# kolinko/effort

Measured on AMD Instinct MI355X. Metric: effective GB/s + tokens/s vs effort %, Mistral-7B FFN 4096x11008 fp16, higher is better.
Workload: dtype f16

## Files before the change

### effort_amd/_lib.py

```python
from __future__ import annotations

import ctypes as C
import os
import subprocess

_HERE = os.path.dirname(os.path.abspath(__file__))
LAB_LIB_PATH = os.path.join(_HERE, "libeffort_hip_lab.so")
LIB_PATH = (LAB_LIB_PATH if os.environ.get("EFFORT_HIP_LIB") == "lab" else os.environ.get("EFFORT_HIP_LIB")) or os.path.join(_HERE, "libeffort_hip.so")

ERRORS = {
    -1: "EFFORT_ERR_ARG", -2: "EFFORT_ERR_SHAPE", -3: "EFFORT_ERR_EFFORT", -4: "EFFORT_ERR_HIP",
    -5: "EFFORT_ERR_KIND", -6: "EFFORT_ERR_CONVERT", -7: "EFFORT_ERR_BLAS", -8: "EFFORT_ERR_COMM",
}


class EffortError(RuntimeError):
    def __init__(self, code: int, where: str, detail: str = ""):
        self.code = code
        super().__init__(f"{where}: {ERRORS.get(code, code)} {detail}".strip())


def build(verbose: bool = False) -> str:
    cmd = ["make", "-C", os.path.join(_HERE, "csrc"), "-j8", "all"]
    res = subprocess.run(cmd, capture_output=not verbose, text=True)
    if res.returncode != 0:
        raise RuntimeError("building libeffort_hip.so failed:\n" + (res.stdout or "") + (res.stderr or ""))
    return LIB_PATH


_P = C.c_void_p
_SIGS = {
    "effort_create": (_P, [C.c_int, _P]),
    "effort_destroy": (None, [_P]),
    "effort_set_stream": (C.c_int, [_P, _P]),
    "effort_sync": (C.c_int, [_P]),
    "effort_set_overlap": (C.c_int, [_P, C.c_int]),
    "effort_set_row_reuse": (C.c_int, [_P, C.c_int]),
    "effort_join": (C.c_int, [_P]),
    "effort_last_error": (C.c_char_p, [_P]),
    "effort_version": (C.c_char_p, []),
    "effort_weights_fp16": (_P, [_P, _P, _P, _P, C.c_int, C.c_int, C.c_int, C.c_int]),
    "effort_weights_fp16_pitched": (_P, [_P, _P, C.c_int, _P, _P, C.c_int, C.c_int, C.c_int, C.c_int]),
    "effort_aligned_row_pitch": (C.c_int, [C.c_int]),
    "effort_weights_q4": (_P, [_P, _P, _P, _P, _P, C.c_int64, C.c_int, C.c_int, C.c_int]),
    "effort_weights_free": (None, [_P]),
    "effort_weights_refresh": (C.c_int, [_P]),
    "effort_weights_align_rows": (C.c_int, [_P]),
    "effort_weights_row_pitch": (C.c_int, [_P]),
    "effort_weights_get_bound": (C.c_int, [_P, C.POINTER(C.c_float)]),
    "effort_weights_set_bound": (C.c_int, [_P, C.POINTER(C.c_float)]),
    "effort_weights_column_shard": (_P, [_P, C.c_int, C.c_int]),
    "effort_comm_unique_id": (C.c_int, [_P]),
    "effort_comm_create": (C.c_int, [_P, C.c_int, C.c_int, _P]),
    "effort_comm_destroy": (C.c_int, [_P]),
    "effort_comm_rank": (C.c_int, [_P]),
    "effort_comm_world": (C.c_int, [_P]),
    "effort_allgather_outputs": (C.c_int, [_P, _P, _P, C.c_int]),
    "effort_bucketmul": (C.c_int, [_P, _P, _P, _P, _P, C.c_double]),
    "effort_bucketmul_q4": (C.c_int, [_P, _P, _P, _P, _P, C.c_double]),
    "effort_bucketmul_group": (C.c_int, [_P, C.c_int, _P, _P, _P, _P, _P]),
    "effort_bucketmul_q4_group": (C.c_int, [_P, C.c_int, _P, _P, _P, _P, _P]),
    "effort_bucketmul_group_fused": (C.c_int, [_P, C.c_int, _P, _P, _P, _P, _P, _P, _P, _P]),
    "effort_bucketmul_q4_group_fused": (C.c_int, [_P, C.c_int, _P, _P, _P, _P, _P, _P, _P, _P]),
    "effort_group_dispatch_count": (C.c_int, [_P, C.c_int, C.POINTER(C.c_uint32)]),
    "effort_group_cutoff": (C.c_int, [_P, C.c_int, C.POINTER(C.c_float)]),
    "effort_debug_occupancy": (C.c_int, [_P, C.c_int, C.c_int, C.c_int, C.c_int]),
    "effort_set_persistent": (C.c_int, [_P, C.c_int]),
    "effort_debug_hook_lane": (C.c_int, [_P, C.c_int]),
    "effort_add_rmsnorm_mul": (C.c_int, [_P, _P, _P, _P, _P, C.c_int]),
    "effort_rope_kv": (C.c_int, [_P, _P, _P, _P, _P, _P, _P, _P, C.c_int, C.c_int, C.c_int, C.c_int, C.c_float]),
    "effort_attention": (C.c_int, [_P, _P, _P, _P, _P, _P, C.c_int, C.c_int, C.c_int]),
    "effort_rope_attention": (C.c_int, [_P, _P, _P, _P, _P, _P, _P, _P, C.c_int, C.c_int, C.c_int, C.c_int, C.c_float]),
    "effort_silu_mul": (C.c_int, [_P, _P, _P, _P, C.c_int]),
    "effort_fetch_row": (C.c_int, [_P, _P, _P, _P, C.c_int]),
    "effort_argmax": (C.c_int, [_P, _P, C.c_int, _P, _P, _P, C.c_int]),
    "effort_decode_status": (C.c_int, [_P, C.POINTER(C.c_int)]),
    "effort_sample": (C.c_int, [_P, _P, C.c_int, _P, _P, _P, _P, C.c_int, _P, _P]),
    "effort_topk": (C.c_int, [_P, _P, C.c_int, C.c_int, _P, _P]),
    "effort_sample_bits": (C.c_uint32, [C.c_uint32, C.c_uint32, C.c_uint32, C.c_uint32]),
    "effort_convert_status": (C.c_int, [_P, C.POINTER(C.c_int)]),
    "effort_q4_outlier_count": (C.c_int64, [C.c_int, C.c_int, C.c_double]),
    "effort_convert_q4": (C.c_int, [_P, _P, C.c_int, C.c_int, C.c_double, _P, _P, _P, _P]),
    "effort_top2_softmax": (C.c_int, [_P, _P, C.c_int, _P, _P]),
    "effort_mix2": (C.c_int, [_P, _P, _P, _P, _P, C.c_int]),
    "effort_moe_route": (C.c_int, [_P, _P, _P, _P, C.c_int, C.c_int, _P, _P, _P]),
    "effort_mix2_add": (C.c_int, [_P, _P, _P, _P, _P, C.c_int]),
    "effort_dense_gemv": (C.c_int, [_P, _P, _P, _P, C.c_int, C.c_int]),
    "effort_dense_gemv_expert": (C.c_int, [_P, _P, _P, _P, _P, C.c_int, C.c_int, C.c_int]),
    "effort_set_dense_backend": (C.c_int, [_P, C.c_int]),
    "effort_last_dispatch_count": (C.c_int, [_P, C.POINTER(C.c_uint32)]),
    "effort_last_cutoff": (C.c_int, [_P, C.POINTER(C.c_float)]),
    "effort_calc_dispatch": (C.c_int, [_P, _P, _P, _P, C.c_double, _P, _P]),
    "effort_convert_fp16": (C.c_int, [_P, _P, C.c_int, C.c_int, _P, _P, _P]),
    "effort_convert_fp16_pitched": (C.c_int, [_P, _P, C.c_int, C.c_int, _P, C.c_int, _P, _P]),
    "effort_cosine": (C.c_int, [_P, _P, _P, C.c_int, C.POINTER(C.c_float)]),
    "effort_set_split_cutoff": (C.c_int, [_P, C.c_int]),
    "effort_set_tuning": (C.c_int, [_P, C.c_int, C.c_int, C.c_int]),
    "effort_is_lab_build": (C.c_int, []),
    "effort_enable_kernel_timing": (C.c_int, [_P, C.c_int]),
    "effort_debug_stamps": (C.c_int, [_P, C.POINTER(C.c_ulonglong)]),
    "effort_debug_slice_counts": (C.c_int, [_P, C.c_int, C.POINTER(C.c_uint32), C.c_int]),
    "effort_debug_plan": (C.c_int, [C.c_int, C.c_int, C.c_int, C.c_int, _P, _P, _P, _P, _P, _P, C.c_int, C.c_int, C.c_int, C.c_int, _P, _P, _P, _P, _P, _P, _P, _P, _P]),
    "effort_debug_trace": (C.c_int, [_P, C.POINTER(C.c_ulonglong), C.c_int]),
    "effort_kernel_clock": (C.c_int, [_P, C.POINTER(C.c_double), C.POINTER(C.c_int)]),
    "effort_kernel_timing": (C.c_int, [_P, C.POINTER(C.c_double), C.POINTER(C.c_double), C.POINTER(C.c_double), C.POINTER(C.c_int)]),
}

_lib = None


def lib() -> C.CDLL:
    global _lib
    if _lib is None:
        if not os.path.exists(LIB_PATH):
            raise RuntimeError(
                f"{LIB_PATH} is missing: the HIP extension has not been built "
                "(run `python -c 'import __graft_entry__ as g; g.build()'` or `make -C effort_amd/csrc`). "
                "effort_amd has no CPU fallback.")
        import torch
        l = C.CDLL(LIB_PATH)
        for name, (res, args) in _SIGS.items():
            if (name.startswith("effort_debug_") or name == "effort_is_lab_build") and os.environ.get("EFFORT_HIP_LIB") and not hasattr(l, name):
                continue
            fn = getattr(l, name)
            fn.restype = res
            fn.argtypes = args
        _lib = l
    return _lib


def exported_symbols() -> list[str]:
    return sorted(_SIGS)
```

### effort_amd/csrc/api.hip

```cpp
#include <dlfcn.h>
#include <rccl/rccl.h>
#include <rocblas/rocblas.h>

#include <cstdio>
#include <cstring>
#include <map>
#include <mutex>
#include <new>
#include <vector>

#include "../../include/effort_hip.h"
#include "../../include/effort_hip_debug.h"
#include "effort_internal.h"
#include "plan.h"
#include "sample_device.h"

using namespace effort;

static constexpr size_t kStampBytes = (size_t)(kTraceOff + kTraceItems * 12) * 8;

struct Lane {
    hipStream_t own = nullptr;
    hipEvent_t done = nullptr;
    bool dirty = false;
    unsigned long long capId = 0;
    float* d_cutoff = nullptr;
    uint32_t* d_count = nullptr;
    float* d_slabs = nullptr;
    uint32_t* d_counters = nullptr;
    uint32_t* d_sliceCounts = nullptr;
    uint32_t* d_queue = nullptr;
    uint32_t lastCalls = 1, lastSliceOff[effort::kMaxGroup] = {0}, lastSlices[effort::kMaxGroup] = {0};
    struct Range { uintptr_t lo, hi; };
    std::vector<Range> reads, writes;
    bool pending = false;
};

struct effort_ctx {
    static constexpr int kMaxLanes = 4;
    int device = 0;
    hipStream_t stream = nullptr;
    int numCU = 256;
    Lane lane[kMaxLanes];
    int nLanes = 1, lastLane = 0, nextLane = 0;
    int busyStreak = 0;
    bool migrated = false;
    hipEvent_t forkEv = nullptr;
    size_t slabBytes = 0;
    uint32_t* d_blockScratch = nullptr;
    uint16_t* d_vhalf = nullptr;
    size_t vhalfElems = 0;
    float* d_cos = nullptr;
    uint16_t* d_convVals = nullptr;
    size_t convElems = 0;
    int* d_status = nullptr;
    int persistent = -1;
    static constexpr uint32_t kMaxTiles = 1024, kMaxSlices = 4096;
    static constexpr size_t kSlabBytes = (size_t)64 << 20;
    static constexpr size_t kMaxRanges = 1024;
    unsigned long long* d_tstamp = nullptr;
    double wallClockKHz = 100000.0;
    rocblas_handle blas = nullptr;
    ncclComm_t comm = nullptr;
    int commRank = 0, commWorld = 1;
    bool denseRocblas = false;
    int tuneW = 0, tuneE = 0, tuneS = 0;
    bool splitCutoff = false;
    bool rowReuse = false;
    bool timing = false;
    bool clock = false;
    bool trace = false;
    static constexpr int kMaxSamples = 4096;
    hipEvent_t* ev = nullptr;
    int nSamples = 0;
    char err[256] = {0};
};

struct effort_w {
    effort_ctx* ctx = nullptr;
    Format fmt = kFp16;
    const uint16_t* buckets = nullptr;
    const uint16_t* bucketsSrc = nullptr;
    uint16_t* aligned = nullptr;
    uint32_t rowPitch = 0;
    uint32_t srcPitch = 0;
    const void* stats = nullptr;
    const uint16_t* probes = nullptr;
    uint32_t inDim = 0, outDim = 0, rowsPerIn = 0, numExperts = 1, cols = 0;
    bool view = false;
    effort_w* parent = nullptr;
    uint32_t viewTrim = 0;
    int views = 0;
    bool dead = false;
    float* rankBound = nullptr;
    uint16_t* means16 = nullptr;
    uint64_t nOutliers = 0;
    uint32_t* olBlockPtr = nullptr;
    uint32_t* olEntry = nullptr;
    uint32_t* olMeta = nullptr;
};

static int fail(effort_ctx* c, int code, const char* what, hipError_t e = hipSuccess) {
    if (c) {
        if (e != hipSuccess) snprintf(c->err, sizeof(c->err), "%s: %s", what, hipGetErrorString(e));
        else snprintf(c->err, sizeof(c->err), "%s", what);
    }
    return code;
}
#define HIP_TRY(ctx, call)                                                   \
    do {                                                                     \
        hipError_t e_ = (call);                                              \
        if (e_ != hipSuccess) return fail((ctx), EFFORT_ERR_HIP, #call, e_); \
    } while (0)

struct RcclApi {
    void* lib = nullptr;
    ncclResult_t (*GetUniqueId)(ncclUniqueId*) = nullptr;
    ncclResult_t (*CommInitRank)(ncclComm_t*, int, ncclUniqueId, int) = nullptr;
    ncclResult_t (*CommDestroy)(ncclComm_t) = nullptr;
    ncclResult_t (*AllGather)(const void*, void*, size_t, ncclDataType_t, ncclComm_t, hipStream_t) = nullptr;
    const char* (*GetErrorString)(ncclResult_t) = nullptr;
    bool ok = false;
};
static const RcclApi& rccl() {
    static RcclApi api = [] {
        RcclApi a;
        for (const char* name : {"librccl.so.1", "librccl.so", "/opt/rocm/lib/librccl.so.1", "/opt/rocm/lib/librccl.so"}) {
            a.lib = dlopen(name, RTLD_NOW | RTLD_GLOBAL);
            if (a.lib) break;
        }
        if (!a.lib) return a;
        a.GetUniqueId = reinterpret_cast<decltype(a.GetUniqueId)>(dlsym(a.lib, "ncclGetUniqueId"));
        a.CommInitRank = reinterpret_cast<decltype(a.CommInitRank)>(dlsym(a.lib, "ncclCommInitRank"));
        a.CommDestroy = reinterpret_cast<decltype(a.CommDestroy)>(dlsym(a.lib, "ncclCommDestroy"));
        a.AllGather = reinterpret_cast<decltype(a.AllGather)>(dlsym(a.lib, "ncclAllGather"));
        a.GetErrorString = reinterpret_cast<decltype(a.GetErrorString)>(dlsym(a.lib, "ncclGetErrorString"));
        a.ok = a.GetUniqueId && a.CommInitRank && a.CommDestroy && a.AllGather && a.GetErrorString;
        return a;
    }();
    return api;
}

extern "C" const char* effort_version(void) { return "effort-hip 0.1 (gfx950)"; }
static char g_createErr[256] = "null context";
extern "C" const char* effort_last_error(effort_ctx* c) { return c ? c->err : g_createErr; }

static bool lane_alloc(effort_ctx* c, Lane& L) {
    bool ok = hipMalloc(&L.d_cutoff, 512) == hipSuccess && hipMalloc(&L.d_count, 16) == hipSuccess &&
              hipMalloc(&L.d_slabs, c->slabBytes) == hipSuccess && hipMalloc(&L.d_counters, effort_ctx::kMaxTiles * 4) == hipSuccess &&
              hipMalloc(&L.d_sliceCounts, effort_ctx::kMaxSlices * 4) == hipSuccess && hipMalloc(&L.d_queue, kQueueWords * 4) == hipSuccess;
    if (!ok) return false;
    hipMemset(L.d_counters, 0, effort_ctx::kMaxTiles * 4);
    hipMemset(L.d_sliceCounts, 0, effort_ctx::kMaxSlices * 4);
    hipMemset(L.d_queue, 0, kQueueWords * 4);
    hipMemset(L.d_cutoff, 0, 512);
    hipMemset(L.d_count, 0, 16);
    return true;
}
static std::mutex g_poolMutex;
static std::map<int, std::vector<hipStream_t>> g_streamPool;
static std::map<int, std::vector<hipEvent_t>> g_eventPool;
static hipStream_t pool_stream(int device) {
    std::lock_guard<std::mutex> lk(g_poolMutex);
    auto& pool = g_streamPool[device];
    if (!pool.empty()) { hipStream_t s = pool.back(); pool.pop_back(); return s; }
    hipStream_t s = nullptr;
    return hipStreamCreateWithFlags(&s, hipStreamNonBlocking) == hipSuccess ? s : nullptr;
}
static hipEvent_t pool_event(int device) {
    std::lock_guard<std::mutex> lk(g_poolMutex);
    auto& pool = g_eventPool[device];
    if (!pool.empty()) { hipEvent_t e = pool.back(); pool.pop_back(); return e; }
    hipEvent_t e = nullptr;
    return hipEventCreateWithFlags(&e, hipEventDisableTiming) == hipSuccess ? e : nullptr;
}
static void pool_put(int device, hipStream_t s) { if (s) { std::lock_guard<std::mutex> lk(g_poolMutex); g_streamPool[device].push_back(s); } }
static void pool_put(int device, hipEvent_t e) { if (e) { std::lock_guard<std::mutex> lk(g_poolMutex); g_eventPool[device].push_back(e); } }

static void lane_free(int device, Lane& L) {
    pool_put(device, L.own);
    pool_put(device, L.done);
    hipFree(L.d_cutoff); hipFree(L.d_count); hipFree(L.d_slabs); hipFree(L.d_counters); hipFree(L.d_sliceCounts); hipFree(L.d_queue);
    L = Lane();
}

extern "C" effort_ctx* effort_create(int device, void* stream) {
    if (hipSetDevice(device) != hipSuccess) return nullptr;
    effort_ctx* c = new (std::nothrow) effort_ctx();
    if (!c) return nullptr;
    c->device = device;
    c->stream = reinterpret_cast<hipStream_t>(stream);
    hipDeviceProp_t prop;
    if (hipGetDeviceProperties(&prop, device) == hipSuccess) c->numCU = prop.multiProcessorCount;
    c->slabBytes = effort_ctx::kSlabBytes;
    {
        static std::mutex m; static std::map<int, bool> prepared;
        std::lock_guard<std::mutex> lk(m);
        if (!prepared[device]) {
            const hipError_t pe = bucket_mul_prepare_device();
            if (pe != hipSuccess) { snprintf(g_createErr, sizeof(g_createErr), "effort_create: kernel attributes: %s", hipGetErrorString(pe)); delete c; return nullptr; }
            prepared[device] = true;
        }
    }
    bool ok = lane_alloc(c, c->lane[0]) && hipMalloc(&c->d_blockScratch, 4096 * 4) == hipSuccess &&
              hipMalloc(&c->d_cos, 16) == hipSuccess && hipMalloc(&c->d_status, 16) == hipSuccess &&
              hipMalloc(&c->d_tstamp, kStampBytes) == hipSuccess;
    if (!ok) { snprintf(g_createErr, sizeof(g_createErr), "effort_create: out of device memory for the context scratch"); effort_destroy(c); return nullptr; }
    int khz = 0;
    if (hipDeviceGetAttribute(&khz, hipDeviceAttributeWallClockRate, device) == hipSuccess && khz > 0) c->wallClockKHz = khz;
    hipMemset(c->d_tstamp, 0, kStampBytes);
    { unsigned long long init[2] = {~0ull, 0ull}; hipMemcpy(c->d_tstamp, init, 16, hipMemcpyHostToDevice); }
    hipMemset(c->d_status, 0, 16);
    return c;
}

static hipStream_t lane_stream(effort_ctx* c, int i) { return c->nLanes > 1 ? c->lane[i].own : c->stream; }
static hipError_t lane_mark(Lane& L) {
    if (!L.dirty) return hipSuccess;
    const hipError_t e = hipEventRecord(L.done, L.own);
    if (e == hipSuccess) L.dirty = false;
    return e;
}
static unsigned long long capture_of(hipStream_t st) {
    hipStreamCaptureStatus cap = hipStreamCaptureStatusNone;
    unsigned long long id = 0;
    if (hipStreamGetCaptureInfo(st, &cap, &id) != hipSuccess) { (void)hipGetLastError(); return 0; }
    return cap == hipStreamCaptureStatusActive ? (id ? id : ~0ull) : 0ull;
}
static bool lanes_match_capture(effort_ctx* c, unsigned long long now) {
    for (int i = 0; i < c->nLanes; i++) {
        Lane& L = c->lane[i];
        if (!L.pending || L.capId == now) continue;
        if (L.capId == 0) {
            snprintf(c->err, sizeof(c->err), "lanes hold launches enqueued BEFORE this hipGraph capture began: call effort_join (or effort_sync) before beginning the capture");
            return false;
        }
        L.pending = false; L.dirty = false; L.capId = 0; L.reads.clear(); L.writes.clear();
    }
    return true;
}
static int join_lanes(effort_ctx* c) {
    if (c->nLanes <= 1) return EFFORT_OK;
    bool any = false;
    for (int i = 0; i < c->nLanes; i++) any = any || c->lane[i].pending;
    if (any && !lanes_match_capture(c, capture_of(c->stream))) return EFFORT_ERR_ARG;
    for (int i = 0; i < c->nLanes; i++) {
        Lane& L = c->lane[i];
        if (!L.pending) continue;
        hipError_t e = lane_mark(L);
        if (e == hipSuccess) e = hipStreamWaitEvent(c->stream, L.done, 0);
        if (e != hipSuccess) { snprintf(c->err, sizeof(c->err), "join: %s", hipGetErrorString(e)); return EFFORT_ERR_HIP; }
        L.pending = false; L.capId = 0; L.reads.clear(); L.writes.clear();
    }
    c->busyStreak = 0; c->migrated = false;
    return EFFORT_OK;
}
static bool overlaps(const std::vector<Lane::Range>& a, const std::vector<Lane::Range>& b) {
    for (const auto& x : a) for (const auto& y : b) if (x.lo < y.hi && y.lo < x.hi) return true;
    return false;
}
struct LaneChoice {
    bool laned = false;
    int li = 0;
    std::vector<Lane::Range> rd, wr;
    int hazard[effort_ctx::kMaxLanes], nh = 0;
    unsigned long long capNow = 0;
};
struct LaneGuard {
    Lane& L; bool forked = false;
    ~LaneGuard() { if (forked) { L.dirty = true; L.pending = true; } }
};
static int choose_lane(effort_ctx* c, LaneChoice& lc, int n, const effort_w* const* ws, const float* const* vs, const uint32_t* const* expNos,
                       float* const* outs, const void* const* vAux, const float* const* resids) {
    if (lc.laned) {
        lc.capNow = capture_of(c->stream);
        if (!lanes_match_capture(c, lc.capNow)) return EFFORT_ERR_ARG;
        bool full = false;
        for (int i = 0; i < c->nLanes; i++) full = full || c->lane[i].reads.size() + c->lane[i].writes.size() > effort_ctx::kMaxRanges;
        if (full) { const int jrc = join_lanes(c); if (jrc != EFFORT_OK) return jrc; }
        auto add = [](std::vector<Lane::Range>& v, const void* p, size_t bytes) { if (p && bytes) v.push_back({(uintptr_t)p, (uintptr_t)p + bytes}); };
        for (int i = 0; i < n; i++) {
            add(lc.rd, vs[i], (size_t)ws[i]->inDim * 4);
            if (expNos && expNos[i]) add(lc.rd, expNos[i], 4);
            if (vAux && vAux[i]) add(lc.rd, vAux[i], (size_t)ws[i]->inDim * 4);
            if (resids && resids[i]) add(lc.rd, resids[i], (size_t)ws[i]->outDim * 4);
            add(lc.wr, outs[i], (size_t)ws[i]->outDim * 4);
        }
        for (int i = 0; i < c->nLanes; i++) {
            const Lane& L = c->lane[i];
            if (L.pending && (overlaps(lc.rd, L.writes) || overlaps(lc.wr, L.writes) || overlaps(lc.wr, L.reads))) lc.hazard[lc.nh++] = i;
        }
        lc.li = lc.nh ? lc.hazard[0] : c->nextLane;
        if (lc.nh == 1 && c->busyStreak >= 4 && !c->migrated) {
            for (int k = 1; k < c->nLanes; k++) {
                const int cand = (lc.hazard[0] + k) % c->nLanes;
                if (!c->lane[cand].pending) { lc.li = cand; c->migrated = true; c->busyStreak = 0; break; }
            }
        }
    } else if (c->nLanes > 1) {
        { const int jrc = join_lanes(c); if (jrc != EFFORT_OK) return jrc; }
    }
    return EFFORT_OK;
}
static int fork_lane(effort_ctx* c, const LaneChoice& lc, LaneGuard& guard) {
    if (!lc.laned || guard.forked) return EFFORT_OK;
    Lane& L = guard.L;
    const int li = lc.li, nh = lc.nh;
    const int* hazard = lc.hazard;
    bool wait = true;
    if (lc.capNow == 0) {
        const hipError_t q = hipStreamQuery(c->stream);
        if (q == hipSuccess) wait = false;
        else {
            (void)hipGetLastError();
            if (q != hipErrorNotReady) return fail(c, EFFORT_ERR_HIP, "hipStreamQuery", q);
        }
    }
    if (wait) {
        HIP_TRY(c, hipEventRecord(c->forkEv, c->stream));
        HIP_TRY(c, hipStreamWaitEvent(L.own, c->forkEv, 0));
    }
    c->busyStreak = (wait && nh == 1 && hazard[0] == li) ? c->busyStreak + 1 : 0;
    guard.forked = true;
    L.capId = lc.capNow;
    auto add_new = [](std::vector<Lane::Range>& have, const std::vector<Lane::Range>& more) {
        for (const auto& x : more) {
            bool seen = false;
            for (const auto& y : have) if (y.lo == x.lo && y.hi == x.hi) { seen = true; break; }
            if (!seen) have.push_back(x);
        }
    };
    for (int k = 0; k < nh; k++) if (hazard[k] != li) {
        Lane& H = c->lane[hazard[k]];
        HIP_TRY(c, lane_mark(H));
        HIP_TRY(c, hipStreamWaitEvent(L.own, H.done, 0));
        add_new(L.reads, H.reads); add_new(L.writes, H.writes);
        H.reads.clear(); H.writes.clear(); H.pending = false;
    }
    if (!nh) c->nextLane = (c->nextLane + 1) % c->nLanes;
    add_new(L.reads, lc.rd);
    add_new(L.writes, lc.wr);
    return EFFORT_OK;
}

extern "C" int effort_set_overlap(effort_ctx* c, int lanes) {
    if (!c || lanes < 1 || lanes > effort_ctx::kMaxLanes) return EFFORT_ERR_ARG;
    hipSetDevice(c->device);
    int rc = join_lanes(c);
    if (rc != EFFORT_OK) return rc;
    if (lanes > 1) {
        if (!c->forkEv && !(c->forkEv = pool_event(c->device))) return fail(c, EFFORT_ERR_HIP, "set_overlap: event");
        for (int i = 0; i < lanes; i++) {
            Lane& L = c->lane[i];
            if (!L.d_slabs && !lane_alloc(c, L)) return fail(c, EFFORT_ERR_HIP, "set_overlap: out of device memory for a lane's scratch");
            if (!L.own && !(L.own = pool_stream(c->device))) return fail(c, EFFORT_ERR_HIP, "set_overlap: stream");
            if (!L.done && !(L.done = pool_event(c->device))) return fail(c, EFFORT_ERR_HIP, "set_overlap: event");
        }
    }
    c->nLanes = lanes; c->lastLane = 0; c->nextLane = 0;
    return EFFORT_OK;
}
extern "C" int effort_join(effort_ctx* c) {
    if (!c) return EFFORT_ERR_ARG;
    return join_lanes(c);
}

extern "C" void effort_destroy(effort_ctx* c) {
    if (!c) return;
    hipSetDevice(c->device);
    for (int i = 0; i < effort_ctx::kMaxLanes; i++) if (c->lane[i].own) hipStreamSynchronize(c->lane[i].own);
    hipStreamSynchronize(c->stream);
    if (c->comm) rccl().CommDestroy(c->comm);
    if (c->blas) rocblas_destroy_handle(c->blas);
    if (c->ev) { for (int i = 0; i < effort_ctx::kMaxSamples * 4; i++) if (c->ev[i]) hipEventDestroy(c->ev[i]); delete[] c->ev; }
    for (int i = 0; i < effort_ctx::kMaxLanes; i++) lane_free(c->device, c->lane[i]);
    pool_put(c->device, c->forkEv);
    hipFree(c->d_blockScratch); hipFree(c->d_vhalf); hipFree(c->d_cos); hipFree(c->d_convVals); hipFree(c->d_status); hipFree(c->d_tstamp);
    delete c;
}

extern "C" int effort_set_stream(effort_ctx* c, void* stream) {
    if (!c) return EFFORT_ERR_ARG;
    if (reinterpret_cast<hipStream_t>(stream) != c->stream && join_lanes(c) != EFFORT_OK) return EFFORT_ERR_HIP;
    c->stream = reinterpret_cast<hipStream_t>(stream);
    if (c->blas) rocblas_set_stream(c->blas, c->stream);
    return EFFORT_OK;
}

extern "C" int effort_sync(effort_ctx* c) {
    if (!c) return EFFORT_ERR_ARG;
    { const int jrc = join_lanes(c); if (jrc != EFFORT_OK) return jrc; }
    HIP_TRY(c, hipStreamSynchronize(c->stream));
    return EFFORT_OK;
}

static int check_shape(uint32_t inDim, uint32_t outDim) {
    if (inDim < (uint32_t)kProbes || outDim == 0 || outDim % 32 || outDim > 16384) return EFFORT_ERR_SHAPE;
    return EFFORT_OK;
}

static int register_bound(effort_ctx* c, effort_w* w) {
    hipSetDevice(c->device);
    const size_t rows = (size_t)w->numExperts * w->rowsPerIn * w->inDim;
    float* scratch = nullptr;
    bool ok = (w->rankBound || hipMalloc(&w->rankBound, (size_t)w->numExperts * 4) == hipSuccess) && hipMalloc(&scratch, rows * 4) == hipSuccess;
    if (ok) ok = launch_rank_bound(w->fmt, w->bucketsSrc, w->srcPitch / 2u, w->stats, w->numExperts, w->rowsPerIn, w->inDim, w->cols, scratch, w->rankBound, c->stream) == hipSuccess;
    if (ok && w->fmt == kFp16) {
        ok = w->means16 || hipMalloc(&w->means16, rows * 2) == hipSuccess;
        if (ok) ok = launch_compact_means(w->stats, w->means16, (uint32_t)rows, c->stream) == hipSuccess;
    }
    if (ok) ok = hipStreamSynchronize(c->stream) == hipSuccess;
    hipFree(scratch);
    return ok ? EFFORT_OK : fail(c, EFFORT_ERR_HIP, "weight registration: rank bound");
}

extern "C" int effort_aligned_row_pitch(int outDim) {
    if (outDim <= 0 || outDim % 32 || outDim > 16384) return EFFORT_ERR_SHAPE;
    return (outDim / 16 * 2 + 127) / 128 * 128;
}

extern "C" effort_w* effort_weights_fp16_pitched(effort_ctx* c, const void* buckets, int rowPitchBytes, const void* stats, const void* probes,
                                                 int inDim, int outDim, int percentLoad, int numExperts) {
    if (!c || !buckets || !stats || !probes) { fail(c, EFFORT_ERR_ARG, "effort_weights_fp16: null argument"); return nullptr; }
    const int pitch = rowPitchBytes ? rowPitchBytes : (outDim > 0 ? outDim / 16 * 2 : 0);
    if (inDim <= 0 || outDim <= 0 || percentLoad < 1 || percentLoad > 16 || numExperts < 1 || check_shape(inDim, outDim) != EFFORT_OK ||
        inDim > 65535 || pitch < outDim / 16 * 2 || pitch % 4 || (size_t)numExperts * percentLoad * inDim * pitch > 0xFFFFFFFFull) {
        fail(c, EFFORT_ERR_SHAPE, "effort_weights_fp16: unsupported shape or row pitch (a multiple of 4 bytes >= 2*cols; buckets < 4 GiB)"); return nullptr; }
    effort_w* w = new (std::nothrow) effort_w();
    if (!w) return nullptr;
    w->ctx = c; w->fmt = kFp16;
    w->buckets = static_cast<const uint16_t*>(buckets); w->stats = stats; w->probes = static_cast<const uint16_t*>(probes);
    w->inDim = inDim; w->outDim = outDim; w->rowsPerIn = percentLoad; w->numExperts = numExperts; w->cols = outDim / 16;
    w->bucketsSrc = w->buckets; w->rowPitch = w->srcPitch = (uint32_t)pitch;
    if (register_bound(c, w) != EFFORT_OK) { effort_weights_free(w); return nullptr; }
    return w;
}
extern "C" effort_w* effort_weights_fp16(effort_ctx* c, const void* buckets, const void* stats, const void* probes,
                                         int inDim, int outDim, int percentLoad, int numExperts) {
    return effort_weights_fp16_pitched(c, buckets, 0, stats, probes, inDim, outDim, percentLoad, numExperts);
}

extern "C" effort_w* effort_weights_q4(effort_ctx* c, const void* buckets, const void* stats, const void* probes,
                                       const void* outliers, int64_t nOutliers, int inDim, int outDim, int numExperts) {
    if (!c || !buckets || !stats || !probes) { fail(c, EFFORT_ERR_ARG, "effort_weights_q4: null argument"); return nullptr; }
    if (inDim <= 0 || outDim <= 0 || numExperts < 1 || check_shape(inDim, outDim) != EFFORT_OK || outDim % 32 || inDim > 65535 ||
        nOutliers < 0 || (size_t)numExperts * 8 * inDim * (outDim / 32) * 2 > 0xFFFFFFFFull) {
        fail(c, EFFORT_ERR_SHAPE, "effort_weights_q4: unsupported shape (or buckets >= 4 GiB)"); return nullptr; }
    effort_w* w = new (std::nothrow) effort_w();
    if (!w) return nullptr;
    w->ctx = c; w->fmt = kQ4;
    w->buckets = static_cast<const uint16_t*>(buckets); w->stats = stats; w->probes = static_cast<const uint16_t*>(probes);
    w->inDim = inDim; w->outDim = outDim; w->rowsPerIn = 8; w->numExperts = numExperts; w->cols = outDim / 32;
    w->bucketsSrc = w->buckets; w->rowPitch = w->srcPitch = w->cols * 2u;
    if (register_bound(c, w) != EFFORT_OK) { effort_weights_free(w); return nullptr; }
    if (outliers && nOutliers > 0) {
        if (outDim > 65536) { fail(c, EFFORT_ERR_SHAPE, "effort_weights_q4: outliers need outDim <= 65536"); effort_weights_free(w); return nullptr; }
        hipSetDevice(c->device);
        {
            int bad[2] = {0, 0};
            bool okv = hipMemsetAsync(c->d_status + 2, 0, 8, c->stream) == hipSuccess &&
                       launch_validate_outliers(static_cast<const float*>(outliers), (uint64_t)nOutliers, (uint32_t)inDim, (uint32_t)outDim, c->d_status + 2, c->stream) == hipSuccess &&
                       hipMemcpyAsync(bad, c->d_status + 2, 8, hipMemcpyDeviceToHost, c->stream) == hipSuccess && hipStreamSynchronize(c->stream) == hipSuccess;
            if (!okv || bad[0] || bad[1]) {
                fail(c, okv ? EFFORT_ERR_ARG : EFFORT_ERR_HIP, !okv ? "effort_weights_q4: outlier validation" :
                     bad[0] ? "effort_weights_q4: outlier entries outside the matrix (inIdx >= inDim or outIdx >= outDim)"
                            : "effort_weights_q4: outlier values that are not f16 numbers (the table comes from an f16 matrix, q4_draft.py:58-67)");
                effort_weights_free(w); return nullptr;
            }
        }
        uint32_t *tmp = nullptr, *rowPtr = nullptr;
        w->nOutliers = (uint64_t)nOutliers;
        const uint32_t olBlocks = ((uint32_t)outDim + 63u) / 64u;
        bool ok = hipMalloc(&rowPtr, ((size_t)outDim + 2) * 4) == hipSuccess && hipMalloc(&w->olBlockPtr, ((size_t)olBlocks + 1) * 4) == hipSuccess &&
                  hipMalloc(&w->olMeta, (size_t)olBlocks * 64 * 4) == hipSuccess &&
                  hipMalloc(&w->olEntry, ((size_t)nOutliers + 64) * 4) == hipSuccess && hipMalloc(&tmp, 4 * (size_t)nOutliers * 4) == hipSuccess;
        if (ok) ok = hipMemsetAsync(w->olEntry + (size_t)nOutliers, 0, 64 * 4, c->stream) == hipSuccess;
        if (ok) ok = launch_build_outlier_index(static_cast<const float*>(outliers), w->nOutliers, (uint32_t)inDim, (uint32_t)outDim, rowPtr, w->olBlockPtr,
                                                w->olEntry, w->olMeta, tmp, c->stream) == hipSuccess;
        if (ok) ok = hipStreamSynchronize(c->stream) == hipSuccess;
        hipFree(tmp);
        uint32_t longest = 0;
        if (ok) ok = hipMemcpy(&longest, rowPtr + (size_t)outDim + 1, 4, hipMemcpyDeviceToHost) == hipSuccess;
        hipFree(rowPtr);
        if (!ok) { fail(c, EFFORT_ERR_HIP, "effort_weights_q4: outlier index"); effort_weights_free(w); return nullptr; }
        if (longest >= (1u << 24)) { fail(c, EFFORT_ERR_SHAPE, "effort_weights_q4: more than 2^24 outliers on one output"); effort_weights_free(w); return nullptr; }
    }
    return w;
}

static int copy_aligned(effort_w* w) {
    const size_t rows = (size_t)w->numExperts * w->rowsPerIn * w->inDim;
    HIP_TRY(w->ctx, hipMemcpy2DAsync(w->aligned, w->rowPitch, w->bucketsSrc, w->srcPitch, (size_t)w->cols * 2, rows, hipMemcpyDeviceToDevice, w->ctx->stream));
    HIP_TRY(w->ctx, hipStreamSynchronize(w->ctx->stream));
    return EFFORT_OK;
}
extern "C" int effort_weights_refresh(effort_w* w) {
    if (!w || !w->ctx || w->dead) return EFFORT_ERR_ARG;
    if (w->view) return fail(w->ctx, EFFORT_ERR_ARG, "effort_weights_refresh: a column shard takes its bound from the full handle -- refresh that one and shard again");
    hipSetDevice(w->ctx->device);
    int rc = join_lanes(w->ctx);
    if (rc == EFFORT_OK) rc = register_bound(w->ctx, w);
    if (rc == EFFORT_OK && w->aligned) rc = copy_aligned(w);
    return rc;
}
extern "C" int effort_weights_align_rows(effort_w* w) {
    if (!w || !w->ctx || w->dead) return EFFORT_ERR_ARG;
    if (w->aligned || w->rowPitch % 128u == 0u) return EFFORT_OK;
    hipSetDevice(w->ctx->device);
    const uint32_t pitch = (w->cols * 2u + 127u) / 128u * 128u;
    const size_t rows = (size_t)w->numExperts * w->rowsPerIn * w->inDim;
    if (rows * pitch > 0xFFFFFFFFull) return fail(w->ctx, EFFORT_ERR_SHAPE, "effort_weights_align_rows: the padded buckets would reach 4 GiB");
    if (hipMalloc(&w->aligned, rows * pitch) != hipSuccess) return fail(w->ctx, EFFORT_ERR_HIP, "effort_weights_align_rows: out of device memory");
    HIP_TRY(w->ctx, hipMemsetAsync(w->aligned, 0, rows * pitch, w->ctx->stream));
    w->rowPitch = pitch;
    const int rc = copy_aligned(w);
    if (rc != EFFORT_OK) { hipFree(w->aligned); w->aligned = nullptr; w->rowPitch = w->srcPitch; return rc; }
    w->buckets = w->aligned;
    return EFFORT_OK;
}
extern "C" int effort_weights_row_pitch(const effort_w* w) { return w ? (int)w->rowPitch : EFFORT_ERR_ARG; }
extern "C" int effort_weights_get_bound(effort_w* w, float* host_out) {
    if (!w || !w->ctx || !host_out || !w->rankBound) return EFFORT_ERR_ARG;
    HIP_TRY(w->ctx, hipMemcpy(host_out, w->rankBound, (size_t)w->numExperts * 4, hipMemcpyDeviceToHost));
    return EFFORT_OK;
}
extern "C" int effort_weights_set_bound(effort_w* w, const float* host_in) {
    if (!w || !w->ctx || !host_in || !w->rankBound || w->dead) return EFFORT_ERR_ARG;
    for (uint32_t e = 0; e < w->numExperts; e++) if (!(host_in[e] >= 0.0f)) return EFFORT_ERR_ARG;
    { const int jrc = join_lanes(w->ctx); if (jrc != EFFORT_OK) return jrc; }
    HIP_TRY(w->ctx, hipStreamSynchronize(w->ctx->stream));
    HIP_TRY(w->ctx, hipMemcpy(w->rankBound, host_in, (size_t)w->numExperts * 4, hipMemcpyHostToDevice));
    return EFFORT_OK;
}

static std::mutex g_viewMutex;
extern "C" void effort_weights_free(effort_w* w) {
    if (!w) return;
    if (w->view) {
        effort_w* const par = w->parent;
        hipFree(w->rankBound);
        delete w;
        bool last = false;
        if (par) { std::lock_guard<std::mutex> lk(g_viewMutex); last = --par->views == 0 && par->dead; if (last) par->dead = false; }
        if (last) effort_weights_free(par);
        return;
    }
    {
        std::lock_guard<std::mutex> lk(g_viewMutex);
        if (w->views > 0) { w->dead = true; return; }
    }
    hipFree(w->olBlockPtr); hipFree(w->olEntry); hipFree(w->olMeta);
    hipFree(w->aligned); hipFree(w->rankBound); hipFree(w->means16);
    delete w;
}

extern "C" effort_w* effort_weights_column_shard(const effort_w* full, int rank, int world) {
    if (!full || !full->ctx) return nullptr;
    effort_ctx* c = full->ctx;
    const uint32_t unit = full->fmt == kFp16 ? 16u : 32u;
    if (world < 1 || rank < 0 || rank >= world || full->cols % (uint32_t)world || (full->cols / (uint32_t)world) % 2u) {
        fail(c, EFFORT_ERR_SHAPE, "effort_weights_column_shard: the bucket columns must split evenly into an even number per rank"); return nullptr; }
    const uint32_t per = full->cols / (uint32_t)world, outDim = per * unit;
    if (check_shape(full->inDim, outDim) != EFFORT_OK) { fail(c, EFFORT_ERR_SHAPE, "effort_weights_column_shard: shard shape"); return nullptr; }
    if (full->nOutliers && outDim % 64u) {
        fail(c, EFFORT_ERR_SHAPE, "effort_weights_column_shard: the shard must hold whole blocks of the outlier index"); return nullptr; }
    effort_w* w = new (std::nothrow) effort_w();
    if (!w) return nullptr;
    {
        std::lock_guard<std::mutex> lk(g_viewMutex);
        if (full->view || full->dead) { fail(c, EFFORT_ERR_ARG, "effort_weights_column_shard: shard a full, live handle"); delete w; return nullptr; }
        const_cast<effort_w*>(full)->views++;
    }
    *w = *full;
    w->view = true; w->parent = const_cast<effort_w*>(full); w->views = 0; w->dead = false;
    w->aligned = nullptr; w->rankBound = nullptr;
    w->buckets = full->buckets + (size_t)rank * per;
    w->viewTrim = (uint32_t)((size_t)rank * per * 2u);
    w->bucketsSrc = w->buckets; w->srcPitch = full->rowPitch;
    w->cols = per; w->outDim = outDim;
    hipSetDevice(c->device);
    if (hipMalloc(&w->rankBound, (size_t)w->numExperts * 4) != hipSuccess ||
        hipMemcpy(w->rankBound, full->rankBound, (size_t)w->numExperts * 4, hipMemcpyDeviceToDevice) != hipSuccess) {
        fail(c, EFFORT_ERR_HIP, "effort_weights_column_shard: bound"); hipFree(w->rankBound);
        effort_w* const par = w->parent;
        delete w;
        bool last;
        { std::lock_guard<std::mutex> lk(g_viewMutex); last = --par->views == 0 && par->dead; if (last) par->dead = false; }
        if (last) effort_weights_free(par);
        return nullptr; }
    if (full->nOutliers) {
        w->olBlockPtr = full->olBlockPtr + (size_t)rank * outDim / 64u;
        w->olMeta = full->olMeta + (size_t)rank * outDim;
    }
    return w;
}
extern "C" int effort_comm_unique_id(void* id_out) {
    if (!id_out) return EFFORT_ERR_ARG;
    static_assert(sizeof(ncclUniqueId) == EFFORT_COMM_ID_BYTES, "effort_hip.h: EFFORT_COMM_ID_BYTES");
    if (!rccl().ok) return EFFORT_ERR_COMM;
    return rccl().GetUniqueId(static_cast<ncclUniqueId*>(id_out)) == ncclSuccess ? EFFORT_OK : EFFORT_ERR_COMM;
}
extern "C" int effort_comm_create(effort_ctx* c, int rank, int world, const void* id) {
    if (!c || !id || world < 1 || rank < 0 || rank >= world) return fail(c, EFFORT_ERR_ARG, "comm_create: bad argument");
    if (c->comm) return fail(c, EFFORT_ERR_ARG, "comm_create: the context has a communicator already");
    hipSetDevice(c->device);
    ncclUniqueId uid;
    memcpy(&uid, id, sizeof(uid));
    if (!rccl().ok) return fail(c, EFFORT_ERR_COMM, "comm_create: librccl.so could not be opened (dlopen) -- multi-GPU needs RCCL");
    const ncclResult_t r = rccl().CommInitRank(&c->comm, world, uid, rank);
    if (r != ncclSuccess) { c->comm = nullptr; snprintf(c->err, sizeof(c->err), "ncclCommInitRank: %s", rccl().GetErrorString(r)); return EFFORT_ERR_COMM; }
    c->commRank = rank; c->commWorld = world;
    return EFFORT_OK;
}
extern "C" int effort_comm_destroy(effort_ctx* c) {
    if (!c) return EFFORT_ERR_ARG;
    if (c->comm) { hipSetDevice(c->device); effort_sync(c); rccl().CommDestroy(c->comm); c->comm = nullptr; c->commRank = 0; c->commWorld = 1; }
    return EFFORT_OK;
}
extern "C" int effort_comm_rank(effort_ctx* c) { return c ? c->commRank : EFFORT_ERR_ARG; }
extern "C" int effort_comm_world(effort_ctx* c) { return c ? c->commWorld : EFFORT_ERR_ARG; }
extern "C" int effort_allgather_outputs(effort_ctx* c, const float* send, float* recv, int count) {
    if (!c || !send || !recv || count < 1) return fail(c, EFFORT_ERR_ARG, "allgather_outputs: bad argument");
    if (!c->comm) return fail(c, EFFORT_ERR_ARG, "allgather_outputs: no communicator (effort_comm_create)");
    { const int jrc = join_lanes(c); if (jrc != EFFORT_OK) return jrc; }
    const ncclResult_t r = rccl().AllGather(send, recv, (size_t)count, ncclFloat, c->comm, c->stream);
    if (r != ncclSuccess) { snprintf(c->err, sizeof(c->err), "ncclAllGather: %s", rccl().GetErrorString(r)); return EFFORT_ERR_COMM; }
    return EFFORT_OK;
}

static int ensure_timing(effort_ctx* c) {
    if (c->ev) return EFFORT_OK;
    c->ev = new (std::nothrow) hipEvent_t[effort_ctx::kMaxSamples * 4]();
    if (!c->ev) return EFFORT_ERR_HIP;
    for (int i = 0; i < effort_ctx::kMaxSamples * 4; i++) HIP_TRY(c, hipEventCreate(&c->ev[i]));
    return EFFORT_OK;
}

static PlanEnv plan_env(const effort_ctx* c, bool laned, bool thinEffort) {
    PlanEnv env;
    env.numCU = c->numCU; env.nLanes = c->nLanes; env.laned = laned;
    env.persistent = c->persistent; env.tuneW = c->tuneW; env.tuneE = c->tuneE; env.tuneS = c->tuneS;
    env.splitCutoff = c->splitCutoff; env.clock = c->clock;
    env.slabBytes = c->slabBytes; env.maxTiles = effort_ctx::kMaxTiles; env.maxSlices = effort_ctx::kMaxSlices;
    env.thinEffort = thinEffort;
#ifdef EFFORT_LAB
    static const uint32_t ablate = getenv("EFFORT_ABLATE") ? (uint32_t)atoi(getenv("EFFORT_ABLATE")) : 0u;
    static const bool noJobs = getenv("EFFORT_NO_CUTJOBS") != nullptr, noCompact = getenv("EFFORT_NO_COMPACT_MEANS") != nullptr;
    env.ablate = ablate; env.noJobs = noJobs; env.noCompact = noCompact;
    if (getenv("EFFORT_TAIL_CALLS")) {
        env.tailCalls = atoi(getenv("EFFORT_TAIL_CALLS"));
        env.tailMult = getenv("EFFORT_TAIL_MULT") ? atoi(getenv("EFFORT_TAIL_MULT")) : 2;
    }
#endif
    return env;
}
static PlanCall plan_call(const effort_w* w, int pre, bool resid) {
    return PlanCall{w->inDim, w->outDim, w->cols, w->rowsPerIn, w->rowPitch, w->numExperts, w->means16 != nullptr, (uint16_t)pre, resid};
}
static bool thin_effort(int n, const double* efforts) {
    double sum = 0.0;
    for (int i = 0; i < n; i++) sum += efforts[i];
    return sum < 0.08 * n;
}

static int do_group(effort_ctx* c, Format fmt, int n, const effort_w* const* ws, const float* const* vs,
                    const uint32_t* const* expNos, float* const* outs, const double* efforts,
                    const int* prologues = nullptr, const void* const* vAux = nullptr, const float* const* resids = nullptr) {
    if (!c || !ws || !vs || !outs || !efforts) return fail(c, EFFORT_ERR_ARG, "bucketmul: null argument");
    if (n < 1 || n > kMaxGroup) return fail(c, EFFORT_ERR_ARG, "bucketmul: group size outside 1..32");
    PlanCall pc[kMaxGroup];
    for (int i = 0; i < n; i++) {
        if (!ws[i] || !vs[i] || !outs[i]) return fail(c, EFFORT_ERR_ARG, "bucketmul: null argument");
        if (ws[i]->dead) return fail(c, EFFORT_ERR_ARG, "bucketmul: the handle was freed (its buffers live on only for its column shards)");
        if (ws[i]->fmt != fmt) return fail(c, EFFORT_ERR_KIND, "bucketmul: weight handle of the wrong kind");
        if (!(efforts[i] >= 0.0 && efforts[i] <= 1.0)) return fail(c, EFFORT_ERR_EFFORT, "bucketmul: effort outside [0,1]");
        const int pre = prologues ? prologues[i] : 0;
        if (pre < 0 || pre > 2 || (pre && (!vAux || !vAux[i]))) return fail(c, EFFORT_ERR_ARG, "bucketmul: bad input prologue");
        if (pre && c->splitCutoff) return fail(c, EFFORT_ERR_KIND, "bucketmul: input prologues need the fused cutoff");
        if (pre && fmt == kQ4 && ws[i]->olBlockPtr && (uint32_t)ws[i]->inDim > bucket_mul_ol_lds_floats())
            return fail(c, EFFORT_ERR_SHAPE, "bucketmul: an input prologue on a Q4 handle with outliers needs inDim <= 16384 (materialise the input, or register without outliers)");
        pc[i] = plan_call(ws[i], pre, resids && resids[i]);
    }
    LaneChoice lc;
    lc.laned = c->nLanes > 1 && !c->timing && !c->clock;
    const PlanEnv env = plan_env(c, lc.laned, thin_effort(n, efforts));
    GroupPlan plan;
    if (plan_group(fmt, env, n, pc, &plan) != EFFORT_OK) return fail(c, plan.err, plan.msg);
    const bool tm = c->timing && c->nSamples < effort_ctx::kMaxSamples;
    hipEvent_t* ev = tm ? c->ev + 4 * c->nSamples : nullptr;
    { const int lrc = choose_lane(c, lc, n, ws, vs, expNos, outs, vAux, resids); if (lrc != EFFORT_OK) return lrc; }
    Lane& L = c->lane[lc.li];
    const hipStream_t st = lc.laned ? L.own : c->stream;
    LaneGuard guard{L};
    c->lastLane = lc.li;
    if (tm) HIP_TRY(c, hipEventRecord(ev[0], st));
    for (uint32_t l = 0; l < plan.nLaunches; l++) {
        const LaunchPlan& lp = plan.launch[l];
        GroupKArgs ga;
        memset(&ga, 0, sizeof(ga));
        ga.groupDone = L.d_counters + effort_ctx::kMaxTiles - 1;
        ga.slabs = L.d_slabs; ga.counters = L.d_counters; ga.sliceCounts = L.d_sliceCounts; ga.cutoff = L.d_cutoff + lp.first;
        ga.tstamp = c->clock ? c->d_tstamp : nullptr;
        ga.ablate = env.ablate; ga.trace = (c->clock && c->trace) ? 1u : 0u;
        ga.split = (c->splitCutoff ? 1u : 0u) | (lp.compact ? 4u : 0u) | (c->rowReuse ? 8u : 0u);
        ga.numCU = (uint32_t)c->numCU; ga.queue = L.d_queue;
        ga.count = lp.count; ga.totalTiles = lp.totalTiles; ga.totalItems = lp.totalItems;
        ga.persistent = lp.persistent; ga.cutJobs = lp.cutJobs; ga.staggerSleeps = lp.staggerSleeps;
        for (uint32_t k = 0; k < lp.count; k++) {
            const int i = (int)(lp.first + k);
            const effort_w* w = ws[i];
            const CallPlan& p = plan.call[i];
            CallDesc& a = ga.call[k];
            a.buckets = w->buckets; a.stats = lp.compact ? (const void*)w->means16 : w->stats; a.rankBound = w->rankBound; a.probes = w->probes; a.v = vs[i];
            a.expNo = expNos ? expNos[i] : nullptr; a.out = outs[i];
            a.ol = OutlierIndex{fmt == kQ4 ? w->olBlockPtr : nullptr, w->olEntry, w->olMeta};
            a.q = (uint16_t)(int)((double)(kProbes - 1) * (1.0 - efforts[i]));
            a.bucketsTrim = (uint16_t)w->viewTrim;
            a.pre = pc[i].pre; a.vAux = a.pre ? vAux[i] : nullptr; a.resid = resids ? resids[i] : nullptr;
            a.slabOff = p.slabOff; a.tileOff = (uint16_t)p.tileOff; a.sliceOff = (uint16_t)p.sliceOff; a.geom = (uint16_t)p.geom;
            ga.geom[p.geom] = p.g;
            ga.wgEnd8[k] = (uint16_t)p.itemEnd8;
            L.lastSliceOff[i] = p.sliceOff; L.lastSlices[i] = p.g.slices;
        }
        { const int frc = fork_lane(c, lc, guard); if (frc != EFFORT_OK) return frc; }
        if (c->splitCutoff && !(env.ablate & 1u)) HIP_TRY(c, launch_find_cutoff_group(ga, st));
        HIP_TRY(c, launch_bucket_mul(fmt, plan.W, plan.E, ga, st));
    }
    L.lastCalls = (uint32_t)n;
    if (tm) { HIP_TRY(c, hipEventRecord(ev[1], st)); c->nSamples++; }
    return EFFORT_OK;
}

extern "C" int effort_bucketmul(effort_ctx* c, const effort_w* w, const float* v, const uint32_t* expNo, float* out, double effort) {
    return do_group(c, kFp16, 1, &w, &v, &expNo, &out, &effort);
}
extern "C" int effort_bucketmul_q4(effort_ctx* c, const effort_w* w, const float* v, const uint32_t* expNo, float* out, double effort) {
    return do_group(c, kQ4, 1, &w, &v, &expNo, &out, &effort);
}
extern "C" int effort_bucketmul_group(effort_ctx* c, int n, const effort_w* const* ws, const float* const* vs,
                                      const uint32_t* const* expNos, float* const* outs, const double* efforts) {
    return do_group(c, kFp16, n, ws, vs, expNos, outs, efforts);
}
extern "C" int effort_bucketmul_group_fused(effort_ctx* c, int n, const effort_w* const* ws, const float* const* vs,
                                            const uint32_t* const* expNos, float* const* outs, const double* efforts,
                                            const int* prologues, const void* const* vAux, const float* const* resids) {
    return do_group(c, kFp16, n, ws, vs, expNos, outs, efforts, prologues, vAux, resids);
}
extern "C" int effort_bucketmul_q4_group_fused(effort_ctx* c, int n, const effort_w* const* ws, const float* const* vs,
                                               const uint32_t* const* expNos, float* const* outs, const double* efforts,
                                               const int* prologues, const void* const* vAux, const float* const* resids) {
    return do_group(c, kQ4, n, ws, vs, expNos, outs, efforts, prologues, vAux, resids);
}
extern "C" int effort_bucketmul_q4_group(effort_ctx* c, int n, const effort_w* const* ws, const float* const* vs,
                                         const uint32_t* const* expNos, float* const* outs, const double* efforts) {
    return do_group(c, kQ4, n, ws, vs, expNos, outs, efforts);
}

extern "C" int effort_calc_dispatch(effort_ctx* c, const effort_w* w, const float* v, const uint32_t* expNo, double effort,
                                    float* dispatch, uint32_t* count) {
    if (!c || !w || !v || !dispatch || w->dead) return fail(c, EFFORT_ERR_ARG, "calc_dispatch: null argument (or a freed handle)");
    if (!(effort >= 0.0 && effort <= 1.0)) return fail(c, EFFORT_ERR_EFFORT, "calc_dispatch: effort outside [0,1]");
    { const int jrc = join_lanes(c); if (jrc != EFFORT_OK) return jrc; }
    Lane& L = c->lane[0];
    c->lastLane = 0;
    const PlanCall pc = plan_call(w, 0, false);
    GroupPlan plan;
    if (plan_group(w->fmt, plan_env(c, false, false), 1, &pc, &plan) != EFFORT_OK) return fail(c, plan.err, "calc_dispatch: geometry");
    const MulGeom& g = plan.call[0].g;
    const uint32_t q = (uint32_t)(int)((double)(kProbes - 1) * (1.0 - effort));
    HIP_TRY(c, launch_find_cutoff(v, w->probes, expNo, q, L.d_cutoff, L.d_count, nullptr, c->stream));
    HIP_TRY(c, launch_calc_dispatch(w->fmt, w->stats, v, expNo, L.d_cutoff, g, dispatch, count, L.d_count, c->d_blockScratch, c->stream));
    L.lastCalls = 1; L.lastSlices[0] = 0;
    return EFFORT_OK;
}

extern "C" int effort_group_dispatch_count(effort_ctx* c, int idx, uint32_t* host_out) {
    if (!c || !host_out || idx < 0 || (uint32_t)idx >= c->lane[c->lastLane].lastCalls) return EFFORT_ERR_ARG;
    { const int jrc = join_lanes(c); if (jrc != EFFORT_OK) return jrc; }
    Lane& L = c->lane[c->lastLane];
    if (L.lastSlices[idx] == 0) {
        HIP_TRY(c, hipMemcpyAsync(host_out, L.d_count, 4, hipMemcpyDeviceToHost, c->stream));
        HIP_TRY(c, hipStreamSynchronize(c->stream));
        return EFFORT_OK;
    }
    static thread_local uint32_t h[effort_ctx::kMaxSlices];
    HIP_TRY(c, hipMemcpyAsync(h, L.d_sliceCounts + L.lastSliceOff[idx], (size_t)L.lastSlices[idx] * 4, hipMemcpyDeviceToHost, c->stream));
    HIP_TRY(c, hipStreamSynchronize(c->stream));
    uint32_t n = 0;
    for (uint32_t i = 0; i < L.lastSlices[idx]; i++) n += h[i];
    *host_out = n;
    return EFFORT_OK;
}
extern "C" int effort_debug_slice_counts(effort_ctx* c, int idx, uint32_t* host, int maxSlices) {
    if (!c || !host || idx < 0 || (uint32_t)idx >= c->lane[c->lastLane].lastCalls || maxSlices < 1) return EFFORT_ERR_ARG;
    { const int jrc = join_lanes(c); if (jrc != EFFORT_OK) return jrc; }
    Lane& L = c->lane[c->lastLane];
    const uint32_t n = L.lastSlices[idx] < (uint32_t)maxSlices ? L.lastSlices[idx] : (uint32_t)maxSlices;
    if (n) HIP_TRY(c, hipMemcpyAsync(host, L.d_sliceCounts + L.lastSliceOff[idx], (size_t)n * 4, hipMemcpyDeviceToHost, c->stream));
    HIP_TRY(c, hipStreamSynchronize(c->stream));
    return (int)n;
}
extern "C" int effort_debug_plan(int q4, int numCU, int lanes, int n, const int* inDim, const int* outDim, const int* percentLoad,
                                 const int* prologue, const int* hasResid, const double* effort, int persistent, int tuneW, int tuneE, int tuneS,
                                 int* we, int* slices, int* tiles, int* sliceRows, int* launchOf,
                                 int* launchPersistent, int* launchCutJobs, int* launchCompact, int* launchStagger) {
    if (numCU < 1 || lanes < 1 || lanes > effort_ctx::kMaxLanes || n < 1 || n > kMaxGroup || !inDim || !outDim || !effort || !we || !slices || !tiles ||
        !sliceRows || !launchOf || !launchPersistent || !launchCutJobs || !launchCompact || !launchStagger) return EFFORT_ERR_ARG;
    const Format fmt = q4 ? kQ4 : kFp16;
    effort_ctx c0;
    c0.numCU = numCU; c0.nLanes = lanes; c0.persistent = persistent; c0.tuneW = tuneW; c0.tuneE = tuneE; c0.tuneS = tuneS;
    c0.slabBytes = effort_ctx::kSlabBytes;
    PlanCall pc[kMaxGroup];
    for (int i = 0; i < n; i++) {
        const int load = q4 ? 8 : (percentLoad ? percentLoad[i] : 16);
        if (inDim[i] <= 0 || outDim[i] <= 0 || check_shape((uint32_t)inDim[i], (uint32_t)outDim[i]) != EFFORT_OK || load < 1 || load > 16) return EFFORT_ERR_SHAPE;
        if (!(effort[i] >= 0.0 && effort[i] <= 1.0)) return EFFORT_ERR_EFFORT;
        const uint32_t cols = (uint32_t)outDim[i] / (q4 ? 32u : 16u);
        pc[i] = PlanCall{(uint32_t)inDim[i], (uint32_t)outDim[i], cols, (uint32_t)load, cols * 2u, 1u, !q4, (uint16_t)(prologue ? prologue[i] : 0), hasResid && hasResid[i]};
    }
    GroupPlan plan;
    const int rc = plan_group(fmt, plan_env(&c0, lanes > 1, thin_effort(n, effort)), n, pc, &plan);
    if (rc != EFFORT_OK) return rc;
    we[0] = plan.W; we[1] = plan.E;
    for (int i = 0; i < n; i++) {
        const CallPlan& p = plan.call[i];
        slices[i] = (int)p.g.slices; tiles[i] = (int)p.g.tiles; sliceRows[i] = (int)p.g.sliceRows; launchOf[i] = (int)p.launch;
    }
    for (uint32_t l = 0; l < plan.nLaunches; l++) {
        const LaunchPlan& lp = plan.launch[l];
        launchPersistent[l] = (int)lp.persistent; launchCutJobs[l] = (int)lp.cutJobs; launchCompact[l] = lp.compact ? 1 : 0; launchStagger[l] = (int)lp.staggerSleeps;
    }
    return (int)plan.nLaunches;
}
extern "C" int effort_group_cutoff(effort_ctx* c, int idx, float* host_out) {
    if (!c || !host_out || idx < 0 || (uint32_t)idx >= c->lane[c->lastLane].lastCalls) return EFFORT_ERR_ARG;
    { const int jrc = join_lanes(c); if (jrc != EFFORT_OK) return jrc; }
    Lane& L = c->lane[c->lastLane];
    HIP_TRY(c, hipMemcpyAsync(host_out, L.d_cutoff + idx, 4, hipMemcpyDeviceToHost, c->stream));
    HIP_TRY(c, hipStreamSynchronize(c->stream));
    return EFFORT_OK;
}
extern "C" int effort_last_dispatch_count(effort_ctx* c, uint32_t* host_out) { return effort_group_dispatch_count(c, 0, host_out); }
extern "C" int effort_last_cutoff(effort_ctx* c, float* host_out) { return effort_group_cutoff(c, 0, host_out); }

extern "C" int effort_set_dense_backend(effort_ctx* c, int rocblas) {
    if (!c) return EFFORT_ERR_ARG;
    c->denseRocblas = rocblas != 0;
    return EFFORT_OK;
}
extern "C" int effort_dense_gemv(effort_ctx* c, const void* W, const float* v, float* out, int inDim, int outDim) {
    if (!c || !W || !v || !out || inDim <= 0 || outDim <= 0) return fail(c, EFFORT_ERR_ARG, "dense_gemv: bad argument");
    { const int jrc = join_lanes(c); if (jrc != EFFORT_OK) return jrc; }
    if (inDim % 16) return fail(c, EFFORT_ERR_SHAPE, "dense_gemv: inDim % 16 != 0 (helpers/mps.swift:18)");
    if (!c->denseRocblas && dense_gemv_supported((uint32_t)inDim, (uint32_t)outDim)) {
        HIP_TRY(c, launch_dense_gemv(static_cast<const uint16_t*>(W), v, out, (uint32_t)inDim, (uint32_t)outDim, c->stream));
        return EFFORT_OK;
    }
    if (!c->blas) {
        if (rocblas_create_handle(&c->blas) != rocblas_status_success) return fail(c, EFFORT_ERR_BLAS, "rocblas_create_handle");
        rocblas_set_stream(c->blas, c->stream);
        rocblas_set_pointer_mode(c->blas, rocblas_pointer_mode_host);
    }
    if ((size_t)inDim > c->vhalfElems) {
        HIP_TRY(c, hipStreamSynchronize(c->stream));
        hipFree(c->d_vhalf); c->d_vhalf = nullptr; c->vhalfElems = 0;
        HIP_TRY(c, hipMalloc(&c->d_vhalf, (size_t)inDim * 2));
        c->vhalfElems = inDim;
    }
    HIP_TRY(c, launch_f32_to_f16(v, c->d_vhalf, inDim, c->stream));
    const float alpha = 1.0f, beta = 0.0f;
    rocblas_status s = rocblas_hssgemv_strided_batched(c->blas, rocblas_operation_transpose, inDim, outDim, &alpha,
                                                       static_cast<const rocblas_half*>(W), inDim, 0,
                                                       reinterpret_cast<const rocblas_half*>(c->d_vhalf), 1, 0, &beta, out, 1, 0, 1);
    if (s != rocblas_status_success) return fail(c, EFFORT_ERR_BLAS, "rocblas_hssgemv_strided_batched");
    return EFFORT_OK;
}
extern "C" int effort_dense_gemv_expert(effort_ctx* c, const void* W, const uint32_t* expNo, const float* v, float* out, int inDim, int outDim,
                                        int numExperts) {
    if (!c || !W || !expNo || !v || !out || inDim <= 0 || outDim <= 0 || numExperts <= 0) return fail(c, EFFORT_ERR_ARG, "dense_gemv_expert: bad argument");
    { const int jrc = join_lanes(c); if (jrc != EFFORT_OK) return jrc; }
    if (!dense_gemv_supported((uint32_t)inDim, (uint32_t)outDim) || (size_t)numExperts * outDim * inDim * 2 > 0xFFFFFFFFull)
        return fail(c, EFFORT_ERR_SHAPE, "dense_gemv_expert: inDim % 16 != 0, inDim > 65536, or a stack of 4 GiB or more");
    HIP_TRY(c, launch_dense_gemv_expert(static_cast<const uint16_t*>(W), expNo, v, out, (uint32_t)inDim, (uint32_t)outDim, (uint32_t)numExperts, c->stream));
    return EFFORT_OK;
}

extern "C" int effort_convert_fp16_pitched(effort_ctx* c, const void* W, int outDim, int inDim, void* buckets, int rowPitchBytes, void* stats, void* probes) {
    if (!c || !W || !buckets || !stats || !probes) return fail(c, EFFORT_ERR_ARG, "convert_fp16: null argument");
    { const int jrc = join_lanes(c); if (jrc != EFFORT_OK) return jrc; }
    if (outDim <= 0 || inDim < kProbes || !(outDim >= kProbes || kProbes % outDim == 0) || outDim > 16384 || inDim > 32000 ||
        outDim % 16 || (outDim / 16) % 4)
        return fail(c, EFFORT_ERR_CONVERT, "convert_fp16: bucketize preconditions violated");
    const int pitch = rowPitchBytes ? rowPitchBytes : outDim / 16 * 2;
    if (pitch < outDim / 16 * 2 || pitch % 8) return fail(c, EFFORT_ERR_CONVERT, "convert_fp16: row pitch must be a multiple of 8 bytes >= 2*cols");
    const size_t elems = (size_t)outDim * inDim;
    if (elems > c->convElems) {
        HIP_TRY(c, hipStreamSynchronize(c->stream));
        hipFree(c->d_convVals); c->d_convVals = nullptr; c->convElems = 0;
        HIP_TRY(c, hipMalloc(&c->d_convVals, elems * 2));
        c->convElems = elems;
    }
    HIP_TRY(c, launch_convert_fp16(static_cast<const uint16_t*>(W), outDim, inDim, static_cast<uint16_t*>(buckets), (uint32_t)pitch / 2u,
                                   static_cast<uint16_t*>(stats), static_cast<uint16_t*>(probes), c->d_convVals, c->d_status, c->stream));
    return EFFORT_OK;
}
extern "C" int effort_convert_fp16(effort_ctx* c, const void* W, int outDim, int inDim, void* buckets, void* stats, void* probes) {
    return effort_convert_fp16_pitched(c, W, outDim, inDim, buckets, 0, stats, probes);
}

extern "C" int64_t effort_q4_outlier_count(int inDim, int outDim, double perc) {
    if (inDim <= 0 || outDim <= 0 || !(perc >= 0.0 && perc <= 1.0)) return EFFORT_ERR_ARG;
    return (int64_t)((double)((int64_t)inDim * outDim) * perc);
}
extern "C" int effort_convert_q4(effort_ctx* c, const void* core2, int inDim, int outDim, double perc, void* buckets, void* stats, void* probes,
                                 void* outliers) {
    if (!c || !core2 || !buckets || !stats || !probes) return fail(c, EFFORT_ERR_ARG, "convert_q4: null argument");
    { const int jrc = join_lanes(c); if (jrc != EFFORT_OK) return jrc; }
    if (inDim <= 0 || outDim <= 0 || outDim % 32 || (int64_t)inDim * outDim >= (1ll << 32) || !(perc >= 0.0 && perc <= 1.0))
        return fail(c, EFFORT_ERR_CONVERT, "convert_q4: outDim % 32 != 0 (q4_draft.py:299), or a matrix of 2^32 elements or more");
    const int64_t cnt = effort_q4_outlier_count(inDim, outDim, perc);
    if (cnt >= (1ll << 31)) return fail(c, EFFORT_ERR_CONVERT, "convert_q4: 2^31 outliers or more (the candidate sort counts in int)");
    if (cnt > 0 && !outliers) return fail(c, EFFORT_ERR_ARG, "convert_q4: outliers buffer missing");
    hipSetDevice(c->device);
    HIP_TRY(c, launch_convert_q4(static_cast<const uint16_t*>(core2), (uint32_t)inDim, (uint32_t)outDim, (uint32_t)cnt, static_cast<uint16_t*>(buckets),
                                 static_cast<float*>(stats), static_cast<uint16_t*>(probes), static_cast<float*>(outliers), c->numCU, c->stream));
    return EFFORT_OK;
}

extern "C" int effort_cosine(effort_ctx* c, const float* a, const float* b, int n, float* host_out) {
    if (!c || !a || !b || !host_out || n <= 0) return EFFORT_ERR_ARG;
    { const int jrc = join_lanes(c); if (jrc != EFFORT_OK) return jrc; }
    HIP_TRY(c, launch_cosine(a, b, n, c->d_cos, c->stream));
    HIP_TRY(c, hipMemcpyAsync(host_out, c->d_cos, 4, hipMemcpyDeviceToHost, c->stream));
    HIP_TRY(c, hipStreamSynchronize(c->stream));
    return EFFORT_OK;
}

extern "C" int effort_add_rmsnorm_mul(effort_ctx* c, float* h, const float* delta, const void* w, float* out, int n) {
    if (!c || !h || !w || !out || n <= 0) return fail(c, EFFORT_ERR_ARG, "add_rmsnorm_mul: bad argument");
    { const int jrc = join_lanes(c); if (jrc != EFFORT_OK) return jrc; }
    HIP_TRY(c, launch_add_rmsnorm_mul(h, delta, static_cast<const uint16_t*>(w), out, (uint32_t)n, c->stream));
    return EFFORT_OK;
}
extern "C" int effort_rope_kv(effort_ctx* c, const float* xq, const float* xk, const float* xv, float* qOut, float* kCache,
                              float* vCache, const uint32_t* pos, int numHeads, int numHeadsKV, int headDim, int maxTokens, float ropeBase) {
    if (!c || !xq || !xk || !xv || !qOut || !kCache || !vCache || !pos) return fail(c, EFFORT_ERR_ARG, "rope_kv: null argument");
    { const int jrc = join_lanes(c); if (jrc != EFFORT_OK) return jrc; }
    if (numHeads <= 0 || numHeadsKV <= 0 || numHeads % numHeadsKV || headDim < 2 || headDim > 1024 || headDim % 2 || !(ropeBase > 1.0f) || maxTokens <= 0)
        return fail(c, EFFORT_ERR_SHAPE, "rope_kv: bad head geometry");
    HIP_TRY(c, launch_rope_kv(xq, xk, xv, qOut, kCache, vCache, pos, numHeads, numHeadsKV, headDim, ropeBase, (uint32_t)maxTokens, c->d_status + 1, c->stream));
    return EFFORT_OK;
}
extern "C" int effort_attention(effort_ctx* c, const float* q, const float* kCache, const float* vCache, const uint32_t* pos,
                                float* out, int numHeads, int headDim, int maxTokens) {
    if (!c || !q || !kCache || !vCache || !pos || !out) return fail(c, EFFORT_ERR_ARG, "attention: null argument");
    { const int jrc = join_lanes(c); if (jrc != EFFORT_OK) return jrc; }
    if (numHeads <= 0 || maxTokens <= 0 || maxTokens > 8192 || (headDim != 64 && headDim != 128 && headDim != 256))
        return fail(c, EFFORT_ERR_SHAPE, "attention: headDim 64/128/256, maxTokens <= 8192");
    HIP_TRY(c, launch_attention(q, kCache, vCache, pos, out, numHeads, headDim, maxTokens, c->stream));
    return EFFORT_OK;
}
extern "C" int effort_rope_attention(effort_ctx* c, const float* xq, const float* xk, const float* xv, float* kCache, float* vCache,
                                     const uint32_t* pos, float* out, int numHeads, int numHeadsKV, int headDim, int maxTokens, float ropeBase) {
    if (!c || !xq || !xk || !xv || !kCache || !vCache || !pos || !out) return fail(c, EFFORT_ERR_ARG, "rope_attention: null argument");
    { const int jrc = join_lanes(c); if (jrc != EFFORT_OK) return jrc; }
    if (numHeads <= 0 || numHeadsKV <= 0 || numHeads % numHeadsKV || maxTokens <= 0 || maxTokens > 8192 || !(ropeBase > 1.0f) ||
        (headDim != 64 && headDim != 128 && headDim != 256))
        return fail(c, EFFORT_ERR_SHAPE, "rope_attention: headDim 64/128/256, maxTokens <= 8192");
    HIP_TRY(c, launch_rope_attention(xq, xk, xv, kCache, vCache, pos, out, numHeads, numHeadsKV, headDim, maxTokens, ropeBase, c->d_status + 1, c->stream));
    return EFFORT_OK;
}
extern "C" int effort_silu_mul(effort_ctx* c, const float* x1, const float* x3, float* out, int n) {
    if (!c || !x1 || !x3 || !out || n <= 0) return fail(c, EFFORT_ERR_ARG, "silu_mul: bad argument");
    { const int jrc = join_lanes(c); if (jrc != EFFORT_OK) return jrc; }
    HIP_TRY(c, launch_silu_mul(x1, x3, out, (uint32_t)n, c->stream));
    return EFFORT_OK;
}
extern "C" int effort_fetch_row(effort_ctx* c, const void* emb, const uint32_t* id, float* out, int n) {
    if (!c || !emb || !id || !out || n <= 0) return fail(c, EFFORT_ERR_ARG, "fetch_row: bad argument");
    { const int jrc = join_lanes(c); if (jrc != EFFORT_OK) return jrc; }
    HIP_TRY(c, launch_fetch_row(static_cast<const uint16_t*>(emb), id, out, (uint32_t)n, c->stream));
    return EFFORT_OK;
}
extern "C" int effort_top2_softmax(effort_ctx* c, const float* gate, int n, uint32_t* idx2, float* val2) {
    if (!c || !gate || !idx2 || !val2 || n < 1) return fail(c, EFFORT_ERR_ARG, "top2_softmax: bad argument");
    { const int jrc = join_lanes(c); if (jrc != EFFORT_OK) return jrc; }
    HIP_TRY(c, launch_top2_softmax(gate, (uint32_t)n, idx2, val2, c->stream));
    return EFFORT_OK;
}
extern "C" int effort_mix2(effort_ctx* c, const float* f0, const float* f1, const float* val2, float* out, int n) {
    if (!c || !f0 || !f1 || !val2 || !out || n <= 0) return fail(c, EFFORT_ERR_ARG, "mix2: bad argument");
    { const int jrc = join_lanes(c); if (jrc != EFFORT_OK) return jrc; }
    HIP_TRY(c, launch_mix2(f0, f1, val2, out, (uint32_t)n, c->stream));
    return EFFORT_OK;
}
extern "C" int effort_moe_route(effort_ctx* c, const float* h, const void* normW, const void* gateW, int n, int numExperts, float* gateOut,
                                uint32_t* idx2, float* val2) {
    if (!c || !h || !normW || !gateW || !idx2 || !val2) return fail(c, EFFORT_ERR_ARG, "moe_route: null argument");
    { const int jrc = join_lanes(c); if (jrc != EFFORT_OK) return jrc; }
    if (n <= 0 || numExperts <= 0 || !moe_route_supported((uint32_t)n, (uint32_t)numExperts))
        return fail(c, EFFORT_ERR_SHAPE, "moe_route: n % 16 == 0, 16 <= n <= 16384, 1 <= numExperts <= 64");
    HIP_TRY(c, launch_moe_route(h, static_cast<const uint16_t*>(normW), static_cast<const uint16_t*>(gateW), (uint32_t)n, (uint32_t)numExperts, gateOut,
                                idx2, val2, c->stream));
    return EFFORT_OK;
}
extern "C" int effort_mix2_add(effort_ctx* c, float* h, const float* f0, const float* f1, const float* val2, int n) {
    if (!c || !h || !f0 || !f1 || !val2 || n <= 0) return fail(c, EFFORT_ERR_ARG, "mix2_add: bad argument");
    { const int jrc = join_lanes(c); if (jrc != EFFORT_OK) return jrc; }
    HIP_TRY(c, launch_mix2_add(h, f0, f1, val2, (uint32_t)n, c->stream));
    return EFFORT_OK;
}
extern "C" int effort_argmax(effort_ctx* c, const float* logits, int n, uint32_t* idOut, uint32_t* pos, uint32_t* history, int historyLen) {
    if (!c || !logits || !idOut || !pos || n <= 0 || (history && historyLen <= 0)) return fail(c, EFFORT_ERR_ARG, "argmax: bad argument");
    { const int jrc = join_lanes(c); if (jrc != EFFORT_OK) return jrc; }
    HIP_TRY(c, launch_argmax(logits, (uint32_t)n, idOut, pos, history, (uint32_t)(history ? historyLen : 0), c->d_status + 1, c->stream));
    return EFFORT_OK;
}
extern "C" int effort_sample(effort_ctx* c, const float* logits, int n, const effort_sample_params* params, uint32_t* idOut, uint32_t* pos,
                             uint32_t* history, int historyLen, uint32_t* topkIdx, float* topkVal) {
    if (!c || !logits || !params || !idOut || !pos || n <= 0 || (history && historyLen <= 0)) return fail(c, EFFORT_ERR_ARG, "sample: bad argument");
    { const int jrc = join_lanes(c); if (jrc != EFFORT_OK) return jrc; }
    HIP_TRY(c, launch_sample(logits, (uint32_t)n, params, idOut, pos, history, (uint32_t)(history ? historyLen : 0), c->d_status + 1, topkIdx, topkVal,
                             c->stream));
    return EFFORT_OK;
}
extern "C" int effort_topk(effort_ctx* c, const float* logits, int n, int k, uint32_t* idx, float* val) {
    if (!c || !logits || !idx || !val || n <= 0 || k < 1 || k > EFFORT_SAMPLE_MAX_K) return fail(c, EFFORT_ERR_ARG, "topk: bad argument (1 <= k <= 64)");
    { const int jrc = join_lanes(c); if (jrc != EFFORT_OK) return jrc; }
    HIP_TRY(c, launch_topk(logits, (uint32_t)n, (uint32_t)k, idx, val, c->stream));
    return EFFORT_OK;
}
extern "C" uint32_t effort_sample_bits(uint32_t seedLo, uint32_t seedHi, uint32_t stream, uint32_t pos) { return philox_x0(seedLo, seedHi, stream, pos); }
extern "C" int effort_decode_status(effort_ctx* c, int* host_out) {
    if (!c || !host_out) return EFFORT_ERR_ARG;
    { const int jrc = join_lanes(c); if (jrc != EFFORT_OK) return jrc; }
    HIP_TRY(c, hipMemcpyAsync(host_out, c->d_status + 1, 4, hipMemcpyDeviceToHost, c->stream));
    HIP_TRY(c, hipMemsetAsync(c->d_status + 1, 0, 4, c->stream));
    HIP_TRY(c, hipStreamSynchronize(c->stream));
    return EFFORT_OK;
}
extern "C" int effort_convert_status(effort_ctx* c, int* host_out) {
    if (!c || !host_out) return EFFORT_ERR_ARG;
    { const int jrc = join_lanes(c); if (jrc != EFFORT_OK) return jrc; }
    HIP_TRY(c, hipMemcpyAsync(host_out, c->d_status, 4, hipMemcpyDeviceToHost, c->stream));
    HIP_TRY(c, hipMemsetAsync(c->d_status, 0, 4, c->stream));
    HIP_TRY(c, hipStreamSynchronize(c->stream));
    return EFFORT_OK;
}

extern "C" int effort_set_tuning(effort_ctx* c, int W, int E, int S) {
    if (!c) return EFFORT_ERR_ARG;
    if ((W || E) && !supported(W ? W : 16, E ? E : 1)) return fail(c, EFFORT_ERR_ARG, "set_tuning: unsupported (waves, elems)");
    if (S < 0) return EFFORT_ERR_ARG;
    c->tuneW = W; c->tuneE = E; c->tuneS = S;
    return EFFORT_OK;
}

extern "C" int effort_debug_occupancy(effort_ctx* c, int q4, int W, int E, int ldsBytes) {
    if (!c || !supported(W, E)) return EFFORT_ERR_ARG;
    return bucket_mul_occupancy(q4 ? kQ4 : kFp16, W, E, (size_t)ldsBytes);
}

extern "C" int effort_set_persistent(effort_ctx* c, int wgPerCU) {
    if (!c || wgPerCU < -1 || wgPerCU > 8) return EFFORT_ERR_ARG;
    c->persistent = wgPerCU;
    return EFFORT_OK;
}

extern "C" int effort_debug_hook_lane(effort_ctx* c, int lane) {
    if (!c || lane < 0 || lane >= c->nLanes) return EFFORT_ERR_ARG;
    c->lastLane = lane;
    return EFFORT_OK;
}

extern "C" int effort_set_row_reuse(effort_ctx* c, int reuse) {
    if (!c) return EFFORT_ERR_ARG;
    c->rowReuse = reuse != 0;
    return EFFORT_OK;
}

extern "C" int effort_set_split_cutoff(effort_ctx* c, int split) {
    if (!c) return EFFORT_ERR_ARG;
    c->splitCutoff = split != 0;
    return EFFORT_OK;
}

#ifdef EFFORT_LAB
static constexpr bool kLabBuild = true;
#else
static constexpr bool kLabBuild = false;
#endif
static int lab_only(effort_ctx* c) { return fail(c, EFFORT_ERR_KIND, "device-clock stamps / traces are compiled into libeffort_hip_lab.so only (EFFORT_HIP_LIB=lab)"); }
extern "C" int effort_is_lab_build(void) { return kLabBuild ? 1 : 0; }

extern "C" int effort_enable_kernel_timing(effort_ctx* c, int enable) {
    if (!c) return EFFORT_ERR_ARG;
    if (!kLabBuild && enable >= 2) return lab_only(c);
    if (enable == 1) { int rc = ensure_timing(c); if (rc != EFFORT_OK) return rc; }
    c->timing = enable == 1;
    c->clock = kLabBuild && enable != 0;
    c->trace = kLabBuild && enable == 3;
    if (c->trace) HIP_TRY(c, hipMemsetAsync(c->d_tstamp + kTraceOff, 0, (size_t)kTraceItems * 96, c->stream));
    c->nSamples = 0;
    HIP_TRY(c, hipMemsetAsync(c->d_tstamp, 0, 4096, c->stream));
    HIP_TRY(c, hipMemsetAsync(c->d_tstamp, 0xFF, 8, c->stream));
    return EFFORT_OK;
}

extern "C" int effort_debug_stamps(effort_ctx* c, unsigned long long* host32) {
    if (!c || !host32) return EFFORT_ERR_ARG;
    if (!kLabBuild) return lab_only(c);
    HIP_TRY(c, hipMemcpyAsync(host32, c->d_tstamp + 8, 192, hipMemcpyDeviceToHost, c->stream));
    unsigned long long lines[32 * 8];
    HIP_TRY(c, hipMemcpyAsync(lines, c->d_tstamp + 64, sizeof(lines), hipMemcpyDeviceToHost, c->stream));
    HIP_TRY(c, hipStreamSynchronize(c->stream));
    for (int i = 0; i < 8; i++) { host32[24 + i] = 0; for (int l = 0; l < 32; l++) host32[24 + i] += lines[l * 8 + i]; }
    return EFFORT_OK;
}

extern "C" int effort_debug_trace(effort_ctx* c, unsigned long long* host, int maxRecords) {
    if (!c || !host || maxRecords < 1 || maxRecords > kTraceItems) return EFFORT_ERR_ARG;
    if (!kLabBuild) return lab_only(c);
    HIP_TRY(c, hipMemcpyAsync(host, c->d_tstamp + kTraceOff, (size_t)maxRecords * 64, hipMemcpyDeviceToHost, c->stream));
    HIP_TRY(c, hipMemcpyAsync(host + (size_t)maxRecords * 8, c->d_tstamp + kTraceOff + (size_t)kTraceItems * 8, (size_t)maxRecords * 32, hipMemcpyDeviceToHost, c->stream));
    HIP_TRY(c, hipStreamSynchronize(c->stream));
    return EFFORT_OK;
}

extern "C" int effort_kernel_clock(effort_ctx* c, double* mul_us_avg, int* n_launches) {
    if (!c) return EFFORT_ERR_ARG;
    if (!kLabBuild) return lab_only(c);
    unsigned long long h[4] = {0, 0, 0, 0};
    HIP_TRY(c, hipMemcpyAsync(h, c->d_tstamp, 32, hipMemcpyDeviceToHost, c->stream));
    HIP_TRY(c, hipStreamSynchronize(c->stream));
    if (mul_us_avg) *mul_us_avg = h[3] ? (double)h[2] / (double)h[3] * 1000.0 / c->wallClockKHz : 0.0;
    if (n_launches) *n_launches = (int)h[3];
    HIP_TRY(c, hipMemsetAsync(c->d_tstamp + 2, 0, 16, c->stream));
    return EFFORT_OK;
}

extern "C" int effort_kernel_timing(effort_ctx* c, double* mul_us, double* cutoff_us, double* integrate_us, int* n) {
    if (!c) return EFFORT_ERR_ARG;
    HIP_TRY(c, hipStreamSynchronize(c->stream));
    double a = 0, b = 0, d = 0;
    for (int i = 0; i < c->nSamples; i++) {
        float ms;
        HIP_TRY(c, hipEventElapsedTime(&ms, c->ev[4 * i + 0], c->ev[4 * i + 1])); b += ms;
    }
    const int ns = c->nSamples ? c->nSamples : 1;
    if (cutoff_us) *cutoff_us = a * 1000.0 / ns;
    if (mul_us) *mul_us = b * 1000.0 / ns;
    if (integrate_us) *integrate_us = d * 1000.0 / ns;
    if (n) *n = c->nSamples;
    c->nSamples = 0;
    return EFFORT_OK;
}
```

### effort_amd/csrc/bucket_mul.hip

```cpp
#include <cstring>
#include <type_traits>

#include "cutoff_device.h"

namespace effort {

#ifndef EFFORT_KBATCH
#define EFFORT_KBATCH 16
#endif
constexpr int kBatch = EFFORT_KBATCH;
#ifndef EFFORT_KBATCH4
#define EFFORT_KBATCH4 8
#endif
template <int E> __host__ __device__ constexpr int batch_rows() { return E >= 4 ? EFFORT_KBATCH4 : kBatch; }
constexpr int kRounds = 16;

#ifndef EFFORT_ABLATE_NOSCATTER
#define EFFORT_ABLATE_NOSCATTER 0
#endif
#ifndef EFFORT_ABLATE_NOLOAD
#define EFFORT_ABLATE_NOLOAD 0
#endif

#ifndef EFFORT_MIN_WAVES_PER_EU
#define EFFORT_MIN_WAVES_PER_EU 4
#endif

#ifndef EFFORT_ROW_AUX
#define EFFORT_ROW_AUX 2
#endif
constexpr int kRowAux = EFFORT_ROW_AUX;
#ifndef EFFORT_OL_NT
#define EFFORT_OL_NT 0
#endif
#if EFFORT_OL_NT
#define EFFORT_OL_LOAD(p) __builtin_nontemporal_load(p)
#else
#define EFFORT_OL_LOAD(p) (*(p))
#endif
#define GA_PERSISTENT(ga) (PERSIST ? (ga).persistent : 0u)
#define GA_CUTJOBS(ga) (PERSIST ? (ga).cutJobs : 0u)
#ifndef EFFORT_LAB
#define EFFORT_PRODUCT_ONLY 1
#if defined(EFFORT_PAD_TEST) || defined(EFFORT_CUT_FINE) || defined(EFFORT_NO_TOUCH) || defined(EFFORT_NO_STAMPS) || EFFORT_ABLATE_NOSCATTER || EFFORT_ABLATE_NOLOAD
#error "lab switches need -DEFFORT_LAB (they belong in libeffort_hip_lab.so / build/variants, never in the shipped library)"
#endif
#endif
#ifdef EFFORT_PRODUCT_ONLY
constexpr bool kProductOnly = true;
#else
constexpr bool kProductOnly = false;
#endif
#ifdef EFFORT_PRODUCT_ONLY
#define GA_TSTAMP(ga) ((unsigned long long*)nullptr)
#define GA_ABLATE(ga) 0u
#define GA_TRACE(ga) 0u
#elif defined(EFFORT_LEAN_STAMPS)
#define GA_TSTAMP(ga) ((ga).tstamp)
#define GA_ABLATE(ga) (PERSIST ? (ga).ablate : 0u)
#define GA_TRACE(ga) 0u
#else
#define GA_TSTAMP(ga) (PERSIST ? (ga).tstamp : nullptr)
#define GA_ABLATE(ga) (PERSIST ? (ga).ablate : 0u)
#define GA_TRACE(ga) (PERSIST ? (ga).trace : 0u)
#endif
constexpr uint32_t kMaxLdsBytes = 160u * 1024u - 1024u;
constexpr int kSc1 = 16;

template <int FMT> struct Fmt;
template <> struct Fmt<kFp16> { static constexpr int kAcc = 16, kSlots = 16; };
template <> struct Fmt<kQ4> { static constexpr int kAcc = 32, kSlots = 64; };

template <int FMT> struct MeanT;
template <> struct MeanT<kFp16> { typedef uint16_t type; };
template <> struct MeanT<kQ4> { typedef float type; };

template <int E> struct Piece;
template <> struct Piece<1> {
    uint32_t w;
    template <int AUX> __device__ __forceinline__ void load(__amdgpu_buffer_rsrc_t r, uint32_t voff, uint32_t soff) { w = __builtin_amdgcn_raw_buffer_load_b16(r, voff, soff, AUX); }
    __device__ __forceinline__ uint32_t word(int) const { return w & 0xFFFFu; }
    __device__ __forceinline__ uint32_t dword(int) const { return w; }
};
template <> struct Piece<2> {
    uint32_t w;
    template <int AUX> __device__ __forceinline__ void load(__amdgpu_buffer_rsrc_t r, uint32_t voff, uint32_t soff) { w = __builtin_amdgcn_raw_buffer_load_b32(r, voff, soff, AUX); }
    __device__ __forceinline__ uint32_t word(int j) const { return (w >> (16 * j)) & 0xFFFFu; }
    __device__ __forceinline__ uint32_t dword(int) const { return w; }
};
template <> struct Piece<4> {
    uint32_t w[2];
    template <int AUX> __device__ __forceinline__ void load(__amdgpu_buffer_rsrc_t r, uint32_t voff, uint32_t soff) {
        auto t = __builtin_amdgcn_raw_buffer_load_b64(r, voff, soff, AUX); w[0] = t[0]; w[1] = t[1];
    }
    __device__ __forceinline__ uint32_t word(int j) const { return (w[j >> 1] >> (16 * (j & 1))) & 0xFFFFu; }
    __device__ __forceinline__ uint32_t dword(int j) const { return w[j >> 1]; }
};
__host__ __device__ inline uint32_t align_up(uint32_t x, uint32_t a) { return (x + a - 1) / a * a; }

constexpr int kOlBatch = 16;
constexpr uint32_t kOlLdsFloats = 16384;
template <int E> __host__ __device__ inline uint32_t ol_outputs_per_item(const MulGeom& g) { return align_up((32u * E * 64u + g.slices - 1u) / g.slices, 64u); }
constexpr uint32_t kOlEarlyFloats = 4096;
constexpr int kOlMerged = 8;
constexpr uint32_t kOlSumFloats = 1024;
template <int E> __host__ __device__ inline uint32_t ol_scratch_bytes(const MulGeom& g) {
    const uint32_t per = ol_outputs_per_item<E>(g);
    return (per > kOlSumFloats ? per : kOlSumFloats) * 4u + (g.inDim <= kOlLdsFloats ? g.inDim * 4u : 0u);
}

template <int FMT, int E, int W>
__host__ __device__ inline LdsPlan plan_lds(const MulGeom* geoms, int nGeoms, bool merge) {
    uint32_t slots = 0, vrows = 0, ol = 0, vEarly = 0;
    for (int i = 0; i < nGeoms; i++) {
        const MulGeom& g = geoms[i];
        if (!g.slices) continue;
        slots = slots > g.slots ? slots : g.slots;
        const uint32_t vr = align_up(g.sliceRows, 64);
        vrows = vrows > vr ? vrows : vr;
        if (FMT != kFp16) {
            const uint32_t x = ol_scratch_bytes<E>(g); ol = ol > x ? ol : x;
            if (merge && W == 8 && g.inDim <= kOlEarlyFloats) vEarly = vEarly > g.inDim * 4u ? vEarly : g.inDim * 4u;
        }
    }
    LdsPlan p;
    uint32_t o = 0;
    p.offM = o; o += align_up(slots, 64) * 4;
    p.offV[0] = o; o += vrows * 4;
    p.offV[1] = FMT == kFp16 ? o : p.offV[0];
    if (FMT == kFp16) o += vrows * 4;
    if (FMT != kFp16 && o < ol) o = align_up(ol, 16);
    p.offA = o; o += (uint32_t)Fmt<FMT>::kSlots * E * 64 * 4;
    p.offL = o; o += align_up(slots * 2, 16);
    const uint32_t tbl = cutoff_table_bytes(64 * W);
    if (o < p.offA + tbl) o = p.offA + tbl;
    p.offC = o; o += 2048;
    p.offO = vEarly ? o : 0u; o += vEarly;
    static_assert(kCutoffLdsBytes <= 1280, "the cutoff scratch must end below the flags of the misc region");
    p.total = o;
    return p;
}
struct ItemRef { uint32_t ci, t, s; };

__device__ __forceinline__ bool locate_item(const GroupKArgs& ga, const uint32_t item, ItemRef& r) {
    uint32_t ci = 0;
    for (uint32_t i = 0; i + 1 < ga.count; i++) if ((item >> 3) >= (uint32_t)ga.wgEnd8[i]) ci = i + 1;
    ci = __builtin_amdgcn_readfirstlane(ci);
    const MulGeom& g = ga.geom[ga.call[ci].geom];
    const uint32_t b = item - (ci ? (uint32_t)ga.wgEnd8[ci - 1] * 8u : 0u), xcd = b & 7u, k = b >> 3;
    r.ci = ci;
    if ((g.slices & 7u) == 0u) {
        r.s = (k / g.tiles) * 8u + ((xcd + ci) & 7u); r.t = k % g.tiles;
        return true;
    }
    const uint32_t per = (uint32_t)ga.wgEnd8[ci] - (ci ? (uint32_t)ga.wgEnd8[ci - 1] : 0u);
    const uint32_t idx = ((xcd + ci) & 7u) * per + k;
    r.s = idx / g.tiles; r.t = idx - r.s * g.tiles;
    return r.s < g.slices;
}

typedef uint32_t u32x4 __attribute__((ext_vector_type(4)));
__device__ __forceinline__ void lds_dma_dword(const u32x4 rsrc, const uint32_t voff, const uint32_t ldsAddr) {
    uint32_t keep;
    asm volatile("s_mov_b32 %0, m0\n\ts_mov_b32 m0, %2\n\ts_nop 0\n\tbuffer_load_dword %1, %3, 0 offen lds\n\ts_mov_b32 m0, %0"
                 : "=&s"(keep) : "v"(voff), "s"(ldsAddr), "s"(rsrc) : "memory");
}
__device__ __forceinline__ u32x4 make_rsrc(const void* base, uint32_t bytes) {
    const uint64_t p = (uint64_t)(size_t)base;
    u32x4 r;
    r[0] = __builtin_amdgcn_readfirstlane((uint32_t)p); r[1] = __builtin_amdgcn_readfirstlane((uint32_t)(p >> 32) & 0xFFFFu);
    r[2] = __builtin_amdgcn_readfirstlane(bytes); r[3] = 0x00020000u;
    return r;
}

template <int FMT, int W, bool COMPACT>
__device__ __forceinline__ void stage_issue(const GroupKArgs& ga, const ItemRef& r, const int tid, char* smem, const LdsPlan& lp, const uint32_t par) {
    constexpr int NT = 64 * W;
    using lds_v = __attribute__((address_space(3))) void;
    const CallDesc& a = ga.call[__builtin_amdgcn_readfirstlane(r.ci)];
    const MulGeom& g = ga.geom[a.geom];
    const uint32_t wave = __builtin_amdgcn_readfirstlane(tid >> 6);
    const uint32_t B = g.sliceRows, j0 = __builtin_amdgcn_readfirstlane(r.s) * B, nb = min(B, g.inDim - j0), lg = g.sliceLog2;
    const uint32_t e = a.expNo ? a.expNo[0] : 0u;
    const uint32_t rowBase = e * g.expertRows;
    const uint32_t rowsPerIn = g.rowsPerIn, inDim = g.inDim, mask = (1u << lg) - 1u;
    const uint32_t nSlots = FMT == kFp16 ? (rowsPerIn << lg) : (nb << 3);
    constexpr bool compact = COMPACT && FMT == kFp16;
    const u32x4 rs = make_rsrc(a.stats, (uint32_t)((size_t)g.numExperts * g.expertRows * (compact ? 2u : 8u)));
    const u32x4 rv = make_rsrc(a.v, inDim * 4u);
    const uint32_t ldsM = __builtin_amdgcn_readfirstlane((uint32_t)(size_t)(lds_v*)(smem + lp.offM));
    const uint32_t ldsV = __builtin_amdgcn_readfirstlane((uint32_t)(size_t)(lds_v*)(smem + ((par & 1u) ? lp.offV[1] : lp.offV[0])));
    if constexpr (compact) {
#pragma unroll
        for (int rr = 0; rr < kRounds / 2; rr++) {
            if (((uint32_t)(rr * NT) + wave * 64u) * 2u >= nSlots) continue;
            const uint32_t c = ((uint32_t)(rr * NT) + (uint32_t)tid) * 2u, rank = c >> lg, jl = c & mask;
            const bool ok = rank < rowsPerIn && jl < nb;
            lds_dma_dword(rs, (rowBase + (ok ? rank * inDim + j0 + jl : j0)) * 2u, ldsM + ((uint32_t)(rr * NT) + wave * 64u) * 4u);
        }
    } else
#pragma unroll
    for (int rr = 0; rr < kRounds; rr++) {
        if ((uint32_t)(rr * NT) + wave * 64u >= nSlots) continue;
        const uint32_t c = rr * NT + tid;
        uint32_t voff;
        if (FMT == kFp16) {
            const uint32_t rank = c >> lg, jl = c & mask;
            const bool ok = rank < rowsPerIn && jl < nb;
            voff = (rowBase + (ok ? rank * inDim + j0 + jl : j0)) * 8u + 4u;
        } else {
            voff = ((rowBase + j0 * 8u + (c < nSlots ? c : 0u)) * 2u + 1u) * 4u;
        }
        lds_dma_dword(rs, voff, ldsM + ((uint32_t)(rr * NT) + wave * 64u) * 4u);
    }
#pragma unroll
    for (int u = 0; u < (FMT == kFp16 ? 1 : 2); u++) {
        if ((uint32_t)(u * NT) + wave * 64u >= nb) continue;
        lds_dma_dword(rv, (j0 + (uint32_t)(u * NT + tid)) * 4u, ldsV + ((uint32_t)(u * NT) + wave * 64u) * 4u);
    }
}

template <int FMT, int E, int W, bool FUSED, bool COMPACT, bool PERSIST, typename Prefetch>
__device__ __forceinline__ void mul_item(const GroupKArgs& ga, const uint32_t item, const ItemRef& ref, char* smem, const LdsPlan& lp, uint32_t& cachedCall,
                                         float& cachedCutoff, const uint32_t par, const bool staged, const bool firstItem, Prefetch prefetch) {
    constexpr int NACC = Fmt<FMT>::kAcc;
    constexpr int TILE_F = NACC * E * 64;
    constexpr int TILE_L = Fmt<FMT>::kSlots * E * 64;
    constexpr int NT = 64 * W;
    constexpr int VPT = 4096 / NT;
    constexpr int KB = batch_rows<E>();

    const uint32_t ci = __builtin_amdgcn_readfirstlane(ref.ci), s = __builtin_amdgcn_readfirstlane(ref.s), t = __builtin_amdgcn_readfirstlane(ref.t);
    const CallDesc& a = ga.call[ci];
    const MulGeom& g = ga.geom[a.geom];
    float* const a_slabs = ga.slabs + (size_t)a.slabOff * 64u;
    uint32_t* const a_counters = ga.counters + a.tileOff;
    uint32_t* const a_sliceCounts = ga.sliceCounts + a.sliceOff;
    float* const a_cutoff = ga.cutoff + ci;
    (void)item;

    int tid0 = threadIdx.x;
    asm volatile("" : "+v"(tid0));
    const int tid = tid0, lane = tid & 63;
#if defined(EFFORT_NO_STAMPS) || defined(EFFORT_CUT_FINE)
    const bool wstamp = false;
#else
    const bool wstamp = GA_TSTAMP(ga) && tid == 0;
#endif
    unsigned long long ph[6] = {0, 0, 0, 0, 0, 0};
    if (wstamp) ph[0] = wall_clock64();
#ifdef EFFORT_CUT_FINE
    const bool stampCut = GA_TSTAMP(ga) && item == 0 && tid == 0, stamp = false;
#define EFFORT_PSTAMP(i) if (stampCut) GA_TSTAMP(ga)[26 + (i)] = clock64();
#else
#define EFFORT_PSTAMP(i)
    const bool stamp = GA_TSTAMP(ga) && item == 0 && tid == 0;
    const bool stampCut = stamp;
#endif
    if (stamp) GA_TSTAMP(ga)[16] = wall_clock64();
    const int wave = __builtin_amdgcn_readfirstlane(tid >> 6);
    const uint32_t B = g.sliceRows;
    const uint32_t offC = __builtin_amdgcn_readfirstlane(lp.offC), offL = __builtin_amdgcn_readfirstlane(lp.offL), offM = __builtin_amdgcn_readfirstlane(lp.offM);
    const uint32_t offA = __builtin_amdgcn_readfirstlane(lp.offA);
    int* acc = reinterpret_cast<int*>(smem + offA);
    float* vblk = reinterpret_cast<float*>(smem + __builtin_amdgcn_readfirstlane((par & 1u) ? lp.offV[1] : lp.offV[0]));
    uint32_t* flags = reinterpret_cast<uint32_t*>(smem + offC + 1280);
    float* wbound = reinterpret_cast<float*>(smem + offC + 1344);
    uint16_t* list = reinterpret_cast<uint16_t*>(smem + offL);
    const uint32_t* m32 = reinterpret_cast<const uint32_t*>(smem + offM);
    const float* means = reinterpret_cast<const float*>(smem + offM);

    const uint32_t j0 = s * B;
    uint32_t vSlabOff = (s * g.tiles + t) * (uint32_t)(TILE_F * 4), vSlabBytes = (uint32_t)min((size_t)0xFFFFFFFFu, (size_t)g.slices * g.tiles * TILE_F * 4);
    uint32_t vSlices = g.slices, vSliceStride = g.tiles * (uint32_t)(TILE_F * 4);
    if constexpr (!PERSIST) asm volatile("" : "+v"(vSlabOff), "+v"(vSlabBytes), "+v"(vSlices), "+v"(vSliceStride));
    const uint32_t nb = min(B, g.inDim - j0);
    const uint32_t e = a.expNo ? a.expNo[0] : 0u;

    EFFORT_PSTAMP(1)
    if (!staged) stage_issue<FMT, W, COMPACT>(ga, ref, tid, smem, lp, par);
    EFFORT_PSTAMP(2)
    constexpr bool kPreZero = !PERSIST;
    if constexpr (kPreZero) cutoff_table_zero<NT>(reinterpret_cast<uint32_t*>(smem + offA), tid);
    constexpr bool kOlMerge = FMT != kFp16 && W == 8 && (!PERSIST || kProductOnly);
    const uint32_t olPer = ol_outputs_per_item<E>(g);
    bool olAny = false, olEarly = false;
    uint32_t olParts = 1u, olStride = 0u;
    uint32_t olBFirst = 0u, olNB = 0u;
    float olVx[kOlMerge ? 8 : 1]; uint32_t olMeta0 = 0u, olBeg0 = 0u, olEnd0 = 0u;
    auto ol_share = [&]() {
        const uint32_t oBeg = min(t * (uint32_t)TILE_F + s * olPer, g.outDim);
        const uint32_t oEnd = max(oBeg, min(min(t * (uint32_t)TILE_F + (s + 1u) * olPer, (t + 1u) * (uint32_t)TILE_F), g.outDim));
        olBFirst = oBeg >> 6; olNB = ((oEnd + 63u) >> 6) - olBFirst;
        olParts = (olNB && olNB < (uint32_t)W) ? (uint32_t)W / olNB : 1u;
        olStride = olNB * 64u;
    };
    if constexpr (FMT != kFp16) {
        olAny = a.ol.blockPtr != nullptr;
        if (olAny) {
            if constexpr (kOlMerge) {
                ol_share();
                olEarly = g.inDim <= kOlEarlyFloats && lp.offO != 0u;
                if (olEarly) {
                    if constexpr (FUSED) {
                        if (a.pre == (uint16_t)kPreNone) {
#pragma unroll
                            for (int u = 0; u < 8; u++) olVx[u] = a.v[min((uint32_t)(u * NT + tid), g.inDim - 1u)];
                        }
                    } else {
#pragma unroll
                    for (int u = 0; u < 8; u++) olVx[u] = a.v[min((uint32_t)(u * NT + tid), g.inDim - 1u)];
                    }
                    if ((uint32_t)wave < olNB * olParts) {
                        const uint32_t bq = (uint32_t)wave / olParts;
                        olMeta0 = a.ol.meta[(size_t)(olBFirst + bq) * 64u + (uint32_t)lane];
                        olBeg0 = a.ol.blockPtr[olBFirst + bq]; olEnd0 = a.ol.blockPtr[olBFirst + bq + 1u];
                    }
                }
            }
        }
    }
    const float rankBound = a.rankBound[e];
    float vj[VPT]; uint16_t prj[VPT];
    const uint16_t* pr = a.probes + (size_t)e * kProbes;
    const bool fused = (ga.split & 1u) == 0u;
#pragma unroll
    for (int i = 0; i < VPT; i++) { vj[i] = 0.0f; prj[i] = 0; }
    const bool needCut = fused && cachedCall != ci;
    const bool viaJob = needCut && GA_CUTJOBS(ga) != 0u && !firstItem;
    const uint32_t pre = FUSED ? (uint32_t)a.pre : (uint32_t)kPreNone;
    float rawn[VPT]; uint32_t auxc[VPT]; uint32_t auxS = 0u;
    uint32_t auxS1 = 0u;
    const bool preAny = FUSED && pre != (uint32_t)kPreNone;
    const bool needCutEarly = fused && cachedCall != ci;
#pragma unroll
    for (int i = 0; i < VPT; i++) { rawn[i] = 0.0f; auxc[i] = 0u; }
    if (preAny) {
        const bool gate = pre == (uint32_t)kPreSiluGate;
        if (needCutEarly || !gate) {
#pragma unroll
            for (int i = 0; i < VPT; i++) rawn[i] = *(a.v + tid + NT * i);
        }
        if (needCutEarly) {
#pragma unroll
            for (int i = 0; i < VPT; i++) {
                auxc[i] = gate ? __float_as_uint(*(reinterpret_cast<const float*>(a.vAux) + tid + NT * i)) : (uint32_t)reinterpret_cast<const uint16_t*>(a.vAux)[tid + NT * i];
                prj[i] = pr[tid + NT * i];
            }
        }
        const uint32_t js = j0 + min((uint32_t)tid, nb - 1u);
        auxS = gate ? __float_as_uint(*(reinterpret_cast<const float*>(a.vAux) + js)) : (uint32_t)reinterpret_cast<const uint16_t*>(a.vAux)[js];
        if constexpr (FUSED && FMT != kFp16) {
            const uint32_t js1 = j0 + min((uint32_t)(tid + NT), nb - 1u);
            auxS1 = gate ? __float_as_uint(*(reinterpret_cast<const float*>(a.vAux) + js1)) : (uint32_t)reinterpret_cast<const uint16_t*>(a.vAux)[js1];
            if (olEarly && !needCutEarly) {
                if (gate) {
#pragma unroll
                    for (int i = 0; i < VPT; i++) rawn[i] = *(a.v + tid + NT * i);
                }
#pragma unroll
                for (int i = 0; i < VPT; i++)
                    auxc[i] = gate ? __float_as_uint(*(reinterpret_cast<const float*>(a.vAux) + tid + NT * i)) : (uint32_t)reinterpret_cast<const uint16_t*>(a.vAux)[tid + NT * i];
            }
        }
    }
    const uint32_t lg = g.sliceLog2;
    const uint32_t nSlots = FMT == kFp16 ? (g.rowsPerIn << lg) : (nb << 3);
    float normInv = 1.0f;
    if (FUSED && pre == kPreRmsNorm) {
        constexpr int R = 1024 / NT;
        static_assert(R >= 1 && R * NT == 1024 && R * W == 16, "fused rmsNorm: the workgroup must divide add_rmsnorm_mul_kernel's 1024 threads");
        float part[R];
#pragma unroll
        for (int r = 0; r < R; r++) part[r] = 0.0f;
#pragma unroll
        for (int i = 0; i < VPT; i++) part[i % R] += rawn[i] * rawn[i];
        for (uint32_t base = 4096u + (uint32_t)tid; base < g.inDim; base += 1024u) {
#pragma unroll
            for (int r = 0; r < R; r++) {
                const uint32_t j = base + (uint32_t)(r * NT);
                if (j < g.inDim) { const float x = *(a.v + j); part[r] += x * x; }
            }
        }
#pragma unroll
        for (int r = 0; r < R; r++) {
            part[r] = wave_sum_f32(part[r]);
            if (lane == 0) wbound[r * W + wave] = part[r];
        }
        __syncthreads();
        float tot = 0.0f;
#pragma unroll
        for (int w2 = 0; w2 < 16; w2++) tot += wbound[w2];
        normInv = 1.0f / sqrtf(tot / (float)g.inDim + 1e-5f);
        __syncthreads();
    }
    auto xform = [&](float x, uint32_t aux) -> float {
        if (!FUSED) return x;
        if (pre == kPreSiluGate) return __uint_as_float(aux) * x / (1.0f + expf(-x));
        if (pre == kPreRmsNorm) return (x * normInv) * half_bits_to_float((uint16_t)aux);
        return x;
    };
    auto load_cut_inputs = [&]() {
        if (preAny) {
#pragma unroll
            for (int i = 0; i < VPT; i++) vj[i] = xform(rawn[i], auxc[i]);
        } else {
#pragma unroll
            for (int i = 0; i < VPT; i++) { vj[i] = *(a.v + tid + NT * i); prj[i] = pr[tid + NT * i]; }
        }
    };
    if constexpr (kPreZero) {
        asm volatile("s_waitcnt lgkmcnt(0)" ::: "memory");
        __builtin_amdgcn_s_barrier();
    }
    if (needCut && !viaJob) load_cut_inputs();
    EFFORT_PSTAMP(3)
    uint32_t* const cutWords = ga.queue + 9 * 16;
    uint32_t cutWord = 0;
    if (viaJob && tid == 0 && !(GA_ABLATE(ga) & 32u)) cutWord = __hip_atomic_load(&cutWords[ci], __ATOMIC_RELAXED, __HIP_MEMORY_SCOPE_AGENT);
    asm volatile("s_waitcnt vmcnt(0)" ::: "memory");
    EFFORT_PSTAMP(4)
    uint32_t vColOK = 0, voff = 0, vRecords = 0, vBuckLo = 0, vBuckHi = 0, vRowPitch = 0, vInDim = 0, vRow0 = 0;
    auto stream_geom = [&]() {
        const uint32_t col = t * (64u * E) + (uint32_t)lane * E;
        vColOK = col < g.cols ? 1u : 0u;
        voff = (vColOK ? col : (g.cols - 1u) / (uint32_t)E * (uint32_t)E) * 2u;
        vRecords = (uint32_t)min((size_t)0xFFFFFFFFu, (size_t)g.numExperts * g.expertRows * g.rowPitch - (size_t)a.bucketsTrim);
        vBuckLo = (uint32_t)(size_t)a.buckets; vBuckHi = (uint32_t)((size_t)a.buckets >> 32);
        vRowPitch = g.rowPitch; vInDim = g.inDim; vRow0 = e * g.expertRows + (FMT == kFp16 ? j0 : j0 * 8u);
    };
    if constexpr (!PERSIST) {
        stream_geom();
        asm volatile("" : "+v"(vColOK), "+v"(voff), "+v"(vRecords), "+v"(vBuckLo), "+v"(vBuckHi), "+v"(vRowPitch), "+v"(vInDim), "+v"(vRow0));
    }
    if constexpr (kOlMerge) {
        if (olEarly) {
            float* const vf = reinterpret_cast<float*>(smem + __builtin_amdgcn_readfirstlane(lp.offO));
#pragma unroll
            for (int u = 0; u < 8; u++) {
                if constexpr (FUSED) { if ((uint32_t)(u * NT + tid) < g.inDim) vf[u * NT + tid] = preAny ? xform(rawn[u % VPT], auxc[u % VPT]) : olVx[u]; }
                else if ((uint32_t)(u * NT + tid) < g.inDim) vf[u * NT + tid] = olVx[u];
            }
        }
    }
    float bound = 0.0f;
#pragma unroll
    for (int u = 0; u < (FMT == kFp16 ? 1 : 2); u++) {
        const uint32_t jl = tid + u * NT;
        if (jl < nb) {
            float x = vblk[jl];
            if constexpr (FUSED && FMT != kFp16) { if (preAny) { x = xform(x, u ? auxS1 : auxS); vblk[jl] = x; } }
            else
            if (preAny) { x = xform(x, auxS); vblk[jl] = x; }
            bound += fabsf(x);
        }
    }
    bound = wave_sum_f32(bound);
    if (lane == 0) wbound[wave] = bound;
    if (tid == 0) { flags[4] = 0u; flags[5] = (uint32_t)(W * KB); }
    if (stamp) GA_TSTAMP(ga)[17] = wall_clock64();
    if (wstamp) ph[1] = wall_clock64();

    uint32_t* tbl = reinterpret_cast<uint32_t*>(smem + offA);
    float cutoff;
    bool fromJob = false;
    if (viaJob) {
        if (tid == 0) {
            for (int spin = 0; spin < ((GA_ABLATE(ga) & 32u) ? 0 : 20000) && !(cutWord >> 31); spin++) {
                __builtin_amdgcn_s_sleep(8);
                cutWord = __hip_atomic_load(&cutWords[ci], __ATOMIC_RELAXED, __HIP_MEMORY_SCOPE_AGENT);
            }
            flags[2] = cutWord >> 31;
            flags[3] = cutWord & 0x7FFFFFFFu;
        }
        __syncthreads();
        fromJob = flags[2] != 0u;
        if (fromJob) { cutoff = __uint_as_float(flags[3]); cachedCall = ci; cachedCutoff = cutoff; }
        else load_cut_inputs();
    }
    if (fromJob) {
    } else if (needCut) {
        cutoff = block_find_cutoff<NT, kPreZero>(vj, prj, a.q, smem + offC, tbl, []() {}, stampCut ? GA_TSTAMP(ga) + 8 : nullptr);
        cachedCall = ci; cachedCutoff = cutoff;
    } else if (fused) {
        cutoff = cachedCutoff;
        __syncthreads();
    } else {
        cutoff = a_cutoff[0];
        __syncthreads();
    }
    const uint32_t slotCap = __builtin_amdgcn_readfirstlane((lp.offV[0] - lp.offM) / 4u) - 1u;
    const uint16_t* m16 = reinterpret_cast<const uint16_t*>(m32);
    auto load_block = [&](int blk, uint32_t (&mraw)[4], float (&vq)[4]) {
#pragma unroll
        for (int u = 0; u < 4; u++) {
            const uint32_t c = min((uint32_t)((blk * 4 + u) * NT + tid), slotCap);
            if constexpr (COMPACT && FMT == kFp16) { mraw[u] = (uint32_t)m16[c] << 16; vq[u] = 0.0f; }
            else { mraw[u] = m32[c]; vq[u] = FMT != kFp16 ? vblk[min(c >> 3, nb - 1u)] : 0.0f; }
        }
    };
    uint32_t mraw0[4]; float vq0[4];
    load_block(0, mraw0, vq0);
    const uint32_t jlSel = (uint32_t)tid & ((1u << lg) - 1u);
    float axRaw = 0.0f;
    if (FMT == kFp16) axRaw = vblk[min(jlSel, nb - 1u)];
    float wb[W];
#pragma unroll
    for (int w2 = 0; w2 < W; w2++) wb[w2] = wbound[w2];
    __builtin_amdgcn_sched_barrier(0);
    for (int i = tid; i < TILE_L; i += NT) acc[i] = 0;
    float L = 0.0f;
#pragma unroll
    for (int w2 = 0; w2 < W; w2++) L += wb[w2];
    L *= rankBound;
    int kexp = 30 - (int)((__float_as_uint(L) >> 23) & 0xFFu) + 126;
    kexp = L > 0.0f ? max(-100, min(100, kexp)) : 0;
    const float scale = __uint_as_float((uint32_t)(127 + kexp) << 23), unscale = __uint_as_float((uint32_t)(127 - kexp) << 23);
    if (stamp) GA_TSTAMP(ga)[18] = wall_clock64();
    if (wstamp) ph[2] = wall_clock64();

#if defined(EFFORT_PAD_TEST) && EFFORT_PAD_TEST == 1
    if (ga.numCU == 0xdeadu) asm volatile(".rept 6000\n s_nop 0\n .endr" ::: "memory");
#elif defined(EFFORT_PAD_TEST) && EFFORT_PAD_TEST == 2
    asm volatile(".rept 1000\n s_nop 0\n .endr" ::: "memory");
#endif
    const float ax = (FMT == kFp16 && jlSel < nb) ? fabsf(axRaw) : 0.0f;
    const bool sel = !(GA_ABLATE(ga) & 8u);
    uint32_t keepMask = 0;
    uint32_t before[kRounds];
    uint32_t wtot = 0;
#pragma unroll
    for (int blk = 0; blk < kRounds / 4; blk++) {
        if (blk > 0 && (uint32_t)(blk * 4 * NT) >= nSlots) {
#pragma unroll
            for (int u = 0; u < 4; u++) before[blk * 4 + u] = wtot;
            continue;
        }
        uint32_t mraw[4]; float vq[4];
        if (blk == 0) {
#pragma unroll
            for (int u = 0; u < 4; u++) { mraw[u] = mraw0[u]; vq[u] = vq0[u]; }
        } else {
            load_block(blk, mraw, vq);
        }
#pragma unroll
        for (int u = 0; u < 4; u++) {
            const int rr = blk * 4 + u;
            before[rr] = wtot;
            const uint32_t c = rr * NT + tid;
            bool k;
            if (FMT == kFp16) k = (cutoff < (kCutoffScale * half_bits_to_float((uint16_t)(mraw[u] >> 16))) * ax) & ((c >> lg) < g.rowsPerIn) & sel;
            else k = (cutoff < (kCutoffScale * __uint_as_float(mraw[u])) * fabsf(vq[u])) & (c < nSlots) & sel;
            keepMask |= k ? (1u << rr) : 0u;
            wtot += (uint32_t)__popcll(__ballot(k));
        }
    }
    uint32_t wbase = 0;
    if (lane == 0) wbase = atomicAdd(&flags[4], wtot);
    wbase = __builtin_amdgcn_readfirstlane(wbase);
#pragma unroll
    for (int rr = 0; rr < kRounds; rr++) {
        if ((uint32_t)(rr * NT) >= nSlots) break;
        const uint32_t c = rr * NT + tid;
        const bool k = (keepMask >> rr) & 1u;
        const unsigned long long m = __ballot(k);
        const uint32_t pos = wbase + before[rr] + __builtin_amdgcn_mbcnt_hi((uint32_t)(m >> 32), __builtin_amdgcn_mbcnt_lo((uint32_t)m, 0u));
        if (k) list[pos] = (uint16_t)(FMT == kFp16 ? (((c >> lg) << 12) | (c & ((1u << lg) - 1u))) : c);
    }
    __syncthreads();
    const uint32_t n = flags[4];
    const uint32_t code0 = list[(uint32_t)(wave * KB) + ((uint32_t)lane & (uint32_t)(KB - 1))];
    if (t == 0 && tid == 0) a_sliceCounts[s] = n;
    if (stamp) GA_TSTAMP(ga)[19] = wall_clock64();
    if (wstamp) ph[3] = wall_clock64();

    if constexpr (PERSIST) stream_geom();
    const bool colOK = vColOK != 0u;
    const __amdgpu_buffer_rsrc_t rsrc = __builtin_amdgcn_make_buffer_rsrc(
        reinterpret_cast<uint16_t*>((size_t)(uint32_t)__builtin_amdgcn_readfirstlane(vBuckLo) | ((size_t)(uint32_t)__builtin_amdgcn_readfirstlane(vBuckHi) << 32)), 0,
        (int)__builtin_amdgcn_readfirstlane(vRecords), 0x00020000);
    const uint32_t nU = (GA_ABLATE(ga) & 4u) ? 0u : __builtin_amdgcn_readfirstlane(n);
    uint32_t* const cursor = flags + 5;
    auto grab = [&]() -> uint32_t {
        uint32_t bq = 0;
        if (lane == 0) bq = atomicAdd(cursor, (uint32_t)KB);
        return __builtin_amdgcn_readfirstlane(bq);
    };

    auto decode_code = [&](uint32_t code, uint32_t& boff, float& dv) {
        {
            uint32_t rowIdx;
            if (FMT == kFp16) { const uint32_t rank = code >> 12, jl = code & 4095u; rowIdx = rank * vInDim + jl; dv = vblk[jl] * scale; }
            else {
                rowIdx = code;
                dv = __int_as_float(__float2int_rn((vblk[code >> 3] * means[code]) * scale));
            }
            boff = (vRow0 + rowIdx) * vRowPitch;
        }
    };
    auto decode = [&](uint32_t i0, uint32_t& boff, float& dv) {
        boff = 0; dv = 0.0f;
        if (lane < KB && nU) decode_code(list[min(i0 + (uint32_t)lane, nU - 1u)], boff, dv);
    };
    auto decode_first = [&](uint32_t i0, uint32_t& boff, float& dv) {
        boff = 0; dv = 0.0f;
        if (lane < KB && nU) decode_code(i0 + (uint32_t)lane < nU ? code0 : (uint32_t)__builtin_amdgcn_readfirstlane((int)code0), boff, dv);
    };
    auto issue = [&](auto aux, Piece<E> (&piece)[KB], uint32_t boff) {
#pragma unroll
        for (int u = 0; u < KB; u++) piece[u].template load<decltype(aux)::value>(rsrc, voff, EFFORT_ABLATE_NOLOAD ? 0u : __builtin_amdgcn_readlane(boff, u));
    };
    using lds_i = __attribute__((address_space(3))) int;
    const uint32_t accB = (uint32_t)(size_t)(lds_i*)(acc + lane);
    constexpr int kShift = (E == 1 ? 8 : E == 2 ? 9 : 10);
    auto row = [&](const Piece<E>& pc, float dd) {
        if (FMT == kFp16) {
#pragma unroll
            for (int j = 0; j < E; j++) {
                const uint32_t dw = pc.dword(j);
                uint32_t a2; int qv;
                asm("v_bfe_u32 %0, %1, %2, 4\n\tv_lshl_add_u32 %0, %0, %3, %4" : "=&v"(a2) : "v"(dw), "n"(16 * (j & 1)), "n"(kShift), "v"(accB));
                if (j & 1) asm("v_fma_mix_f32 %0, %1, %2, 0 op_sel:[0,1,0] op_sel_hi:[0,1,0]\n\tv_cvt_rpi_i32_f32 %0, %0" : "=v"(qv) : "v"(dd), "v"(dw));
                else asm("v_fma_mix_f32 %0, %1, %2, 0 op_sel_hi:[0,1,0]\n\tv_cvt_rpi_i32_f32 %0, %0" : "=v"(qv) : "v"(dd), "v"(dw));
                __hip_atomic_fetch_add((lds_i*)(size_t)a2 + j * 64, qv, __ATOMIC_RELAXED, __HIP_MEMORY_SCOPE_WORKGROUP);
            }
        } else {
            const int di = __float_as_int(dd);
#pragma unroll
            for (int j = 0; j < E; j++) {
                const uint32_t x = pc.word(j);
#pragma unroll
                for (int q = 0; q < 4; q++) {
                    uint32_t a2;
                    asm("v_bfe_u32 %0, %1, %2, 4\n\tv_lshl_add_u32 %0, %0, %3, %4" : "=&v"(a2) : "v"(x), "n"(4 * q), "n"(kShift), "v"(accB));
                    __hip_atomic_fetch_add((lds_i*)(size_t)a2 + ((3 - q) * 16 * E + j) * 64, di, __ATOMIC_RELAXED, __HIP_MEMORY_SCOPE_WORKGROUP);
                }
            }
        }
    };
    auto accumulate = [&](const Piece<E> (&piece)[KB], float dv, uint32_t nv) {
        if (EFFORT_ABLATE_NOSCATTER) {
#pragma unroll
            for (int u = 0; u < KB; u++) asm volatile("" ::"v"(piece[u].word(E - 1)), "v"(dv));
            return;
        }
        if (!colOK) return;
        if (nv == (uint32_t)KB) {
#pragma unroll
            for (int u = 0; u < KB; u++) row(piece[u], __uint_as_float(__builtin_amdgcn_readlane(__float_as_uint(dv), u)));
        } else {
#pragma unroll
            for (int u = 0; u < KB; u++)
                if ((uint32_t)u < nv) row(piece[u], __uint_as_float(__builtin_amdgcn_readlane(__float_as_uint(dv), u)));
        }
    };

    bool asked = false;
    using lds_f = __attribute__((address_space(3))) float;
    uint32_t olLen = 0u, olOut = 0u, olKa = 0u, olKf = 0u, olK1 = 0u, olCur = 0u, olSlot = 0xFFFFFFFFu;
    float olAcc = 0.0f;
    const lds_f* olV = nullptr;
    if constexpr (kOlMerge) {
        if (olEarly) {
            olV = (const lds_f*)(size_t)(uint32_t)(size_t)(__attribute__((address_space(3))) void*)(smem + __builtin_amdgcn_readfirstlane(lp.offO));
            if ((uint32_t)wave < olNB * olParts) {
                const uint32_t bq = (uint32_t)wave / olParts, part = (uint32_t)wave % olParts;
                olLen = olMeta0 >> 8; olOut = olMeta0 & 63u;
                const uint32_t olLenAll = olLen;
                const uint32_t maxLen = (uint32_t)__builtin_amdgcn_readfirstlane((int)olLen);
                const uint32_t chunk = (maxLen + olParts - 1u) / olParts, k0 = min(maxLen, part * chunk);
                const uint32_t bBeg = __builtin_amdgcn_readfirstlane(olBeg0), bEnd = __builtin_amdgcn_readfirstlane(olEnd0);
                olK1 = bEnd > bBeg ? min(maxLen, k0 + chunk) : k0;
                olKa = olKf = k0;
                olCur = bBeg + wave_sum_u32(min(olLenAll, k0));
                olLen = min(olLenAll, olK1);
                olSlot = part * olStride + bq * 64u + olOut;
            }
        }
    }
    auto ol_fma = [](float x, uint32_t ent, float acc) -> float {
        float r;
        asm("v_fma_mix_f32 %0, %1, %2, %3 op_sel:[0,1,0] op_sel_hi:[0,1,0]" : "=v"(r) : "v"(x), "v"(ent), "v"(acc));
        return r;
    };
    auto ol_fetch = [&](uint32_t (&ent)[kOlMerged]) {
#pragma unroll
        for (int u = 0; u < kOlMerged; u++) {
            ent[u] = EFFORT_OL_LOAD((a.ol.entry + olCur) + lane);
            olCur += (uint32_t)__popcll(__ballot(olLen > olKf + (uint32_t)u));
        }
        olKf += (uint32_t)kOlMerged;
    };
    auto ol_add = [&](const uint32_t (&ent)[kOlMerged]) {
        float x[kOlMerged];
#pragma unroll
        for (int u = 0; u < kOlMerged; u++) x[u] = olV[ent[u] & 0xFFFFu];
#pragma unroll
        for (int u = 0; u < kOlMerged; u++)
            { const float r = ol_fma(x[u], ent[u], olAcc); olAcc = olLen > olKa + (uint32_t)u ? r : olAcc; }
        olKa += (uint32_t)kOlMerged;
    };
    auto stream_rows = [&](auto withOl, auto aux) {
        constexpr bool OL = decltype(withOl)::value;
        Piece<E> pa[KB], pb[KB];
        uint32_t entA[OL ? kOlMerged : 1], entB[OL ? kOlMerged : 1];
        uint32_t boffA, boffB; float dvA, dvB;
        uint32_t baseA = (uint32_t)(wave * KB), baseB;
        if (baseA < nU) { decode_first(baseA, boffA, dvA); issue(aux, pa, boffA); }
        if constexpr (OL) ol_fetch(entA);
        while (baseA < nU) {
            if (!asked && nU - baseA <= 4u * KB * W) asked = prefetch();
            if (wstamp && GA_TRACE(ga) && item + GA_CUTJOBS(ga) < (uint32_t)kTraceItems) {
                const uint32_t q0 = (4u * baseA) / nU, q1 = min(4u, (4u * (baseA + 2u * KB * W)) / nU);
                for (uint32_t q = q0 + 1u; q <= q1 && q < 4u; q++) GA_TSTAMP(ga)[kTraceOff + (size_t)kTraceItems * 8u + (size_t)(item + GA_CUTJOBS(ga)) * 4u + q - 1u] = wall_clock64();
            }
            baseB = grab();
            decode(baseB, boffB, dvB);
            issue(aux, pb, boffB);
            if constexpr (OL) ol_fetch(entB);
            accumulate(pa, dvA, __builtin_amdgcn_readfirstlane(min((uint32_t)KB, nU - baseA)));
            if constexpr (OL) ol_add(entA);
            baseA = grab();
            decode(baseA, boffA, dvA);
            issue(aux, pa, boffA);
            if constexpr (OL) ol_fetch(entA);
            accumulate(pb, dvB, __builtin_amdgcn_readfirstlane(baseB < nU ? min((uint32_t)KB, nU - baseB) : 0u));
            if constexpr (OL) ol_add(entB);
        }
        if constexpr (OL) {
            while (olKa < olK1) {
                ol_fetch(entB); ol_add(entA);
                if (olKa >= olK1) break;
                ol_fetch(entA); ol_add(entB);
            }
        }
    };
    constexpr bool kRowSwitch = kRowAux != 0 && (PERSIST || E == 4);
    const bool rowsReused = kRowSwitch && (ga.split & 8u) != 0u;
    auto stream = [&](auto withOl) {
        if constexpr (kRowSwitch) { if (rowsReused) { stream_rows(withOl, std::integral_constant<int, 0>{}); return; } }
        stream_rows(withOl, std::integral_constant<int, kRowAux>{});
    };
    if constexpr (kOlMerge) { if (olEarly) stream(std::true_type{}); else stream(std::false_type{}); }
    else stream(std::false_type{});
    if (!asked) asked = prefetch();
    __syncthreads();
    if (stamp) GA_TSTAMP(ga)[20] = wall_clock64();
    if (wstamp) ph[4] = wall_clock64();

    float* const olsum = reinterpret_cast<float*>(smem + offM);
    if constexpr (FMT != kFp16) {
        if (olAny) {
            const OutlierIndex& ol = a.ol;
            float* const vfull = olEarly ? reinterpret_cast<float*>(smem + __builtin_amdgcn_readfirstlane(lp.offO)) : olsum + (olPer > kOlSumFloats ? olPer : kOlSumFloats);
            const bool vLds = g.inDim <= kOlLdsFloats;
            if constexpr (!kOlMerge) ol_share();
            const uint32_t bFirst = olBFirst, nB = olNB, parts = olParts;
            if (vLds && !olEarly) {
                for (uint32_t i0 = 0; i0 < g.inDim; i0 += NT * 8u) {
                    float x[8];
#pragma unroll
                    for (int u = 0; u < 8; u++) x[u] = a.v[min(i0 + u * NT + tid, g.inDim - 1u)];
                    if constexpr (FUSED) {
                        uint32_t xa[8];
#pragma unroll
                        for (int u = 0; u < 8; u++) xa[u] = 0u;
                        if (preAny) {
#pragma unroll
                            for (int u = 0; u < 8; u++) {
                                const uint32_t i = min(i0 + u * NT + tid, g.inDim - 1u);
                                xa[u] = pre == (uint32_t)kPreSiluGate ? __float_as_uint(*(reinterpret_cast<const float*>(a.vAux) + i)) : (uint32_t)reinterpret_cast<const uint16_t*>(a.vAux)[i];
                            }
                        }
#pragma unroll
                        for (int u = 0; u < 8; u++) {
                            const uint32_t i = i0 + u * NT + tid;
                            if (i < g.inDim) vfull[i] = preAny ? xform(x[u], xa[u]) : x[u];
                        }
                    } else
#pragma unroll
                    for (int u = 0; u < 8; u++) {
                        const uint32_t i = i0 + u * NT + tid;
                        if (i < g.inDim) vfull[i] = x[u];
                    }
                }
                __syncthreads();
            }
            if (olSlot != 0xFFFFFFFFu) olsum[olSlot] = olAcc;
            const lds_f* const vfullL = (const lds_f*)(size_t)(uint32_t)(size_t)(__attribute__((address_space(3))) void*)vfull;
            auto run_blocks = [&](auto fromLds) {
                for (uint32_t q = (uint32_t)wave + (olEarly ? (uint32_t)W : 0u); q < nB * parts; q += (uint32_t)W) {
                    const uint32_t bq = q / parts, part = q % parts;
                    const uint32_t meta = ol.meta[(size_t)(bFirst + bq) * 64u + (uint32_t)lane];
                    const uint32_t lenAll = meta >> 8, myOut = meta & 63u;
                    const uint32_t maxLen = (uint32_t)__builtin_amdgcn_readfirstlane((int)lenAll);
                    const uint32_t chunk = (maxLen + parts - 1u) / parts, k0 = min(maxLen, part * chunk), k1 = min(maxLen, k0 + chunk);
                    const uint32_t myLen = min(lenAll, k1);
                    const uint32_t bBeg = __builtin_amdgcn_readfirstlane(ol.blockPtr[bFirst + bq]), bEnd = __builtin_amdgcn_readfirstlane(ol.blockPtr[bFirst + bq + 1u]);
                    uint32_t cur = bBeg + wave_sum_u32(min(lenAll, k0));
                    float acc = 0.0f;
                    auto fetch = [&](uint32_t (&ent)[kOlBatch], uint32_t kk) {
#pragma unroll
                        for (int u = 0; u < kOlBatch; u++) {
                            ent[u] = EFFORT_OL_LOAD((ol.entry + cur) + lane);
                            cur += (uint32_t)__popcll(__ballot(myLen > kk + (uint32_t)u));
                        }
                    };
                    auto add = [&](const uint32_t (&ent)[kOlBatch], uint32_t kk) {
                        float x[kOlBatch];
#pragma unroll
                        for (int u = 0; u < kOlBatch; u++) {
                            const uint32_t in = ent[u] & 0xFFFFu;
                            if constexpr (decltype(fromLds)::value) x[u] = vfullL[in]; else x[u] = a.v[in];
                        }
#pragma unroll
                        for (int u = 0; u < kOlBatch; u++)
                            { const float r = ol_fma(x[u], ent[u], acc); acc = myLen > kk + (uint32_t)u ? r : acc; }
                    };
                    if (k0 < k1 && bEnd > bBeg) {
                        uint32_t entA[kOlBatch], entB[kOlBatch];
                        uint32_t kk = k0;
                        fetch(entA, kk);
                        for (;;) {
                            const bool more = kk + (uint32_t)kOlBatch < k1;
                            if (more) fetch(entB, kk + (uint32_t)kOlBatch);
                            add(entA, kk);
                            if (!more) break;
                            kk += (uint32_t)kOlBatch;
                            const bool more2 = kk + (uint32_t)kOlBatch < k1;
                            if (more2) fetch(entA, kk + (uint32_t)kOlBatch);
                            add(entB, kk);
                            if (!more2) break;
                            kk += (uint32_t)kOlBatch;
                        }
                    }
                    olsum[part * olStride + bq * 64u + myOut] = acc;
                }
            };
            if (vLds) run_blocks(std::true_type{}); else run_blocks(std::false_type{});
            __syncthreads();
        }
    }

    const __amdgpu_buffer_rsrc_t srs = __builtin_amdgcn_make_buffer_rsrc(a_slabs, 0, (int)__builtin_amdgcn_readfirstlane(vSlabBytes), 0x00020000);
    const uint32_t slabOff = __builtin_amdgcn_readfirstlane(vSlabOff);
    const uint32_t nSlices = __builtin_amdgcn_readfirstlane(vSlices);
    auto tile_out = [&](int o) -> float {
        if (FMT == kFp16) return (float)acc[o] * unscale;
        const int slot = o / (E * 64), rem = o % (E * 64);
        const int p = (((slot >> 3) * 16 + (slot & 7)) * E * 64) + rem;
        float r = (float)(acc[p] - acc[p + 8 * E * 64]) * unscale;
        if (olAny) {
            const uint32_t ol_o = (uint32_t)((rem & 63) * E + (rem >> 6)) * 32u + (uint32_t)slot - s * olPer;
            if (ol_o < olPer && (uint32_t)(t * TILE_F) + s * olPer + ol_o < g.outDim) {
                float so = olsum[ol_o];
                for (uint32_t pp = 1; pp < olParts; pp++) so += olsum[pp * olStride + ol_o];
                r += so;
            }
        }
        return r;
    };
    if (fused && t == 0 && s == 0 && tid == 0 && !GA_CUTJOBS(ga)) a_cutoff[0] = cutoff;
    {
        constexpr int kIt = (TILE_F + NT * 2 - 1) / (NT * 2);
        float s0[kIt], s1[kIt];
#pragma unroll
        for (int it = 0; it < kIt; it++) {
            const int o = min(tid * 2 + it * NT * 2, TILE_F - 2);
            s0[it] = tile_out(o); s1[it] = tile_out(o + 1);
        }
#pragma unroll
        for (int it = 0; it < kIt; it++) {
            const int o = tid * 2 + it * NT * 2;
            if (TILE_F % (NT * 2) != 0 && o >= TILE_F) continue;
            typedef uint32_t u2 __attribute__((ext_vector_type(2)));
            u2 pk; pk[0] = __float_as_uint(s0[it]); pk[1] = __float_as_uint(s1[it]);
            __builtin_amdgcn_raw_buffer_store_b64(pk, srs, (uint32_t)o * 4u, slabOff, kSc1);
        }
    }
    asm volatile("s_waitcnt vmcnt(0)" ::: "memory");
    if (stamp) { GA_TSTAMP(ga)[21] = wall_clock64(); GA_TSTAMP(ga)[22] = n; }
    if (wstamp) ph[5] = wall_clock64();
    auto flush_stamps = [&]() {
#ifndef EFFORT_PRODUCT_ONLY
        if (!wstamp) return;
        if (GA_TRACE(ga) && item + GA_CUTJOBS(ga) < (uint32_t)kTraceItems) {
            unsigned long long* rec = GA_TSTAMP(ga) + kTraceOff + (size_t)(item + GA_CUTJOBS(ga)) * 8u;
            rec[0] = (unsigned long long)(item + GA_CUTJOBS(ga)) | ((unsigned long long)blockIdx.x << 32);
            rec[1] = (unsigned long long)(__builtin_amdgcn_s_getreg((31 << 11) | 20) & 0xFu) | ((unsigned long long)(ci & 0xFu) << 4) | ((unsigned long long)(n & 0xFFFFu) << 8) | ((unsigned long long)(t & 0xFFu) << 24) |
                     ((unsigned long long)__builtin_amdgcn_s_getreg((31 << 11) | 4) << 32);
#pragma unroll
            for (int i = 0; i < 6; i++) rec[2 + i] = ph[i];
        }
        unsigned long long* line = GA_TSTAMP(ga) + 64 + (item & 31u) * 8u;
#pragma unroll
        for (int i = 0; i < 5; i++) atomicAdd(&line[i], ph[i + 1] - ph[i]);
        atomicAdd(&line[5], 1ull);
        atomicMin(&GA_TSTAMP(ga)[0], ph[0]);
        atomicMax(&GA_TSTAMP(ga)[26], ph[0]);
        atomicMax(&GA_TSTAMP(ga)[28], ph[5] - ph[0]);
        atomicMax(&GA_TSTAMP(ga)[29], ph[4] - ph[3]);
        atomicMax(&GA_TSTAMP(ga)[1], (unsigned long long)wall_clock64());
#endif
    };
    {
        __syncthreads();
        if (tid == 0) {
            const uint32_t ticket = __hip_atomic_fetch_add(&a_counters[t], 1u, __ATOMIC_RELAXED, __HIP_MEMORY_SCOPE_AGENT);
            flags[0] = (ticket == nSlices - 1u) ? 1u : 0u;
        }
        __syncthreads();
        if (flags[0] == 0u) { flush_stamps(); return; }
    }
    if (GA_ABLATE(ga) & 2u) { if (tid == 0) __hip_atomic_store(&a_counters[t], 0u, __ATOMIC_RELAXED, __HIP_MEMORY_SCOPE_AGENT); return; }

    const bool rstamp = GA_TSTAMP(ga) && ci == 0 && t == 0 && tid == 0;
    if (rstamp) GA_TSTAMP(ga)[23] = wall_clock64();
    typedef uint32_t u4v __attribute__((ext_vector_type(4)));
    const uint32_t sliceStride = __builtin_amdgcn_readfirstlane(vSliceStride);
    constexpr int kCols4 = TILE_F / 4;
    constexpr int G = NT / kCols4 >= 2 ? NT / kCols4 : 1;
    float* const gpart = reinterpret_cast<float*>(smem + offA + (uint32_t)TILE_L * 4u);
    static_assert(G == 1 || (uint32_t)TILE_L * 4u + (uint32_t)G * TILE_F * 4u <= (cutoff_table_bytes(NT) > (uint32_t)TILE_L * 4u ? cutoff_table_bytes(NT) : (uint32_t)TILE_L * 4u),
                  "the thread groups' partial sums must fit behind the tile");
    auto reduce_tile = [&](auto kc) {
        constexpr int kRed = decltype(kc)::value;
        const int grp = G > 1 ? tid / kCols4 : 0;
        const uint32_t per = G > 1 ? ((nSlices + G - 1) / G + 3u) / 4u * 4u : nSlices;
        const uint32_t sl0 = (uint32_t)grp * per, sl1 = min(nSlices, sl0 + per);
        for (int o = (G > 1 ? tid % kCols4 : tid) * 4; o < TILE_F; o += (G > 1 ? kCols4 : NT) * 4) {
            const uint32_t vo = t * (uint32_t)(TILE_F * 4) + (uint32_t)o * 4u;
            float res[4] = {0.0f, 0.0f, 0.0f, 0.0f};
            if (FUSED && a.resid && (G == 1 || grp == 0)) {
#pragma unroll
                for (int h = 0; h < 4; h++) {
                    const uint32_t oo = (uint32_t)o + h, lane2 = oo & 63u, sj = oo >> 6, j = sj % E, slot = sj / E;
                    const uint32_t c2 = t * (64u * E) + lane2 * E + j;
                    if (c2 < g.cols) res[h] = *(a.resid + c2 * NACC + slot);
                }
            }
            float sm[4][4];
#pragma unroll
            for (int h = 0; h < 4; h++) { sm[h][0] = 0.0f; sm[h][1] = 0.0f; sm[h][2] = 0.0f; sm[h][3] = 0.0f; }
            for (uint32_t sl = sl0; sl < sl1; sl += kRed) {
                u4v r[kRed];
#pragma unroll
                for (int i = 0; i < kRed; i++)
                    r[i] = __builtin_amdgcn_raw_buffer_load_b128(srs, vo, min(sl + i, nSlices - 1u) * sliceStride, kSc1);
#pragma unroll
                for (int i = 0; i < kRed; i++) {
                    if (sl + i < sl1) {
#pragma unroll
                        for (int h = 0; h < 4; h++) sm[h][i & 3] += __uint_as_float(r[i][h]);
                    }
                }
            }
            float tot[4];
#pragma unroll
            for (int h = 0; h < 4; h++) tot[h] = (sm[h][0] + sm[h][1]) + (sm[h][2] + sm[h][3]);
            if (G > 1) {
#pragma unroll
                for (int h = 0; h < 4; h++) gpart[grp * TILE_F + o + h] = tot[h];
                __syncthreads();
                if (grp != 0) continue;
#pragma unroll
                for (int h = 0; h < 4; h++) {
                    tot[h] = gpart[o + h];
                    for (int g2 = 1; g2 < G; g2++) tot[h] += gpart[g2 * TILE_F + o + h];
                }
            }
#pragma unroll
            for (int h = 0; h < 4; h++) {
                const uint32_t oo = (uint32_t)o + h;
                const uint32_t lane2 = oo & 63u, sj = oo >> 6, j = sj % E, slot = sj / E;
                const uint32_t c2 = t * (64u * E) + lane2 * E + j;
                if (c2 < g.cols) {
                    const uint32_t oi = c2 * NACC + slot;
                    const float val = (FUSED && a.resid) ? res[h] + tot[h] : tot[h];
                    a.out[oi] = val;
                }
            }
        }
    };
    if (nSlices <= 8u * G) reduce_tile(std::integral_constant<int, 8>{});
    else reduce_tile(std::integral_constant<int, 16>{});
    if (PERSIST && G > 1) __syncthreads();
    if (rstamp) GA_TSTAMP(ga)[24] = wall_clock64();
    if (tid == 0) {
        __hip_atomic_store(&a_counters[t], 0u, __ATOMIC_RELAXED, __HIP_MEMORY_SCOPE_AGENT);
#if !defined(EFFORT_CUT_FINE) && !defined(EFFORT_PRODUCT_ONLY)
        if (GA_TSTAMP(ga)) {
            flush_stamps();
            const uint32_t done = __hip_atomic_fetch_add(ga.groupDone, 1u, __ATOMIC_RELAXED, __HIP_MEMORY_SCOPE_AGENT);
            if (done == ga.totalTiles - 1u) {
                const unsigned long long t0 = __hip_atomic_load(&GA_TSTAMP(ga)[0], __ATOMIC_RELAXED, __HIP_MEMORY_SCOPE_AGENT);
                const unsigned long long t1 = __hip_atomic_load(&GA_TSTAMP(ga)[1], __ATOMIC_RELAXED, __HIP_MEMORY_SCOPE_AGENT);
                GA_TSTAMP(ga)[2] += t1 - t0; GA_TSTAMP(ga)[3] += 1;
                GA_TSTAMP(ga)[27] += __hip_atomic_load(&GA_TSTAMP(ga)[26], __ATOMIC_RELAXED, __HIP_MEMORY_SCOPE_AGENT) - t0;
                __hip_atomic_store(&GA_TSTAMP(ga)[26], 0ull, __ATOMIC_RELAXED, __HIP_MEMORY_SCOPE_AGENT);
                __hip_atomic_store(&GA_TSTAMP(ga)[0], ~0ull, __ATOMIC_RELAXED, __HIP_MEMORY_SCOPE_AGENT);
                __hip_atomic_store(&GA_TSTAMP(ga)[1], 0ull, __ATOMIC_RELAXED, __HIP_MEMORY_SCOPE_AGENT);
                __hip_atomic_store(ga.groupDone, 0u, __ATOMIC_RELAXED, __HIP_MEMORY_SCOPE_AGENT);
            }
        }
#endif
    }
}

template <int NT>
__device__ __forceinline__ void cutoff_job(const GroupKArgs& ga, uint32_t ci, char* smem) {
    constexpr int VPT = 4096 / NT;
    const CallDesc& a = ga.call[ci];
    int tid0 = threadIdx.x;
    asm volatile("" : "+v"(tid0));
    const int tid = tid0;
    const uint32_t e = a.expNo ? a.expNo[0] : 0u;
    const uint16_t* pr = a.probes + (size_t)e * kProbes;
    float vj[VPT]; uint16_t prj[VPT];
#pragma unroll
    for (int i = 0; i < VPT; i++) { vj[i] = a.v[tid + NT * i]; prj[i] = pr[tid + NT * i]; }
    [[maybe_unused]] constexpr bool PERSIST = true;
    const unsigned long long tj0 = (GA_TSTAMP(ga) && GA_TRACE(ga)) ? wall_clock64() : 0ull;
    const float cutoff = block_find_cutoff<NT>(vj, prj, a.q, smem + cutoff_table_bytes(NT), reinterpret_cast<uint32_t*>(smem), []() {}, nullptr);
    if (tid == 0 && GA_TSTAMP(ga) && GA_TRACE(ga)) {
        unsigned long long* rec = GA_TSTAMP(ga) + kTraceOff + (size_t)ci * 8u;
        rec[0] = (unsigned long long)ci | ((unsigned long long)blockIdx.x << 32) | (1ull << 63);
        rec[1] = (unsigned long long)__builtin_amdgcn_s_getreg((31 << 11) | 20) | ((unsigned long long)__builtin_amdgcn_s_getreg((31 << 11) | 4) << 32);
        rec[2] = tj0; rec[3] = wall_clock64();
    }
    if (tid == 0) {
        __hip_atomic_store(&ga.queue[9 * 16 + ci], __float_as_uint(cutoff) | 0x80000000u, __ATOMIC_RELAXED, __HIP_MEMORY_SCOPE_AGENT);
        __hip_atomic_store(reinterpret_cast<uint32_t*>(ga.cutoff + ci), __float_as_uint(cutoff), __ATOMIC_RELAXED, __HIP_MEMORY_SCOPE_AGENT);
    }
    __syncthreads();
}

template <int FMT, int E, int W, bool FUSED, bool COMPACT = false, bool PERSIST = true>
__global__ __launch_bounds__(64 * W, (FUSED && FMT != kFp16 && W == 2 ? 2 : W <= 8 ? EFFORT_MIN_WAVES_PER_EU : 4)) void bucket_mul_kernel(const GroupKArgs ga) {
    extern __shared__ __attribute__((aligned(16))) char smem[];
    __shared__ uint32_t s_item;
    __shared__ unsigned long long s_next;
#ifdef EFFORT_CUT_FINE
    if (GA_TSTAMP(ga) && blockIdx.x == 0 && threadIdx.x == 0) GA_TSTAMP(ga)[26] = clock64();
#endif
#ifndef EFFORT_NO_TOUCH
    if constexpr (!PERSIST) {
        const uint32_t* const kw = reinterpret_cast<const uint32_t*>(&ga);
        uint32_t touch[12];
#pragma unroll
        for (int i = 0; i < 12; i++) touch[i] = kw[i * 16];
#pragma unroll
        for (int i = 0; i < 12; i++) asm volatile("" :: "s"(touch[i]));
    }
#endif
#ifdef EFFORT_CUT_FINE
#define EFFORT_ESTAMP(i) if (GA_TSTAMP(ga) && blockIdx.x == 0 && threadIdx.x == 0) GA_TSTAMP(ga)[16 + (i)] = clock64();
#else
#define EFFORT_ESTAMP(i)
#endif
    EFFORT_ESTAMP(0)
#ifdef EFFORT_Q4_STAGGER_US
    const uint32_t staggerSleeps = (uint32_t)((EFFORT_Q4_STAGGER_US) * 10 / 9);
#else
    const uint32_t staggerSleeps = ga.staggerSleeps;
#endif
    if constexpr (PERSIST) {
        if (GA_PERSISTENT(ga) && staggerSleeps && blockIdx.x >= ga.numCU)
            for (uint32_t i = 0; i < staggerSleeps; i++) __builtin_amdgcn_s_sleep(32);
    }
    const uint32_t total = ga.totalItems + GA_CUTJOBS(ga);
    uint32_t cachedCall = 0xFFFFFFFFu; float cachedCutoff = 0.0f;
    const uint32_t x = blockIdx.x & 7u;
    uint32_t dry = 0;
    auto pull = [&]() -> uint32_t {
        uint32_t got = total;
        for (uint32_t tries = 0; tries < 8u && got >= total; tries++) {
            const uint32_t q = (x + tries) & 7u;
            if ((dry >> q) & 1u) continue;
            const uint32_t cand = __hip_atomic_fetch_add(&ga.queue[q * 16u], 1u, __ATOMIC_RELAXED, __HIP_MEMORY_SCOPE_AGENT) * 8u + q;
            if (cand < total) got = cand; else dry |= 1u << q;
            if (GA_ABLATE(ga) & 64u) break;
        }
        return got;
    };
    auto pull_sync = [&]() -> uint32_t {
        if (threadIdx.x == 0) s_item = pull();
        __syncthreads();
        const uint32_t it = __builtin_amdgcn_readfirstlane(s_item);
        __syncthreads();
        return it;
    };
    constexpr bool kPipe = !FUSED && FMT == kFp16;
    const LdsPlan lp = ga.lp;
    uint32_t par = 0;
    bool staged = false;
    uint32_t gen = 0;
    if (threadIdx.x == 0) __hip_atomic_store(&s_next, 0ull, __ATOMIC_RELAXED, __HIP_MEMORY_SCOPE_WORKGROUP);
    uint32_t item = GA_PERSISTENT(ga) ? pull_sync() : blockIdx.x;
    while (item < total) {
        if (item < GA_CUTJOBS(ga)) {
            if (item < ga.count) cutoff_job<64 * W>(ga, item, smem);
            item = GA_PERSISTENT(ga) ? pull_sync() : total;
            continue;
        }
        ItemRef ref;
        EFFORT_ESTAMP(1)
        if (!locate_item(ga, item - GA_CUTJOBS(ga), ref)) {
            item = GA_PERSISTENT(ga) ? pull_sync() : total;
            continue;
        }
        EFFORT_ESTAMP(2)
        gen++;
        bool stagedNext = false;
        auto prefetch = [&]() -> bool {
            if (!GA_PERSISTENT(ga)) return true;
            if (threadIdx.x == 0)
                __hip_atomic_store(&s_next, ((unsigned long long)gen << 32) | (unsigned long long)pull(), __ATOMIC_RELAXED, __HIP_MEMORY_SCOPE_WORKGROUP);
            const unsigned long long nx = __hip_atomic_load(&s_next, __ATOMIC_RELAXED, __HIP_MEMORY_SCOPE_WORKGROUP);
            if (__builtin_amdgcn_readfirstlane((uint32_t)(nx >> 32)) != gen) return false;
            const uint32_t next = __builtin_amdgcn_readfirstlane((uint32_t)nx);
            ItemRef nref;
            if (kPipe && !(GA_ABLATE(ga) & 128u) && next >= GA_CUTJOBS(ga) && next < total && locate_item(ga, next - GA_CUTJOBS(ga), nref)) {
                int tid0 = threadIdx.x;
                asm volatile("" : "+v"(tid0));
                stage_issue<FMT, W, COMPACT>(ga, nref, tid0, smem, lp, par ^ 1u);
                stagedNext = true;
            }
            return true;
        };
        const bool firstOwn = gen == 1u && (GA_ABLATE(ga) & 512u) != 0u;
        mul_item<FMT, E, W, FUSED, COMPACT, PERSIST>(ga, item - GA_CUTJOBS(ga), ref, smem, lp, cachedCall, cachedCutoff, par, staged, firstOwn, prefetch);
        item = GA_PERSISTENT(ga) ? __builtin_amdgcn_readfirstlane((uint32_t)__hip_atomic_load(&s_next, __ATOMIC_RELAXED, __HIP_MEMORY_SCOPE_WORKGROUP)) : total;
        staged = stagedNext;
        par ^= 1u;
    }
    if (GA_PERSISTENT(ga) && threadIdx.x == 0) {
        const uint32_t gone = __hip_atomic_fetch_add(&ga.queue[8 * 16], 1u, __ATOMIC_RELAXED, __HIP_MEMORY_SCOPE_AGENT);
        if (gone == gridDim.x - 1u) {
            for (int i = 0; i <= 8; i++) __hip_atomic_store(&ga.queue[i * 16], 0u, __ATOMIC_RELAXED, __HIP_MEMORY_SCOPE_AGENT);
            for (int i = 0; i < kMaxGroup; i++) __hip_atomic_store(&ga.queue[9 * 16 + i], 0u, __ATOMIC_RELAXED, __HIP_MEMORY_SCOPE_AGENT);
        }
    }
}

template <int FMT, int E, int W>
static hipError_t launch_mul_t(const GroupKArgs& gaIn, hipStream_t st) {
    GroupKArgs ga = gaIn;
    constexpr bool kLean = W == 8;
#ifdef EFFORT_LEAN_STAMPS
    const bool lean = kLean && !ga.persistent && !ga.ablate;
#else
    const bool lean = kLean && !ga.persistent && !ga.tstamp && !ga.ablate;
#endif
    const LdsPlan lp = ga.lp = plan_lds<FMT, E, W>(ga.geom, kMaxGeoms, lean || (kLean && kProductOnly));
    uint32_t lds = lp.total;
    if (lp.offA > 65536u && FMT == kFp16) return hipErrorInvalidValue;
    for (uint32_t i = 0; i < ga.count; i++) {
        const MulGeom& g = ga.geom[ga.call[i].geom];
        if (g.slots > (uint32_t)kRounds * 64 * W || g.slots != (FMT == kFp16 ? (g.rowsPerIn << g.sliceLog2) : g.sliceRows * 8u)) return hipErrorInvalidValue;
        if (FMT == kFp16 ? (1u << g.sliceLog2) > 64u * W : g.sliceRows > 128u * W) return hipErrorInvalidValue;
        if (((uint32_t)ga.wgEnd8[i] - (i ? (uint32_t)ga.wgEnd8[i - 1] : 0u)) * 8u != align_up(g.tiles * g.slices, 8)) return hipErrorInvalidValue;
    }
    if (ga.totalItems != (uint32_t)ga.wgEnd8[ga.count - 1] * 8u) return hipErrorInvalidValue;
    uint32_t grid = ga.totalItems;
    if (ga.persistent) {
        const uint32_t R = ga.persistent;
        grid = ga.numCU * R;
        const uint32_t force = (160u * 1024u) / (R + 1u) + 512u;
        if (lds < force && force <= (160u * 1024u) / R) lds = force;
    }
    bool fusedAny = false;
    for (uint32_t i = 0; i < ga.count; i++) fusedAny = fusedAny || ga.call[i].pre || ga.call[i].resid;
    for (uint32_t i = 0; FMT != kFp16 && i < ga.count; i++)
        if (ga.call[i].pre && ga.call[i].ol.blockPtr && ga.geom[ga.call[i].geom].inDim > kOlLdsFloats) return hipErrorInvalidValue;
    if (lds > kMaxLdsBytes) return hipErrorInvalidValue;
    const bool compact = (ga.split & 4u) != 0u;
    if (compact && (FMT != kFp16 || (fusedAny && !lean))) return hipErrorInvalidValue;
    const dim3 gd(grid), bd(64 * W);
    if constexpr (kLean) {
        if (lean && compact && fusedAny) { hipLaunchKernelGGL((bucket_mul_kernel<kFp16, E, W, true, true, false>), gd, bd, lds, st, ga); return hipGetLastError(); }
        if (lean && compact) { hipLaunchKernelGGL((bucket_mul_kernel<kFp16, E, W, false, true, false>), gd, bd, lds, st, ga); return hipGetLastError(); }
        if (lean && fusedAny) { hipLaunchKernelGGL((bucket_mul_kernel<FMT, E, W, true, false, false>), gd, bd, lds, st, ga); return hipGetLastError(); }
        if (lean) { hipLaunchKernelGGL((bucket_mul_kernel<FMT, E, W, false, false, false>), gd, bd, lds, st, ga); return hipGetLastError(); }
    }
    if (fusedAny) hipLaunchKernelGGL((bucket_mul_kernel<FMT, E, W, true>), gd, bd, lds, st, ga);
    else if (compact) hipLaunchKernelGGL((bucket_mul_kernel<kFp16, E, W, false, true>), gd, bd, lds, st, ga);
    else hipLaunchKernelGGL((bucket_mul_kernel<FMT, E, W, false>), gd, bd, lds, st, ga);
    return hipGetLastError();
}

#define EFFORT_GEOMS(X) X(16, 1) X(16, 2) X(16, 4) X(8, 1) X(8, 2) X(8, 4) X(4, 1) X(4, 2) X(4, 4) X(2, 4)

template <int FMT, int E, int W>
static hipError_t prepare_t() {
    auto set = [&](const void* f) {
        hipFuncAttributes fa;
        hipError_t e = hipFuncGetAttributes(&fa, f);
        if (e != hipSuccess) return e;
        if (fa.sharedSizeBytes > 1024u) return hipErrorInvalidValue;
        return hipFuncSetAttribute(f, hipFuncAttributeMaxDynamicSharedMemorySize, (int)(160u * 1024u - (uint32_t)fa.sharedSizeBytes));
    };
    constexpr bool kLean = W == 8;
    hipError_t err = set(reinterpret_cast<const void*>(&bucket_mul_kernel<FMT, E, W, false>));
    if constexpr (kLean) if (err == hipSuccess) err = set(reinterpret_cast<const void*>(&bucket_mul_kernel<FMT, E, W, false, false, false>));
    if constexpr (FMT != kFp16) {
        if (err == hipSuccess) err = set(reinterpret_cast<const void*>(&bucket_mul_kernel<FMT, E, W, true>));
        if constexpr (kLean) if (err == hipSuccess) err = set(reinterpret_cast<const void*>(&bucket_mul_kernel<FMT, E, W, true, false, false>));
    }
    if constexpr (FMT == kFp16) {
        if (err == hipSuccess) err = set(reinterpret_cast<const void*>(&bucket_mul_kernel<kFp16, E, W, true>));
        if (err == hipSuccess) err = set(reinterpret_cast<const void*>(&bucket_mul_kernel<kFp16, E, W, false, true>));
        if constexpr (kLean) if (err == hipSuccess) err = set(reinterpret_cast<const void*>(&bucket_mul_kernel<kFp16, E, W, true, false, false>));
        if constexpr (kLean) if (err == hipSuccess) err = set(reinterpret_cast<const void*>(&bucket_mul_kernel<kFp16, E, W, false, true, false>));
        if constexpr (kLean) if (err == hipSuccess) err = set(reinterpret_cast<const void*>(&bucket_mul_kernel<kFp16, E, W, true, true, false>));
    }
    return err;
}
hipError_t bucket_mul_prepare_device() {
    hipError_t err = hipSuccess;
#define EFFORT_CASE(w, e) if (err == hipSuccess) err = prepare_t<kFp16, e, w>(); if (err == hipSuccess) err = prepare_t<kQ4, e, w>();
    EFFORT_GEOMS(EFFORT_CASE)
#undef EFFORT_CASE
    return err;
}

template <int FMT>
static hipError_t launch_mul_fmt(int W, int E, const GroupKArgs& a, hipStream_t st) {
#define EFFORT_CASE(w, e) if (W == w && E == e) return launch_mul_t<FMT, e, w>(a, st);
    EFFORT_GEOMS(EFFORT_CASE)
#undef EFFORT_CASE
    return hipErrorInvalidValue;
}

hipError_t launch_bucket_mul(Format fmt, int W, int E, const GroupKArgs& a, hipStream_t st) {
    return fmt == kFp16 ? launch_mul_fmt<kFp16>(W, E, a, st) : launch_mul_fmt<kQ4>(W, E, a, st);
}

size_t bucket_mul_lds_bytes(Format fmt, int W, int E, const MulGeom& g, bool lean) {
#define EFFORT_CASE(w, e)                                                                     \
    if (W == w && E == e)                                                                     \
        return fmt == kFp16 ? plan_lds<kFp16, e, w>(&g, 1, lean).total : plan_lds<kQ4, e, w>(&g, 1, lean).total;
    EFFORT_GEOMS(EFFORT_CASE)
#undef EFFORT_CASE
    return 0;
}

int bucket_mul_occupancy(Format fmt, int W, int E, size_t ldsBytes) {
    int n = 0;
#define EFFORT_CASE(w, e)                                                                                              \
    if (W == w && E == e) {                                                                                            \
        const void* f = fmt == kFp16 ? reinterpret_cast<const void*>(&bucket_mul_kernel<kFp16, e, w, false>)                  \
                                     : reinterpret_cast<const void*>(&bucket_mul_kernel<kQ4, e, w, false>);                   \
        if (hipOccupancyMaxActiveBlocksPerMultiprocessor(&n, f, 64 * w, ldsBytes) != hipSuccess) n = 0;                \
    }
    EFFORT_GEOMS(EFFORT_CASE)
#undef EFFORT_CASE
    return n;
}

uint32_t bucket_mul_ol_lds_floats() { return kOlLdsFloats; }

uint32_t bucket_mul_max_candidates(int W) { return (uint32_t)kRounds * 64u * (uint32_t)W; }

}
```

### effort_amd/csrc/plan.h

```cpp
#pragma once
#include "effort_internal.h"

namespace effort {

constexpr int kMaxLaunches = kMaxGroup / kMaxGeoms + 1;

struct PlanEnv {
    int numCU = 256, nLanes = 1;
    bool laned = false;
    int persistent = -1;
    int tuneW = 0, tuneE = 0, tuneS = 0;
    bool splitCutoff = false, clock = false;
    uint32_t ablate = 0;
    bool noJobs = false, noCompact = false;
    size_t slabBytes = 0;
    uint32_t maxTiles = 0, maxSlices = 0;
    bool thinEffort = false;
    int tailCalls = 0, tailMult = 0;
};
struct PlanCall {
    uint32_t inDim, outDim, cols, rowsPerIn, rowPitch, numExperts;
    bool hasMeans16;
    uint16_t pre;
    bool hasResid;
};
struct CallPlan {
    MulGeom g;
    uint32_t mult;
    uint32_t launch, geom;
    uint32_t slabOff, tileOff, sliceOff;
    uint32_t itemEnd8;
};
struct LaunchPlan {
    uint32_t first, count;
    uint32_t persistent, cutJobs, staggerSleeps;
    bool compact;
    uint32_t totalItems, totalTiles, realItems;
};
struct GroupPlan {
    int W = 0, E = 0;
    int err = 0;
    const char* msg = "";
    uint32_t nLaunches = 0;
    CallPlan call[kMaxGroup];
    LaunchPlan launch[kMaxLaunches];
};

bool supported(int W, int E);
int plan_group(Format fmt, const PlanEnv& env, int n, const PlanCall* calls, GroupPlan* plan);

}
```

### effort_amd/csrc/plan.hip

```cpp
#include <cstring>

#include "../../include/effort_hip.h"
#include "plan.h"

namespace effort {

static uint32_t round8(uint32_t x) { return (x + 7u) / 8u * 8u; }
static uint32_t min_slices(uint32_t inDim) { return round8((inDim + 511u) / 512u); }
static uint32_t max_slices(uint32_t inDim) { return round8((inDim + 127u) / 128u); }
static uint32_t tiles_at(const PlanCall& w, int E) { return (w.cols + 64 * E - 1) / (64 * E); }
static uint32_t group_tiles(int n, const PlanCall* ws, int E) {
    uint32_t t = 0;
    for (int i = 0; i < n; i++) t += tiles_at(ws[i], E);
    return t;
}
static uint32_t padded_items(uint32_t tiles, uint32_t slices) { return round8(tiles * slices); }
static uint32_t padded_min_items(int n, const PlanCall* ws, int E) {
    uint32_t t = 0;
    for (int i = 0; i < n; i++) t += padded_items(tiles_at(ws[i], E), min_slices(ws[i].inDim));
    return t;
}
static bool fits_one_round(const PlanEnv& env, int n, uint32_t tiles, uint32_t allTiles, uint32_t s) {
    const bool same = allTiles == (uint32_t)n * tiles;
    return (same ? (uint32_t)n * padded_items(tiles, s) : allTiles * s + 7u * (uint32_t)n) <= (uint32_t)env.numCU;
}

bool supported(int W, int E) {
    return (W == 16 && (E == 1 || E == 2 || E == 4)) || (W == 8 && (E == 1 || E == 2 || E == 4)) ||
           (W == 4 && (E == 1 || E == 2 || E == 4)) || (W == 2 && E == 4);
}

static uint32_t q4_one_round(const PlanEnv& env, uint32_t inDim, uint32_t groupTiles1) {
    if (env.nLanes > 1 || env.tuneS || !groupTiles1) return 0;
    const uint32_t sMin = (inDim + 831u) / 832u;
    const uint32_t S = (uint32_t)env.numCU * 15u / 8u / groupTiles1;
    return S >= sMin && S >= 2u ? S : 0u;
}
static uint32_t q4_one_per_cu(const PlanEnv& env, uint32_t inDim, uint32_t tiles1, int n, uint32_t groupTiles1) {
    if (env.nLanes > 1 || env.tuneS || n < 3 || n > 9) return 0;
    const uint32_t sMin = (inDim + 831u) / 832u, hi = max_slices(inDim);
    auto fits = [&](uint32_t s) { return fits_one_round(env, n, tiles1, groupTiles1 ? groupTiles1 : (uint32_t)n * tiles1, s); };
    uint32_t S = sMin > 2u ? sMin : 2u;
    if (!fits(S)) return 0;
    const uint32_t top = env.thinEffort ? min_slices(inDim) : hi;
    while (S < top && S < hi && fits(S + 1u)) S++;
    return S;
}
static uint32_t pick_slices(const PlanEnv& env, Format fmt, const PlanCall& w, int groupSize, int E, uint32_t groupTiles = 0, bool fill = true) {
    const uint32_t tiles = tiles_at(w, E);
    const uint32_t lo = min_slices(w.inDim), hi = max_slices(w.inDim);
    if (fmt != kFp16 && (E == 1 || groupSize >= 8) && fill) {
        const uint32_t S = q4_one_per_cu(env, w.inDim, tiles, groupSize, groupTiles);
        if (S) return S;
    }
    if (fmt != kFp16 && E == 1 && groupSize >= 8 && groupTiles) {
        const uint32_t S = q4_one_round(env, w.inDim, groupTiles);
        if (S) return S;
    }
    if (groupSize >= 8 && (fmt != kFp16 || !fill || env.nLanes > 1 || env.thinEffort)) return lo;
    const uint32_t target = (E == 1 && fmt == kFp16) ? (uint32_t)env.numCU : (uint32_t)env.numCU * 3u / 4u;
    const uint32_t allTiles = groupTiles ? groupTiles : (uint32_t)groupSize * tiles;
    uint32_t S = (target / allTiles + 4u) / 8u * 8u;
    if (S < lo) S = lo;
    if (S > hi) S = hi;
    if ((w.inDim & (w.inDim - 1u)) == 0u && (S & (S - 1u)) != 0u) {
        uint32_t up = 8u;
        while (up < S) up <<= 1;
        S = up <= hi ? up : up >> 1;
    }
    if (fmt == kFp16 && fill && groupSize >= 3 && env.nLanes <= 1) {
        auto fits = [&](uint32_t s) { return fits_one_round(env, groupSize, tiles, allTiles, s); };
        if (fits(S)) { if (!env.thinEffort) while (S < hi && fits(S + 1u)) S++; }
        else {
            uint32_t s2 = S;
            while (s2 > lo && !fits(s2)) s2--;
            if (fits(s2)) S = s2;
        }
    }
    return S;
}

static int pick_elems(const PlanEnv& env, Format fmt, int n, const PlanCall* ws) {
    if (env.tuneE) return env.tuneE;
    if (fmt != kFp16) {
        if (n < 8) return 1;
        uint32_t inMax = 0;
        for (int i = 0; i < n; i++) inMax = inMax > ws[i].inDim ? inMax : ws[i].inDim;
        if (n < 10) {
            uint32_t tMax = 0;
            bool same = true;
            for (int i = 0; i < n; i++) {
                const uint32_t t = tiles_at(ws[i], 1);
                same = same && (tMax == 0 || t == tMax); tMax = tMax > t ? tMax : t;
            }
            if (q4_one_per_cu(env, inMax, tMax, n, same ? 0u : group_tiles(n, ws, 1))) return 1;
        }
        if (n >= 10) {
            if (q4_one_round(env, inMax, group_tiles(n, ws, 1))) return 1;
        }
        return 2;
    }
    if (env.tuneS) return 2;
    auto items = [&](int E) {
        uint32_t t = 0;
        const uint32_t gt = group_tiles(n, ws, E);
        for (int i = 0; i < n; i++) t += tiles_at(ws[i], E) * pick_slices(env, fmt, ws[i], n, E, gt, false);
        return t;
    };
    const uint32_t numCU = (uint32_t)env.numCU;
    auto only_wide_tiles_fit = [&] { return padded_min_items(n, ws, 1) > numCU && padded_min_items(n, ws, 2) <= numCU; };
    auto fill = [&](int E) {
        double used = 0, have = 0;
        for (int i = 0; i < n; i++) { used += ws[i].cols; have += (double)tiles_at(ws[i], E) * 64 * E; }
        return have > 0 ? used / have : 1.0;
    };
    const double f1 = fill(1), f2 = fill(2), f4 = fill(4), best = f1 > f2 ? (f1 > f4 ? f1 : f4) : (f2 > f4 ? f2 : f4);
    if (n >= 8) {
        const uint32_t i4 = items(4);
        if (((i4 > numCU / 2 && i4 <= numCU) || i4 >= 3u * numCU) && f4 >= 0.8 * best) return 4;
        if (f2 >= 0.8 * best) return 2;
        if (env.nLanes <= 1 && f2 >= 0.7 * best && only_wide_tiles_fit()) return 2;
        return 1;
    }
    const uint32_t i2 = items(2);
    if (f2 < 0.8 * best) return 1;
    if (n >= 3 && f4 >= 0.8 * best && env.nLanes <= 1) {
        uint32_t lo2 = 0, lo4 = 0;
        for (int i = 0; i < n; i++) {
            const uint32_t lo = min_slices(ws[i].inDim);
            lo2 += tiles_at(ws[i], 2) * lo; lo4 += tiles_at(ws[i], 4) * lo;
        }
        if (lo2 > numCU && lo4 <= numCU * 15u / 16u) return 4;
    }
    bool narrow = true;
    for (int i = 0; i < n; i++) narrow = narrow && ws[i].cols <= 256u;
    if (narrow && f1 >= 0.8 * best && n >= 3 && env.nLanes <= 1 && f2 >= 0.8 * best && only_wide_tiles_fit()) return 2;
    if (narrow && f1 >= 0.8 * best && !(env.nLanes > 1 && n >= 3)) return 1;
    return (i2 * 10u < numCU * 3u / 4u * 6u && items(1) > i2) ? 1 : 2;
}

static uint32_t tile_floats(Format fmt, int E) { return (fmt == kFp16 ? 16u : 32u) * (uint32_t)E * 64u; }
static int choose_geom(const PlanEnv& env, Format fmt, const PlanCall& w, int groupSize, int W, int E, uint32_t groupTiles, uint32_t sliceMult, MulGeom* g) {
    memset(g, 0, sizeof(*g));
    g->inDim = w.inDim; g->outDim = w.outDim; g->cols = w.cols; g->rowsPerIn = w.rowsPerIn;
    g->expertRows = w.rowsPerIn * w.inDim; g->numExperts = w.numExperts;
    g->tiles = tiles_at(w, E);
    g->elems = (uint32_t)E;
    g->rowPitch = w.rowPitch;
    const uint32_t tileFloats = tile_floats(fmt, E);
    const size_t ldsMax = 160 * 1024;
    uint32_t S;
    if (env.tuneS) S = env.tuneS;
    else {
        const uint32_t want = pick_slices(env, fmt, w, groupSize, E, groupTiles) * sliceMult;
        const uint32_t cap = (env.numCU * 2u) / g->tiles / 8 * 8;
        S = cap < want ? cap : want;
    }
    if (S > w.inDim) S = w.inDim / 8 * 8;
    if (S < 1) S = 1;
    const uint32_t maxCand = bucket_mul_max_candidates(W);
    for (;;) {
        g->sliceRows = (w.inDim + S - 1) / S;
        g->slices = (w.inDim + g->sliceRows - 1) / g->sliceRows;
        g->sliceLog2 = 0; while ((1u << g->sliceLog2) < g->sliceRows) g->sliceLog2++;
        g->slots = fmt == kFp16 ? (g->rowsPerIn << g->sliceLog2) : g->sliceRows * 8u;
        const size_t lds = bucket_mul_lds_bytes(fmt, W, E, *g, true);
        const bool fits = lds <= ldsMax && g->slots <= maxCand && (size_t)g->slots * 4 + (size_t)g->sliceRows * 8 + 1024 <= 65536 &&
                          (fmt == kFp16 ? (1u << g->sliceLog2) <= 64u * (uint32_t)W : g->sliceRows <= 128u * (uint32_t)W);
        const size_t slab = (size_t)g->slices * g->tiles * tileFloats * 4;
        if (fits && slab <= env.slabBytes) break;
        if (!fits) { S += 1; if (S > w.inDim + 8) return EFFORT_ERR_SHAPE; }
        else return EFFORT_ERR_SHAPE;
    }
    return EFFORT_OK;
}
static int plan_fail(GroupPlan* P, int code, const char* msg) { P->err = code; P->msg = msg; return code; }

static uint32_t geom_index(MulGeom* geoms, uint32_t& n, const MulGeom& g) {
    uint32_t k = 0;
    while (k < n && memcmp(&geoms[k], &g, sizeof(g)) != 0) k++;
    if (k == n && n < (uint32_t)kMaxGeoms) geoms[n++] = g;
    return k;
}

static void finish_launch(Format fmt, const PlanEnv& env, int W, const PlanCall* ws, const GroupPlan* P, LaunchPlan* lp) {
    const uint32_t R = env.persistent < 0 ? 2u : (uint32_t)env.persistent;
    const uint32_t perCU = (env.persistent < 0 && fmt == kFp16 && !env.laned) ? 6u : R;
    lp->persistent = (R && lp->realItems > (uint32_t)env.numCU * perCU) ? R : 0u;
    bool plain = true;
    for (uint32_t i = 0; i < lp->count; i++) plain = plain && !ws[lp->first + i].pre;
    lp->cutJobs = (lp->persistent && !env.splitCutoff && plain && !env.noJobs) ? (lp->count + 7u) / 8u * 8u : 0u;
    const bool leanGrid = lp->persistent == 0u && W == 8 && !env.clock && !env.ablate;
    bool compact = fmt == kFp16 && !env.noCompact && (leanGrid || (lp->persistent != 0u && plain));
    for (uint32_t i = 0; compact && !leanGrid && i < lp->count; i++) compact = !ws[lp->first + i].hasResid;
    for (uint32_t i = 0; compact && i < lp->count; i++) {
        const MulGeom& g = P->call[lp->first + i].g;
        compact = ws[lp->first + i].hasMeans16 && g.inDim % 2u == 0u && g.sliceRows % 2u == 0u;
    }
    lp->compact = compact;
    lp->staggerSleeps = (lp->persistent && fmt == kQ4 && !env.laned) ? 11u : 0u;
}

int plan_group(Format fmt, const PlanEnv& env, int n, const PlanCall* ws, GroupPlan* P) {
    P->err = EFFORT_OK; P->msg = ""; P->nLaunches = 0;
    const bool laned = env.laned;
    const int W = env.tuneW ? env.tuneW : 8;
    const int E = pick_elems(env, fmt, n, ws);
    P->W = W; P->E = E;
    const char* const noGeometry = "bucketmul: no launch geometry for this shape/tuning";
    if (!supported(W, E)) return plan_fail(P, EFFORT_ERR_ARG, noGeometry);
    const uint32_t groupTiles = group_tiles(n, ws, E);
    MulGeom g1[kMaxGroup], g2[kMaxGroup];
    uint32_t it1[kMaxGroup], base = 0;
    for (int i = 0; i < n; i++) {
        const int rc = choose_geom(env, fmt, ws[i], n, W, E, groupTiles, 1, &g1[i]);
        if (rc != EFFORT_OK) return plan_fail(P, rc, noGeometry);
        it1[i] = padded_items(g1[i].tiles, g1[i].slices);
        base += it1[i];
    }
    int thinFrom = n;
    if (E == 2 && n >= 8 && !laned && !env.tuneS && env.persistent < 0 && !env.thinEffort) {
        const uint32_t round = 2u * (uint32_t)env.numCU, over = base % round;
        if (base > round && over != 0u && over * 32u <= round * 7u && (fmt != kFp16 || base <= 6u * (uint32_t)env.numCU)) {
            int tc = 0;
            uint32_t thin = 0;
            while (tc < n && tc < 4 && (tc < 2 || thin < over)) thin += it1[n - 1 - tc++];
            MulGeom seen[kMaxGeoms];
            uint32_t nSeen = 0, extra = 0;
            bool ok = thin >= over;
            for (int i = 0; ok && i < n; i++) {
                const bool t = i >= n - tc;
                if (t) {
                    ok = choose_geom(env, fmt, ws[i], n, W, E, groupTiles, 2, &g2[i]) == EFFORT_OK;
                    const uint32_t it2 = padded_items(g2[i].tiles, g2[i].slices);
                    ok = ok && it2 > it1[i];
                    extra += it2 - it1[i];
                }
                ok = ok && geom_index(seen, nSeen, t ? g2[i] : g1[i]) < (uint32_t)kMaxGeoms;
            }
            if (ok && (fmt != kFp16 || base + extra <= 6u * (uint32_t)env.numCU)) thinFrom = n - tc;
        }
    }
    uint32_t nGeoms = 0, wg = 0;
    MulGeom geoms[kMaxGeoms];
    size_t slabOff = 0; uint32_t tileOff = 0, sliceOff = 0;
    LaunchPlan* lp = nullptr;
    auto begin = [&](uint32_t firstCall) {
        lp = &P->launch[P->nLaunches++];
        memset(lp, 0, sizeof(*lp));
        lp->first = firstCall;
        nGeoms = 0; wg = 0;
    };
    begin(0);
    for (int i = 0; i < n; i++) {
        uint32_t mult = i >= thinFrom ? 2u : 1u;
        MulGeom g = mult == 2u ? g2[i] : g1[i];
        if (n >= 8 && !env.tuneS && env.tailMult) {
            mult = 1;
            if (i >= n - env.tailCalls) mult = (uint32_t)env.tailMult;
            if (env.tailMult >= 4 && i >= n - env.tailCalls && i < n - env.tailCalls / 2) mult = (uint32_t)env.tailMult / 2;
            const int rc = choose_geom(env, fmt, ws[i], n, W, E, groupTiles, mult, &g);
            if (rc != EFFORT_OK) return plan_fail(P, rc, noGeometry);
        }
        uint32_t gi = geom_index(geoms, nGeoms, g);
        if (gi == (uint32_t)kMaxGeoms) {
            finish_launch(fmt, env, W, ws, P, lp);
            begin((uint32_t)i);
            gi = geom_index(geoms, nGeoms, g);
        }
        CallPlan& a = P->call[i];
        const size_t slab = (size_t)g.slices * g.tiles * tile_floats(fmt, E) * 4;
        if (tileOff + g.tiles + 1 > env.maxTiles || sliceOff + g.slices > env.maxSlices || slabOff + slab > env.slabBytes)
            return plan_fail(P, EFFORT_ERR_SHAPE, "bucketmul: group exceeds the context scratch");
        a.g = g; a.mult = mult; a.launch = P->nLaunches - 1u; a.geom = gi;
        a.slabOff = (uint32_t)(slabOff / 256); a.tileOff = tileOff; a.sliceOff = sliceOff;
        wg += padded_items(g.tiles, g.slices);
        if (wg / 8u > 0xFFFFu) return plan_fail(P, EFFORT_ERR_SHAPE, "bucketmul: group exceeds the launch descriptor's item range");
        a.itemEnd8 = wg / 8u;
        lp->count = (uint32_t)i - lp->first + 1u;
        lp->totalItems = wg; lp->totalTiles += g.tiles; lp->realItems += g.tiles * g.slices;
        slabOff += (slab + 255) / 256 * 256; tileOff += g.tiles; sliceOff += g.slices;
    }
    finish_launch(fmt, env, W, ws, P, lp);
    return EFFORT_OK;
}

}
```

### effort_amd/runtime.py

```python
from __future__ import annotations

import ctypes as C

import torch

from . import _lib


class Gpu:
    def __init__(self, device: int | None = None):
        if not torch.cuda.is_available():
            raise RuntimeError("effort_amd needs an AMD GPU (torch.cuda.is_available() is False); there is no CPU fallback")
        self.device = torch.cuda.current_device() if device is None else int(device)
        self._lib = _lib.lib()
        with torch.cuda.device(self.device):
            stream = torch.cuda.current_stream(self.device).cuda_stream
            self.ctx = self._lib.effort_create(self.device, C.c_void_p(stream))
        self.has_comm = False
        self.dense_rocblas = False
        if not self.ctx:
            raise RuntimeError("effort_create failed: " + (self._lib.effort_last_error(None) or b"").decode())
        self._stream = stream

    def _bind_stream(self):
        cur = torch.cuda.current_stream(self.device)
        stream = cur.cuda_stream
        if stream != self._stream:
            old = getattr(self, "_stream_obj", None)
            if old is not None and not torch.cuda.is_current_stream_capturing():
                try:
                    cur.wait_stream(old)
                except RuntimeError:
                    pass
            self._lib.effort_set_stream(self.ctx, C.c_void_p(stream))
            self._stream = stream
        self._stream_obj = cur

    def check(self, rc: int, where: str):
        if rc != 0:
            detail = self._lib.effort_last_error(self.ctx)
            raise _lib.EffortError(rc, where, detail.decode() if detail else "")

    def eval(self):
        self.check(self._lib.effort_sync(self.ctx), "gpu.eval")

    def set_overlap(self, lanes: int = 4):
        self._bind_stream()
        self.check(self._lib.effort_set_overlap(self.ctx, int(lanes)), "set_overlap")

    def join(self):
        self.check(self._lib.effort_join(self.ctx), "join")

    def set_row_reuse(self, reuse: bool = True):
        self.check(self._lib.effort_set_row_reuse(self.ctx, int(bool(reuse))), "set_row_reuse")

    @staticmethod
    def comm_unique_id() -> bytes:
        buf = (C.c_char * 128)()
        rc = _lib.lib().effort_comm_unique_id(buf)
        if rc != 0:
            raise _lib.EffortError(rc, "comm_unique_id")
        return bytes(buf)

    def comm_create(self, rank: int, world: int, uid: bytes):
        if len(uid) != 128:
            raise ValueError("the communicator id is 128 bytes")
        self._bind_stream()
        self.check(self._lib.effort_comm_create(self.ctx, int(rank), int(world), C.c_char_p(uid)), "comm_create")
        self.has_comm = True

    def comm_destroy(self):
        self.check(self._lib.effort_comm_destroy(self.ctx), "comm_destroy")
        self.has_comm = False

    @property
    def comm_world(self) -> int:
        return int(self._lib.effort_comm_world(self.ctx))

    @property
    def comm_rank(self) -> int:
        return int(self._lib.effort_comm_rank(self.ctx))

    def allgather_outputs(self, send: torch.Tensor, recv: torch.Tensor, count: int | None = None):
        n = int(send.numel() if count is None else count)
        if not (send.is_cuda and recv.is_cuda and send.dtype == torch.float32 and recv.dtype == torch.float32 and send.is_contiguous()
                and recv.is_contiguous() and send.numel() >= n and recv.numel() >= n * self.comm_world):
            raise ValueError("allgather_outputs: contiguous f32 CUDA tensors, recv holding world * count elements")
        self._bind_stream()
        self.check(self._lib.effort_allgather_outputs(self.ctx, C.c_void_p(send.data_ptr()), C.c_void_p(recv.data_ptr()), n), "allgather_outputs")

    def hook_lane(self, lane: int):
        self.check(self._lib.effort_debug_hook_lane(self.ctx, int(lane)), "hook_lane")

    def set_tuning(self, waves: int = 0, elems: int = 0, slices: int = 0):
        self.check(self._lib.effort_set_tuning(self.ctx, waves, elems, slices), "set_tuning")

    def set_split_cutoff(self, split: bool = True):
        self.check(self._lib.effort_set_split_cutoff(self.ctx, int(split)), "set_split_cutoff")

    def enable_kernel_timing(self, mode: int = 1):
        self._bind_stream()
        self.check(self._lib.effort_enable_kernel_timing(self.ctx, int(mode)), "enable_kernel_timing")

    def kernel_clock(self):
        us, n = C.c_double(), C.c_int()
        self.check(self._lib.effort_kernel_clock(self.ctx, C.byref(us), C.byref(n)), "kernel_clock")
        return {"mul_us": us.value, "launches": n.value}

    def set_persistent(self, wg_per_cu: int = -1):
        self.check(self._lib.effort_set_persistent(self.ctx, int(wg_per_cu)), "set_persistent")

    def set_dense_backend(self, rocblas: bool = False):
        self.check(self._lib.effort_set_dense_backend(self.ctx, int(bool(rocblas))), "set_dense_backend")
        self.dense_rocblas = bool(rocblas)

    def convert_status(self) -> int:
        n = C.c_int(0)
        self.check(self._lib.effort_convert_status(self.ctx, C.byref(n)), "convert_status")
        return int(n.value)

    def debug_stamps(self):
        buf = (C.c_ulonglong * 32)()
        self.check(self._lib.effort_debug_stamps(self.ctx, buf), "debug_stamps")
        return list(buf)

    def slice_counts(self, idx: int = 0, n: int = 4096):
        buf = (C.c_uint32 * n)()
        k = self._lib.effort_debug_slice_counts(self.ctx, int(idx), buf, n)
        if k < 0:
            self.check(k, "slice_counts")
        return list(buf[:k])

    def debug_trace(self, n: int = 4096):
        buf = (C.c_ulonglong * (12 * n))()
        self.check(self._lib.effort_debug_trace(self.ctx, buf, n), "debug_trace")
        return [tuple(buf[8 * i:8 * i + 8]) + tuple(buf[8 * n + 4 * i:8 * n + 4 * i + 4]) for i in range(n)]

    def kernel_timing(self):
        mul, cut, integ, n = C.c_double(), C.c_double(), C.c_double(), C.c_int()
        self.check(self._lib.effort_kernel_timing(self.ctx, C.byref(mul), C.byref(cut), C.byref(integ), C.byref(n)), "kernel_timing")
        return {"mul_us": mul.value, "cutoff_us": cut.value, "integrate_us": integ.value, "samples": n.value}

    def last_dispatch_count(self, idx: int = 0) -> int:
        n = C.c_uint32()
        self.check(self._lib.effort_group_dispatch_count(self.ctx, int(idx), C.byref(n)), "last_dispatch_count")
        return int(n.value)

    def last_cutoff(self, idx: int = 0) -> float:
        x = C.c_float()
        self.check(self._lib.effort_group_cutoff(self.ctx, int(idx), C.byref(x)), "last_cutoff")
        return float(x.value)

    def close(self):
        if getattr(self, "ctx", None):
            self._lib.effort_destroy(self.ctx)
            self.ctx = None

    def __del__(self):
        try:
            self.close()
        except Exception:
            pass


def plan(calls, *, q4: bool = False, numCU: int = 256, lanes: int = 1, persistent: int = -1, waves: int = 0, elems: int = 0, slices: int = 0) -> dict:
    n = len(calls)
    rows = [tuple(c) + (16, 0, 0)[len(c) - 3:] for c in calls]
    ints = lambda k: (C.c_int * n)(*[int(r[k]) for r in rows])
    out = [(C.c_int * max(n, 2))() for _ in range(9)]
    k = _lib.lib().effort_debug_plan(int(q4), numCU, lanes, n, ints(0), ints(1), ints(3), ints(4), ints(5), (C.c_double * n)(*[float(r[2]) for r in rows]),
                                     persistent, waves, elems, slices, *out)
    if k < 0:
        raise _lib.EffortError(k, "plan")
    we, per_call, per_launch = out[0], out[1:5], out[5:]
    res = {"W": we[0], "E": we[1]}
    res.update({name: list(a[:n]) for name, a in zip(("slices", "tiles", "sliceRows", "launch"), per_call)})
    res.update({name: list(a[:k]) for name, a in zip(("persistent", "cutJobs", "compact", "stagger"), per_launch)})
    return res


_gpus: dict[int, Gpu] = {}


def gpu(device: int | None = None) -> Gpu:
    if not torch.cuda.is_available():
        raise RuntimeError("effort_amd needs an AMD GPU (torch.cuda.is_available() is False); there is no CPU fallback")
    d = torch.cuda.current_device() if device is None else int(device)
    g = _gpus.get(d)
    if g is None:
        g = _gpus[d] = Gpu(d)
    return g
```

### include/effort_hip_debug.h

```cpp
#ifndef EFFORT_HIP_DEBUG_H
#define EFFORT_HIP_DEBUG_H

#include "effort_hip.h"

#ifdef __cplusplus
extern "C" {
#endif

EFFORT_API int effort_set_tuning(effort_ctx* ctx, int wavesPerGroup, int elemsPerLane, int rowSlices);
EFFORT_API int effort_set_split_cutoff(effort_ctx* ctx, int split);

EFFORT_API int effort_set_persistent(effort_ctx* ctx, int wgPerCU);

EFFORT_API int effort_debug_hook_lane(effort_ctx* ctx, int lane);

EFFORT_API int effort_is_lab_build(void);
EFFORT_API int effort_enable_kernel_timing(effort_ctx* ctx, int enable);
EFFORT_API int effort_kernel_clock(effort_ctx* ctx, double* mul_us_avg, int* n_launches);
EFFORT_API int effort_kernel_timing(effort_ctx* ctx, double* mul_us_avg, double* cutoff_us_avg,
                         double* integrate_us_avg, int* n_samples);
EFFORT_API int effort_debug_occupancy(effort_ctx* ctx, int q4, int waves, int elems, int ldsBytes);
EFFORT_API int effort_debug_stamps(effort_ctx* ctx, unsigned long long* host32);
EFFORT_API int effort_debug_slice_counts(effort_ctx* ctx, int idx, uint32_t* host, int maxSlices);
EFFORT_API int effort_debug_plan(int q4, int numCU, int lanes, int n, const int* inDim, const int* outDim, const int* percentLoad,
                      const int* prologue, const int* hasResid, const double* effort, int persistent, int tuneW, int tuneE, int tuneS,
                      int* we, int* slices, int* tiles, int* sliceRows, int* launchOf,
                      int* launchPersistent, int* launchCutJobs, int* launchCompact, int* launchStagger);
EFFORT_API int effort_debug_trace(effort_ctx* ctx, unsigned long long* host, int maxRecords);

#ifdef __cplusplus
}
#endif
#endif
```

Measured before the change: 21610.

## Chain consecutive row slices per persistent work item to reuse accumulators

Adds an item-chaining mode in which a persistent workgroup processes 2 or 4 consecutive input slices of the same output tile in sequence. It keeps the LDS accumulator across them and writes partial results to the slab only once, shrinking slab traffic and the final reduction. The shared scale exponent is computed from a bound that covers all chained slices, and the next slice is prefetched directly without pulling from the queue. The heuristic turns chaining on only for laned (multi-device) fp16 launches; the single-GPU default stays at 1, so the benchmark path likely does not change. In exchange there is less parallelism per item and some precision headroom is lost to the wider bound.

```diff
diff --git a/effort_amd/_lib.py b/effort_amd/_lib.py
--- a/effort_amd/_lib.py
+++ b/effort_amd/_lib.py
@@ -66,6 +66,7 @@
     "effort_group_cutoff": (C.c_int, [_P, C.c_int, C.POINTER(C.c_float)]),
     "effort_debug_occupancy": (C.c_int, [_P, C.c_int, C.c_int, C.c_int, C.c_int]),
     "effort_set_persistent": (C.c_int, [_P, C.c_int]),
+    "effort_set_item_slices": (C.c_int, [_P, C.c_int]),
     "effort_debug_hook_lane": (C.c_int, [_P, C.c_int]),
     "effort_add_rmsnorm_mul": (C.c_int, [_P, _P, _P, _P, _P, C.c_int]),
     "effort_rope_kv": (C.c_int, [_P, _P, _P, _P, _P, _P, _P, _P, C.c_int, C.c_int, C.c_int, C.c_int, C.c_float]),
@@ -100,7 +101,7 @@
     "effort_enable_kernel_timing": (C.c_int, [_P, C.c_int]),
     "effort_debug_stamps": (C.c_int, [_P, C.POINTER(C.c_ulonglong)]),
     "effort_debug_slice_counts": (C.c_int, [_P, C.c_int, C.POINTER(C.c_uint32), C.c_int]),
-    "effort_debug_plan": (C.c_int, [C.c_int, C.c_int, C.c_int, C.c_int, _P, _P, _P, _P, _P, _P, C.c_int, C.c_int, C.c_int, C.c_int, _P, _P, _P, _P, _P, _P, _P, _P, _P]),
+    "effort_debug_plan": (C.c_int, [C.c_int, C.c_int, C.c_int, C.c_int, _P, _P, _P, _P, _P, _P, C.c_int, C.c_int, C.c_int, C.c_int, C.c_int, _P, _P, _P, _P, _P, _P, _P, _P, _P, _P, _P, _P]),
     "effort_debug_trace": (C.c_int, [_P, C.POINTER(C.c_ulonglong), C.c_int]),
     "effort_kernel_clock": (C.c_int, [_P, C.POINTER(C.c_double), C.POINTER(C.c_int)]),
     "effort_kernel_timing": (C.c_int, [_P, C.POINTER(C.c_double), C.POINTER(C.c_double), C.POINTER(C.c_double), C.POINTER(C.c_int)]),
diff --git a/effort_amd/csrc/api.hip b/effort_amd/csrc/api.hip
--- a/effort_amd/csrc/api.hip
+++ b/effort_amd/csrc/api.hip
@@ -55,6 +55,7 @@
     size_t convElems = 0;
     int* d_status = nullptr;
     int persistent = -1;
+    int chain = -1;
     static constexpr uint32_t kMaxTiles = 1024, kMaxSlices = 4096;
     static constexpr size_t kSlabBytes = (size_t)64 << 20;
     static constexpr size_t kMaxRanges = 1024;
@@ -639,7 +640,7 @@
 static PlanEnv plan_env(const effort_ctx* c, bool laned, bool thinEffort) {
     PlanEnv env;
     env.numCU = c->numCU; env.nLanes = c->nLanes; env.laned = laned;
-    env.persistent = c->persistent; env.tuneW = c->tuneW; env.tuneE = c->tuneE; env.tuneS = c->tuneS;
+    env.persistent = c->persistent; env.chain = c->chain; env.tuneW = c->tuneW; env.tuneE = c->tuneE; env.tuneS = c->tuneS;
     env.splitCutoff = c->splitCutoff; env.clock = c->clock;
     env.slabBytes = c->slabBytes; env.maxTiles = effort_ctx::kMaxTiles; env.maxSlices = effort_ctx::kMaxSlices;
     env.thinEffort = thinEffort;
@@ -702,7 +703,7 @@
         ga.slabs = L.d_slabs; ga.counters = L.d_counters; ga.sliceCounts = L.d_sliceCounts; ga.cutoff = L.d_cutoff + lp.first;
         ga.tstamp = c->clock ? c->d_tstamp : nullptr;
         ga.ablate = env.ablate; ga.trace = (c->clock && c->trace) ? 1u : 0u;
-        ga.split = (c->splitCutoff ? 1u : 0u) | (lp.compact ? 4u : 0u) | (c->rowReuse ? 8u : 0u);
+        ga.split = (c->splitCutoff ? 1u : 0u) | (lp.compact ? 4u : 0u) | (c->rowReuse ? 8u : 0u) | ((lp.chain == 4u ? 2u : lp.chain == 2u ? 1u : 0u) << 4);
         ga.numCU = (uint32_t)c->numCU; ga.queue = L.d_queue;
         ga.count = lp.count; ga.totalTiles = lp.totalTiles; ga.totalItems = lp.totalItems;
         ga.persistent = lp.persistent; ga.cutJobs = lp.cutJobs; ga.staggerSleeps = lp.staggerSleeps;
@@ -801,14 +802,14 @@
     return (int)n;
 }
 extern "C" int effort_debug_plan(int q4, int numCU, int lanes, int n, const int* inDim, const int* outDim, const int* percentLoad,
-                                 const int* prologue, const int* hasResid, const double* effort, int persistent, int tuneW, int tuneE, int tuneS,
-                                 int* we, int* slices, int* tiles, int* sliceRows, int* launchOf,
+                                 const int* prologue, const int* hasResid, const double* effort, int persistent, int tuneW, int tuneE, int tuneS, int itemSlices,
+                                 int* we, int* slices, int* tiles, int* sliceRows, int* launchOf, int* itemSlicesOf, int* slabOff, int* itemEnd,
                                  int* launchPersistent, int* launchCutJobs, int* launchCompact, int* launchStagger) {
     if (numCU < 1 || lanes < 1 || lanes > effort_ctx::kMaxLanes || n < 1 || n > kMaxGroup || !inDim || !outDim || !effort || !we || !slices || !tiles ||
-        !sliceRows || !launchOf || !launchPersistent || !launchCutJobs || !launchCompact || !launchStagger) return EFFORT_ERR_ARG;
+        !sliceRows || !launchOf || !itemSlicesOf || !slabOff || !itemEnd || !(itemSlices == -1 || itemSlices == 1 || itemSlices == 2 || itemSlices == 4) || !launchPersistent || !launchCutJobs || !launchCompact || !launchStagger) return EFFORT_ERR_ARG;
     const Format fmt = q4 ? kQ4 : kFp16;
     effort_ctx c0;
-    c0.numCU = numCU; c0.nLanes = lanes; c0.persistent = persistent; c0.tuneW = tuneW; c0.tuneE = tuneE; c0.tuneS = tuneS;
+    c0.numCU = numCU; c0.nLanes = lanes; c0.persistent = persistent; c0.chain = itemSlices; c0.tuneW = tuneW; c0.tuneE = tuneE; c0.tuneS = tuneS;
     c0.slabBytes = effort_ctx::kSlabBytes;
     PlanCall pc[kMaxGroup];
     for (int i = 0; i < n; i++) {
@@ -825,6 +826,7 @@
     for (int i = 0; i < n; i++) {
         const CallPlan& p = plan.call[i];
         slices[i] = (int)p.g.slices; tiles[i] = (int)p.g.tiles; sliceRows[i] = (int)p.g.sliceRows; launchOf[i] = (int)p.launch;
+        itemSlicesOf[i] = (int)p.chain; slabOff[i] = (int)p.slabOff; itemEnd[i] = (int)(p.chain > 1u ? p.itemEnd8 : p.itemEnd8 * 8u);
     }
     for (uint32_t l = 0; l < plan.nLaunches; l++) {
         const LaunchPlan& lp = plan.launch[l];
@@ -1061,6 +1063,12 @@
     return bucket_mul_occupancy(q4 ? kQ4 : kFp16, W, E, (size_t)ldsBytes);
 }
 
+extern "C" int effort_set_item_slices(effort_ctx* c, int n) {
+    if (!c) return EFFORT_ERR_ARG;
+    if (!(n == -1 || n == 1 || n == 2 || n == 4)) return fail(c, EFFORT_ERR_ARG, "set_item_slices: -1 (heuristic), 1, 2 or 4");
+    c->chain = n;
+    return EFFORT_OK;
+}
 extern "C" int effort_set_persistent(effort_ctx* c, int wgPerCU) {
     if (!c || wgPerCU < -1 || wgPerCU > 8) return EFFORT_ERR_ARG;
     c->persistent = wgPerCU;
diff --git a/effort_amd/csrc/bucket_mul.hip b/effort_amd/csrc/bucket_mul.hip
--- a/effort_amd/csrc/bucket_mul.hip
+++ b/effort_amd/csrc/bucket_mul.hip
@@ -141,6 +141,17 @@
     return p;
 }
 struct ItemRef { uint32_t ci, t, s; };
+__host__ __device__ __forceinline__ uint32_t chain_log2(const GroupKArgs& ga) { return (ga.split >> 4) & 3u; }
+__device__ __forceinline__ bool locate_chained(const GroupKArgs& ga, const uint32_t item, const uint32_t lg, ItemRef& r) {
+    const uint32_t idx = (item & 7u) * (ga.totalItems >> 3) + (item >> 3);
+    uint32_t ci = 0;
+    for (uint32_t i = 0; i + 1 < ga.count; i++) if (idx >= (uint32_t)ga.wgEnd8[i]) ci = i + 1;
+    ci = __builtin_amdgcn_readfirstlane(ci);
+    const MulGeom& g = ga.geom[ga.call[ci].geom];
+    const uint32_t b = idx - (ci ? (uint32_t)ga.wgEnd8[ci - 1] : 0u), grp = b / g.tiles;
+    r.ci = ci; r.s = grp << lg; r.t = b - grp * g.tiles;
+    return idx < (uint32_t)ga.wgEnd8[ga.count - 1];
+}
 
 __device__ __forceinline__ bool locate_item(const GroupKArgs& ga, const uint32_t item, ItemRef& r) {
     uint32_t ci = 0;
@@ -220,9 +231,16 @@
     }
 }
 
+struct ChainRef {
+    uint32_t lg;
+    uint32_t sub, nSub;
+    int kexp;
+};
 template <int FMT, int E, int W, bool FUSED, bool COMPACT, bool PERSIST, typename Prefetch>
 __device__ __forceinline__ void mul_item(const GroupKArgs& ga, const uint32_t item, const ItemRef& ref, char* smem, const LdsPlan& lp, uint32_t& cachedCall,
-                                         float& cachedCutoff, const uint32_t par, const bool staged, const bool firstItem, Prefetch prefetch) {
+                                         float& cachedCutoff, const uint32_t par, const bool staged, const bool firstItem, ChainRef& ch, Prefetch prefetch) {
+    constexpr bool kChain = PERSIST && !FUSED && FMT == kFp16;
+    const bool first = !kChain || ch.sub == 0u, last = !kChain || ch.sub + 1u >= ch.nSub;
     constexpr int NACC = Fmt<FMT>::kAcc;
     constexpr int TILE_F = NACC * E * 64;
     constexpr int TILE_L = Fmt<FMT>::kSlots * E * 64;
@@ -271,8 +289,9 @@
     const float* means = reinterpret_cast<const float*>(smem + offM);
 
     const uint32_t j0 = s * B;
-    uint32_t vSlabOff = (s * g.tiles + t) * (uint32_t)(TILE_F * 4), vSlabBytes = (uint32_t)min((size_t)0xFFFFFFFFu, (size_t)g.slices * g.tiles * TILE_F * 4);
-    uint32_t vSlices = g.slices, vSliceStride = g.tiles * (uint32_t)(TILE_F * 4);
+    const uint32_t clg = kChain ? ch.lg : 0u, nGroups = kChain ? (g.slices + (1u << clg) - 1u) >> clg : g.slices;
+    uint32_t vSlabOff = ((kChain ? s >> clg : s) * g.tiles + t) * (uint32_t)(TILE_F * 4), vSlabBytes = (uint32_t)min((size_t)0xFFFFFFFFu, (size_t)nGroups * g.tiles * TILE_F * 4);
+    uint32_t vSlices = nGroups, vSliceStride = g.tiles * (uint32_t)(TILE_F * 4);
     if constexpr (!PERSIST) asm volatile("" : "+v"(vSlabOff), "+v"(vSlabBytes), "+v"(vSlices), "+v"(vSliceStride));
     const uint32_t nb = min(B, g.inDim - j0);
     const uint32_t e = a.expNo ? a.expNo[0] : 0u;
@@ -418,6 +437,20 @@
     uint32_t* const cutWords = ga.queue + 9 * 16;
     uint32_t cutWord = 0;
     if (viaJob && tid == 0 && !(GA_ABLATE(ga) & 32u)) cutWord = __hip_atomic_load(&cutWords[ci], __ATOMIC_RELAXED, __HIP_MEMORY_SCOPE_AGENT);
+    float vLater = 0.0f;
+    if constexpr (kChain) {
+        if (first && ch.nSub > 1u) {
+            float x[3];
+#pragma unroll
+            for (uint32_t k = 1; k < 4u; k++) {
+                const uint32_t j = j0 + k * B + (uint32_t)tid;
+                const bool ok = k < ch.nSub && (uint32_t)tid < B && j < g.inDim;
+                x[k - 1u] = a.v[ok ? j : j0];
+                x[k - 1u] = ok ? fabsf(x[k - 1u]) : 0.0f;
+            }
+            vLater = (x[0] + x[1]) + x[2];
+        }
+    }
     asm volatile("s_waitcnt vmcnt(0)" ::: "memory");
     EFFORT_PSTAMP(4)
     uint32_t vColOK = 0, voff = 0, vRecords = 0, vBuckLo = 0, vBuckHi = 0, vRowPitch = 0, vInDim = 0, vRow0 = 0;
@@ -455,6 +488,7 @@
             bound += fabsf(x);
         }
     }
+    if constexpr (kChain) bound += vLater;
     bound = wave_sum_f32(bound);
     if (lane == 0) wbound[wave] = bound;
     if (tid == 0) { flags[4] = 0u; flags[5] = (uint32_t)(W * KB); }
@@ -508,13 +542,19 @@
 #pragma unroll
     for (int w2 = 0; w2 < W; w2++) wb[w2] = wbound[w2];
     __builtin_amdgcn_sched_barrier(0);
-    for (int i = tid; i < TILE_L; i += NT) acc[i] = 0;
+    if (first) for (int i = tid; i < TILE_L; i += NT) acc[i] = 0;
     float L = 0.0f;
 #pragma unroll
     for (int w2 = 0; w2 < W; w2++) L += wb[w2];
     L *= rankBound;
     int kexp = 30 - (int)((__float_as_uint(L) >> 23) & 0xFFu) + 126;
+    if constexpr (kChain) {
+        if (ch.lg != 0u && (__float_as_uint(L) & 0x7FFFFFu) < 0x7F0000u) kexp += 1;
+    }
     kexp = L > 0.0f ? max(-100, min(100, kexp)) : 0;
+    if constexpr (kChain) {
+        if (first) ch.kexp = __builtin_amdgcn_readfirstlane(kexp); else kexp = ch.kexp;
+    }
     const float scale = __uint_as_float((uint32_t)(127 + kexp) << 23), unscale = __uint_as_float((uint32_t)(127 - kexp) << 23);
     if (stamp) GA_TSTAMP(ga)[18] = wall_clock64();
     if (wstamp) ph[2] = wall_clock64();
@@ -861,6 +901,7 @@
         return r;
     };
     if (fused && t == 0 && s == 0 && tid == 0 && !GA_CUTJOBS(ga)) a_cutoff[0] = cutoff;
+    if constexpr (kChain) { if (!last) return; }
     {
         constexpr int kIt = (TILE_F + NT * 2 - 1) / (NT * 2);
         float s0[kIt], s1[kIt];
@@ -1097,30 +1138,46 @@
     uint32_t gen = 0;
     if (threadIdx.x == 0) __hip_atomic_store(&s_next, 0ull, __ATOMIC_RELAXED, __HIP_MEMORY_SCOPE_WORKGROUP);
     uint32_t item = GA_PERSISTENT(ga) ? pull_sync() : blockIdx.x;
+    constexpr bool kChain = PERSIST && kPipe;
+    ItemRef ref = {0u, 0u, 0u};
+    ChainRef ch = {0u, 0u, 1u, 0};
+    if constexpr (kChain) ch.lg = chain_log2(ga);
+    bool more = false;
     while (item < total) {
-        if (item < GA_CUTJOBS(ga)) {
-            if (item < ga.count) cutoff_job<64 * W>(ga, item, smem);
-            item = GA_PERSISTENT(ga) ? pull_sync() : total;
-            continue;
-        }
-        ItemRef ref;
-        EFFORT_ESTAMP(1)
-        if (!locate_item(ga, item - GA_CUTJOBS(ga), ref)) {
-            item = GA_PERSISTENT(ga) ? pull_sync() : total;
-            continue;
-        }
-        EFFORT_ESTAMP(2)
-        gen++;
+        if (!kChain || !more) {
+            if (item < GA_CUTJOBS(ga)) {
+                if (item < ga.count) cutoff_job<64 * W>(ga, item, smem);
+                item = GA_PERSISTENT(ga) ? pull_sync() : total;
+                continue;
+            }
+            EFFORT_ESTAMP(1)
+            if (!((kChain && ch.lg) ? locate_chained(ga, item - GA_CUTJOBS(ga), ch.lg, ref) : locate_item(ga, item - GA_CUTJOBS(ga), ref))) {
+                item = GA_PERSISTENT(ga) ? pull_sync() : total;
+                continue;
+            }
+            EFFORT_ESTAMP(2)
+            gen++;
+            if constexpr (kChain) { ch.sub = 0u; ch.nSub = min(1u << ch.lg, ga.geom[ga.call[ref.ci].geom].slices - ref.s); }
+        }
         bool stagedNext = false;
+        const bool lastSub = !kChain || ch.sub + 1u >= ch.nSub;
         auto prefetch = [&]() -> bool {
             if (!GA_PERSISTENT(ga)) return true;
-            if (threadIdx.x == 0)
-                __hip_atomic_store(&s_next, ((unsigned long long)gen << 32) | (unsigned long long)pull(), __ATOMIC_RELAXED, __HIP_MEMORY_SCOPE_WORKGROUP);
-            const unsigned long long nx = __hip_atomic_load(&s_next, __ATOMIC_RELAXED, __HIP_MEMORY_SCOPE_WORKGROUP);
-            if (__builtin_amdgcn_readfirstlane((uint32_t)(nx >> 32)) != gen) return false;
-            const uint32_t next = __builtin_amdgcn_readfirstlane((uint32_t)nx);
             ItemRef nref;
-            if (kPipe && !(GA_ABLATE(ga) & 128u) && next >= GA_CUTJOBS(ga) && next < total && locate_item(ga, next - GA_CUTJOBS(ga), nref)) {
+            bool real = false;
+            if (kChain && !lastSub) {
+                nref = ref; nref.s = ref.s + 1u;
+                real = true;
+            } else {
+                if (threadIdx.x == 0)
+                    __hip_atomic_store(&s_next, ((unsigned long long)gen << 32) | (unsigned long long)pull(), __ATOMIC_RELAXED, __HIP_MEMORY_SCOPE_WORKGROUP);
+                const unsigned long long nx = __hip_atomic_load(&s_next, __ATOMIC_RELAXED, __HIP_MEMORY_SCOPE_WORKGROUP);
+                if (__builtin_amdgcn_readfirstlane((uint32_t)(nx >> 32)) != gen) return false;
+                const uint32_t next = __builtin_amdgcn_readfirstlane((uint32_t)nx);
+                if (kPipe && !(GA_ABLATE(ga) & 128u) && next >= GA_CUTJOBS(ga) && next < total)
+                    real = (kChain && ch.lg) ? locate_chained(ga, next - GA_CUTJOBS(ga), ch.lg, nref) : locate_item(ga, next - GA_CUTJOBS(ga), nref);
+            }
+            if (kPipe && real) {
                 int tid0 = threadIdx.x;
                 asm volatile("" : "+v"(tid0));
                 stage_issue<FMT, W, COMPACT>(ga, nref, tid0, smem, lp, par ^ 1u);
@@ -1129,10 +1186,12 @@
             return true;
         };
         const bool firstOwn = gen == 1u && (GA_ABLATE(ga) & 512u) != 0u;
-        mul_item<FMT, E, W, FUSED, COMPACT, PERSIST>(ga, item - GA_CUTJOBS(ga), ref, smem, lp, cachedCall, cachedCutoff, par, staged, firstOwn, prefetch);
-        item = GA_PERSISTENT(ga) ? __builtin_amdgcn_readfirstlane((uint32_t)__hip_atomic_load(&s_next, __ATOMIC_RELAXED, __HIP_MEMORY_SCOPE_WORKGROUP)) : total;
+        mul_item<FMT, E, W, FUSED, COMPACT, PERSIST>(ga, item - GA_CUTJOBS(ga), ref, smem, lp, cachedCall, cachedCutoff, par, staged, firstOwn, ch, prefetch);
+        more = kChain && !lastSub;
+        if (!more) item = GA_PERSISTENT(ga) ? __builtin_amdgcn_readfirstlane((uint32_t)__hip_atomic_load(&s_next, __ATOMIC_RELAXED, __HIP_MEMORY_SCOPE_WORKGROUP)) : total;
         staged = stagedNext;
         par ^= 1u;
+        if (more) { ch.sub++; ref.s++; }
     }
     if (GA_PERSISTENT(ga) && threadIdx.x == 0) {
         const uint32_t gone = __hip_atomic_fetch_add(&ga.queue[8 * 16], 1u, __ATOMIC_RELAXED, __HIP_MEMORY_SCOPE_AGENT);
@@ -1155,13 +1214,20 @@
     const LdsPlan lp = ga.lp = plan_lds<FMT, E, W>(ga.geom, kMaxGeoms, lean || (kLean && kProductOnly));
     uint32_t lds = lp.total;
     if (lp.offA > 65536u && FMT == kFp16) return hipErrorInvalidValue;
+    const uint32_t chainLg = chain_log2(ga);
+    if (chainLg > 2u) return hipErrorInvalidValue;
+    if (chainLg) {
+        if (FMT != kFp16 || !ga.persistent) return hipErrorInvalidValue;
+        for (uint32_t i = 0; i < ga.count; i++) if (ga.call[i].pre || ga.call[i].resid) return hipErrorInvalidValue;
+    }
     for (uint32_t i = 0; i < ga.count; i++) {
         const MulGeom& g = ga.geom[ga.call[i].geom];
         if (g.slots > (uint32_t)kRounds * 64 * W || g.slots != (FMT == kFp16 ? (g.rowsPerIn << g.sliceLog2) : g.sliceRows * 8u)) return hipErrorInvalidValue;
         if (FMT == kFp16 ? (1u << g.sliceLog2) > 64u * W : g.sliceRows > 128u * W) return hipErrorInvalidValue;
-        if (((uint32_t)ga.wgEnd8[i] - (i ? (uint32_t)ga.wgEnd8[i - 1] : 0u)) * 8u != align_up(g.tiles * g.slices, 8)) return hipErrorInvalidValue;
-    }
-    if (ga.totalItems != (uint32_t)ga.wgEnd8[ga.count - 1] * 8u) return hipErrorInvalidValue;
+        const uint32_t range = (uint32_t)ga.wgEnd8[i] - (i ? (uint32_t)ga.wgEnd8[i - 1] : 0u);
+        if (chainLg ? range != g.tiles * ((g.slices + (1u << chainLg) - 1u) >> chainLg) : range * 8u != align_up(g.tiles * g.slices, 8)) return hipErrorInvalidValue;
+    }
+    if (ga.totalItems != (chainLg ? align_up((uint32_t)ga.wgEnd8[ga.count - 1], 8) : (uint32_t)ga.wgEnd8[ga.count - 1] * 8u)) return hipErrorInvalidValue;
     uint32_t grid = ga.totalItems;
     if (ga.persistent) {
         const uint32_t R = ga.persistent;
diff --git a/effort_amd/csrc/plan.h b/effort_amd/csrc/plan.h
--- a/effort_amd/csrc/plan.h
+++ b/effort_amd/csrc/plan.h
@@ -10,6 +10,7 @@
     bool laned = false;
     int persistent = -1;
     int tuneW = 0, tuneE = 0, tuneS = 0;
+    int chain = -1;
     bool splitCutoff = false, clock = false;
     uint32_t ablate = 0;
     bool noJobs = false, noCompact = false;
@@ -27,6 +28,7 @@
 struct CallPlan {
     MulGeom g;
     uint32_t mult;
+    uint32_t chain;
     uint32_t launch, geom;
     uint32_t slabOff, tileOff, sliceOff;
     uint32_t itemEnd8;
@@ -35,6 +37,7 @@
     uint32_t first, count;
     uint32_t persistent, cutJobs, staggerSleeps;
     bool compact;
+    uint32_t chain;
     uint32_t totalItems, totalTiles, realItems;
 };
 struct GroupPlan {
diff --git a/effort_amd/csrc/plan.hip b/effort_amd/csrc/plan.hip
--- a/effort_amd/csrc/plan.hip
+++ b/effort_amd/csrc/plan.hip
@@ -183,7 +183,7 @@
     return k;
 }
 
-static void finish_launch(Format fmt, const PlanEnv& env, int W, const PlanCall* ws, const GroupPlan* P, LaunchPlan* lp) {
+static void finish_launch(Format fmt, const PlanEnv& env, int W, const PlanCall* ws, GroupPlan* P, LaunchPlan* lp) {
     const uint32_t R = env.persistent < 0 ? 2u : (uint32_t)env.persistent;
     const uint32_t perCU = (env.persistent < 0 && fmt == kFp16 && !env.laned) ? 6u : R;
     lp->persistent = (R && lp->realItems > (uint32_t)env.numCU * perCU) ? R : 0u;
@@ -199,6 +199,25 @@
     }
     lp->compact = compact;
     lp->staggerSleeps = (lp->persistent && fmt == kQ4 && !env.laned) ? 11u : 0u;
+    uint32_t chain = 1u;
+    if (fmt == kFp16 && lp->persistent && lp->cutJobs && plain) {
+        bool resid = false;
+        for (uint32_t i = 0; i < lp->count; i++) resid = resid || ws[lp->first + i].hasResid;
+        if (!resid) chain = env.chain < 0 ? (env.laned ? 2u : 1u) : (uint32_t)env.chain;
+    }
+    if (chain > 1u) {
+        uint32_t end = 0;
+        for (uint32_t i = 0; i < lp->count; i++) { const MulGeom& g = P->call[lp->first + i].g; end += g.tiles * ((g.slices + chain - 1u) / chain); }
+        if (end > 0xFFFFu) chain = 1u;
+    }
+    lp->chain = chain;
+    uint32_t end = 0;
+    for (uint32_t i = 0; i < lp->count; i++) {
+        CallPlan& a = P->call[lp->first + i];
+        a.chain = chain;
+        if (chain > 1u) { end += a.g.tiles * ((a.g.slices + chain - 1u) / chain); a.itemEnd8 = end; }
+    }
+    if (chain > 1u) lp->totalItems = round8(end);
 }
 
 int plan_group(Format fmt, const PlanEnv& env, int n, const PlanCall* ws, GroupPlan* P) {
diff --git a/effort_amd/runtime.py b/effort_amd/runtime.py
--- a/effort_amd/runtime.py
+++ b/effort_amd/runtime.py
@@ -110,6 +110,9 @@
     def set_persistent(self, wg_per_cu: int = -1):
         self.check(self._lib.effort_set_persistent(self.ctx, int(wg_per_cu)), "set_persistent")
 
+    def set_chain(self, n: int = -1):
+        self.check(self._lib.effort_set_item_slices(self.ctx, int(n)), "set_chain")
+
     def set_dense_backend(self, rocblas: bool = False):
         self.check(self._lib.effort_set_dense_backend(self.ctx, int(bool(rocblas))), "set_dense_backend")
         self.dense_rocblas = bool(rocblas)
@@ -163,18 +166,19 @@
             pass
 
 
-def plan(calls, *, q4: bool = False, numCU: int = 256, lanes: int = 1, persistent: int = -1, waves: int = 0, elems: int = 0, slices: int = 0) -> dict:
+def plan(calls, *, q4: bool = False, numCU: int = 256, lanes: int = 1, persistent: int = -1, waves: int = 0, elems: int = 0, slices: int = 0,
+         chain: int = -1) -> dict:
     n = len(calls)
     rows = [tuple(c) + (16, 0, 0)[len(c) - 3:] for c in calls]
     ints = lambda k: (C.c_int * n)(*[int(r[k]) for r in rows])
-    out = [(C.c_int * max(n, 2))() for _ in range(9)]
+    out = [(C.c_int * max(n, 2))() for _ in range(12)]
     k = _lib.lib().effort_debug_plan(int(q4), numCU, lanes, n, ints(0), ints(1), ints(3), ints(4), ints(5), (C.c_double * n)(*[float(r[2]) for r in rows]),
-                                     persistent, waves, elems, slices, *out)
+                                     persistent, waves, elems, slices, chain, *out)
     if k < 0:
         raise _lib.EffortError(k, "plan")
-    we, per_call, per_launch = out[0], out[1:5], out[5:]
+    we, per_call, per_launch = out[0], out[1:8], out[8:]
     res = {"W": we[0], "E": we[1]}
-    res.update({name: list(a[:n]) for name, a in zip(("slices", "tiles", "sliceRows", "launch"), per_call)})
+    res.update({name: list(a[:n]) for name, a in zip(("slices", "tiles", "sliceRows", "launch", "chain", "slabOff", "itemEnd"), per_call)})
     res.update({name: list(a[:k]) for name, a in zip(("persistent", "cutJobs", "compact", "stagger"), per_launch)})
     return res
 
diff --git a/include/effort_hip_debug.h b/include/effort_hip_debug.h
--- a/include/effort_hip_debug.h
+++ b/include/effort_hip_debug.h
@@ -11,6 +11,7 @@
 EFFORT_API int effort_set_split_cutoff(effort_ctx* ctx, int split);
 
 EFFORT_API int effort_set_persistent(effort_ctx* ctx, int wgPerCU);
+EFFORT_API int effort_set_item_slices(effort_ctx* ctx, int n);
 
 EFFORT_API int effort_debug_hook_lane(effort_ctx* ctx, int lane);
 
@@ -23,8 +24,8 @@
 EFFORT_API int effort_debug_stamps(effort_ctx* ctx, unsigned long long* host32);
 EFFORT_API int effort_debug_slice_counts(effort_ctx* ctx, int idx, uint32_t* host, int maxSlices);
 EFFORT_API int effort_debug_plan(int q4, int numCU, int lanes, int n, const int* inDim, const int* outDim, const int* percentLoad,
-                      const int* prologue, const int* hasResid, const double* effort, int persistent, int tuneW, int tuneE, int tuneS,
-                      int* we, int* slices, int* tiles, int* sliceRows, int* launchOf,
+                      const int* prologue, const int* hasResid, const double* effort, int persistent, int tuneW, int tuneE, int tuneS, int itemSlices,
+                      int* we, int* slices, int* tiles, int* sliceRows, int* launchOf, int* itemSlicesOf, int* slabOff, int* itemEnd,
                       int* launchPersistent, int* launchCutJobs, int* launchCompact, int* launchStagger);
 EFFORT_API int effort_debug_trace(effort_ctx* ctx, unsigned long long* host, int maxRecords);
 
```

After: 21080. -2.5%, worse.
